# henryhungle/MTN

Measured on AMD Instinct MI355X. Metric: train-step samples/sec (d_model=512, 6L MTN), higher is better.
Workload: dtype bf16; 1 GPU; cfg2: d_model=512 N=6 h=8 d_ff=2048 |V|=3000 Q/H/C/T=20/128/40/20 frames=[32, 32] ft=[2048, 128]; batch_per_gpu=32, global_batch=32, parallelism=dp1, hip_graph=True, rccl_ranks=1

## Files before the change

### include/mtn_hip.h

```cpp
#ifndef MTN_HIP_H
#define MTN_HIP_H

#include <stdint.h>

#ifdef __cplusplus
extern "C" {
#endif

#define MTN_F32 0
#define MTN_BF16 1

#define MTN_OK 0
#define MTN_ERR_ARG 1
#define MTN_ERR_LAUNCH 2

const char* mtn_last_error(void);
int mtn_version(void);

typedef struct {
    float p;
    uint32_t salt;
    const uint64_t* seed;
} mtn_dropout;

// ... 79 lines not shown
} mtn_ln_fwd_desc;
typedef struct {
    int rows, d;
    const long* tokens;
    const float* dx;
    float emb_scale;
    mtn_dropout drop;
    float* dlut;
    int lut_rows;
} mtn_embed_bwd_desc;
int mtn_embed_bwd_group(int count, const mtn_embed_bwd_desc* descs , void* stream);
typedef struct {
    int rows, d;
    float eps;
    const float *x, *a2, *mean, *rstd, *g, *dres;
    float* dx;
    float* partial;
    void* dx_lp;
    int dx_lp_dtype;
    mtn_dropout dx_lp_drop;
} mtn_ln_bwd_desc;
int mtn_layernorm_fwd_group(int dtype, int count, const mtn_ln_fwd_desc* descs , void* stream);
int mtn_layernorm_bwd_group(int count, const mtn_ln_bwd_desc* descs , void* stream);
int mtn_layernorm_fwd(int dtype, int rows, int d, float eps, const float* x, const float* a2, const float* b2,
                      float* y_f32, void* y_lp, float* mean, float* rstd, void* stream);
typedef struct {
    const void* w;
    const float *bias, *a2, *b2;
    float* out;
    int K, block_start;
} mtn_ln_fold_desc;
int mtn_ln_fold(int dtype, const mtn_ln_fold_desc* descs_device, const int* block_desc, int total_blocks, int d, void* stream);
long mtn_layernorm_bwd_partial_floats(int rows, int d);
int mtn_layernorm_bwd_nparts(int rows);
typedef struct {
    const float* partial;
    int nparts, d;
    float *da2, *db2;
} mtn_ln_finalize_desc;
#define MTN_LN_FINALIZE_MAX_GROUP 112
int mtn_layernorm_bwd_finalize(int count, const mtn_ln_finalize_desc* descs , void* stream);
int mtn_layernorm_bwd(int rows, int d, float eps, const float* x, const float* a2, const float* mean,
                      const float* rstd, const float* g, const float* dres, float* dx, float* da2, float* db2,
                      float* partial, void* stream);

typedef struct {
    int B, h, a, m, dk;
    const void *q, *k, *v;
    int ldq, ldkv;
    const uint8_t* mask;
    long mask_sb, mask_sq;
    mtn_dropout drop;
    void* o;
    int ldo;
    float* lse;
    const void* d_o;
    void *dq, *dk_out, *dv_out;
    int q0, qn, kv_accum;
    float* kv_acc;
    int kv_last;
} mtn_attn_args;
#define MTN_ATTN_MAX_GROUP 4
int mtn_attention_fwd_group(int dtype, int count, const mtn_attn_args* args , void* stream);
int mtn_attention_bwd_group(int dtype, int count, const mtn_attn_args* args , void* stream);
int mtn_attention_fwd(int dtype, const mtn_attn_args* args, void* stream);
int mtn_attention_bwd(int dtype, const mtn_attn_args* args, void* stream);

typedef struct {
    int B, a, m, d, h;
    int self_attn;
    float ln_eps;
    mtn_dropout drop_attn;
    mtn_dropout drop_out;
    const float* x;
    const void* mem;
    const uint8_t* mask;
    long mask_sb, mask_sq;
    const float *ln_a, *ln_b;
    const void* w_qkv;
    const float* b_qkv;
    const void* w_o;
    const float* b_o;
    const void* w_qkv_t;
    const void* w_o_t;
    float* y;
    void* xn;
    float* mean;
    float* rstd;
    void* qkv;
    void* kv;
    void* o;
    float* lse;
    const float* dy;
    float* dx;
    float* dmem;
    int dmem_accumulate;
    float *d_ln_a, *d_ln_b;
    float *d_w_qkv, *d_b_qkv, *d_w_o, *d_b_o;
    void* ws_lp;
    float* ws_f32;
    int defer_param_grads;
    const void* dyl_ready;
    void* next_dyl;
    mtn_dropout next_drop;
    int kv_ready;
    void* dmem_lp;
    mtn_dropout dmem_lp_drop;
    const float* ln_fold;
} mtn_mha_args;
int mtn_mha_sublayer_fwd(int dtype, const mtn_mha_args* args, void* stream);
int mtn_mha_sublayer_bwd(int dtype, const mtn_mha_args* args, void* stream);
int mtn_mha_param_grad_work(int dtype, const mtn_mha_args* args, mtn_gemm_problem* out3, mtn_ln_finalize_desc* out_ln);
long mtn_mha_bwd_ws_lp_elems(int B, int a, int m, int d, int self_attn);
long mtn_mha_bwd_ws_f32_floats(int B, int a, int m, int d);

typedef struct {
    int rows, d, d_ff;
    float ln_eps;
    mtn_dropout drop_hidden;
    mtn_dropout drop_out;
    const float* x;
    const float *ln_a, *ln_b;
    const void* w1;
    const float* b1;
    const void* w2;
    const float* b2;
    const void* w1_t;
    const void* w2_t;
    float* y;
    void* xn;
    float* mean;
    float* rstd;
    void* hid;
    const float* dy;
    float* dx;
    float *d_ln_a, *d_ln_b, *d_w1, *d_b1, *d_w2, *d_b2;
    void* ws_lp;
    float* ws_f32;
    int defer_param_grads;
    const void* dyl_ready;
    void* next_dyl;
    mtn_dropout next_drop;
    void* y_lp;
    const float* ln_fold;
} mtn_ffn_args;
int mtn_ffn_sublayer_fwd(int dtype, const mtn_ffn_args* args, void* stream);
int mtn_ffn_sublayer_bwd(int dtype, const mtn_ffn_args* args, void* stream);
long mtn_ffn_bwd_ws_f32_floats(int rows, int d, int d_ff);
int mtn_ffn_param_grad_work(int dtype, const mtn_ffn_args* args, mtn_gemm_problem* out2, mtn_ln_finalize_desc* out_ln);

#define MTN_SUBLAYER_MAX_GROUP 4
int mtn_fused_enable(int on);
int mtn_fused_counters(long* out4);
long mtn_ln_epilogue_groups(void);
int mtn_sublayer_group_fwd(int dtype, int n_mha, const mtn_mha_args* mha, int n_ffn, const mtn_ffn_args* ffn, void* stream);
int mtn_sublayer_group_bwd(int dtype, int n_mha, const mtn_mha_args* mha, int n_ffn, const mtn_ffn_args* ffn, void* stream);

int mtn_cast_f32_to_lp(int dtype, long n, const float* src, void* dst, void* stream);
typedef struct {
    long n;
    const float* src;
    void* dst;
    mtn_dropout drop;
    const float* gate;
} mtn_cast_desc;
#define MTN_CAST_MAX_GROUP 8
int mtn_cast_group(int dtype, int count, const mtn_cast_desc* descs , void* stream);
int mtn_dropout_bwd_to_lp(int dtype, long n, const float* src, mtn_dropout drop, void* dst, void* stream);

#define MTN_LOSSHEAD_MAX_SEG 4
typedef struct {
    int n_seg;
    int rows[MTN_LOSSHEAD_MAX_SEG];
    const long* target[MTN_LOSSHEAD_MAX_SEG];
    const float* norm[MTN_LOSSHEAD_MAX_SEG];
    float coef[MTN_LOSSHEAD_MAX_SEG];
    int V, ldz, pad;
    float smoothing;
    const float* logits;
    float* lse;
    float* rowloss;
    const float* gloss;
    void* dlogits;
    int ldd;
} mtn_losshead_args;
int mtn_losshead_fwd(const mtn_losshead_args* args, void* stream);
int mtn_losshead_bwd(int dtype, const mtn_losshead_args* args, void* stream);

typedef struct {
    long off;
    int rows, cols;
    int tile_start;
    int reserved;
    long dst_off;
} mtn_transpose_desc;
int mtn_transpose_group(int dtype, const void* src, void* dst, const mtn_transpose_desc* descs_device, int count,
                        int total_tiles, void* stream);

int mtn_noam_tick(float* state, float factor, int model_size, int warmup, float beta1, float beta2, void* stream);
int mtn_adam_step(int dtype, long n, float* p, const float* g, float* m, float* v, void* p_lp, const float* state,
                  const float* grad_scale, float beta1, float beta2, float eps, void* stream);
int mtn_adam_step_chunks(int dtype, int n_chunks, const long* off, const int* len, float* p, const float* g, float* m, float* v,
                         void* p_lp, const float* state, const float* grad_scale, float beta1, float beta2, float eps, void* stream);

#define MTN_ASSEMBLE_MAX_GROUP 8
typedef struct {
    const int64_t* flat;
    const int64_t* start;
    const int32_t* len;
    const int32_t* ids;
    int B, L;
    int64_t pad;
    int64_t* out;
    uint8_t* mask;
    uint8_t* std_mask;
    int64_t* n_nonpad;
    const int32_t* row_len;
} mtn_assemble_tokens_desc;
int mtn_assemble_tokens(int count, const mtn_assemble_tokens_desc* descs , void* stream);
typedef struct {
    const float* flat;
    const int64_t* start;
    const int32_t* len;
    const int32_t* ids;
    int B, V, F, skip;
    float* out;
    uint8_t* mask;
} mtn_assemble_features_desc;
int mtn_assemble_features(int count, const mtn_assemble_features_desc* descs , void* stream);

int mtn_topk_rows(const float* x, int rows, int V, long ldx, int k, int extra_col, float* out, void* stream);
typedef struct {
    int dialogues, width, L, k_top, k, beam, unk, eos, pad, min_len;
    double penalty;
    const float* top;
    long* tokens; int* pos; int* anc;
    double* lp; int* n_live; int* step; int* flags;
    int* log_parent; int* log_tok; double* log_score; double* log_done; int* log_n_old; int* log_n_new;
} mtn_beam_args;
int mtn_beam_advance(const mtn_beam_args* args , void* stream);
typedef struct {
    mtn_beam_args beam;
    int groups; float diversity;
} mtn_diverse_args;
int mtn_diverse_advance(const mtn_diverse_args* args , void* stream);
typedef struct {
    int rows, V; long ldx;
    const float* logp;
    float temperature; int top_k; float top_p;
    int n_banned; int banned[4]; int eos, min_len;
    const long* seed;
    const long* key;
    int* step;
    int L;
    int* log_tok; float* log_logp; float* log_u;
    long* tokens; int* pos; int* anc;
} mtn_sample_args;
int mtn_sample_rows(const mtn_sample_args* args , void* stream);
typedef struct {
    int n_seq, L, V, pad; long ldz;
    const float* logits;
    const long* target;
    float* tok_logp;
    int* tok_rank;
    double* seq_logp;
    int* seq_len;
} mtn_score_args;
int mtn_score_rows(const mtn_score_args* args , void* stream);
typedef struct {
    int rows, V; long ldx, ldo;
    const float* logp; float* out;
    int ngram; float theta;
    int L;
    const int* hist; long ldh; const int* hist_len;
    const int* log_tok; const int* log_parent; const int* step;
    int width, rows_per_step;
} mtn_constrain_args;
int mtn_constrain_rows(const mtn_constrain_args* args , void* stream);
typedef struct {
    int rows, V, M, mode;
    const float* x[8]; long ld[8]; float w[8];
    float* out; long ldo;
} mtn_ensemble_args;
int mtn_ensemble_rows(const mtn_ensemble_args* args , void* stream);
int mtn_log_softmax_rows(const float* x, int rows, int V, long ldx, float* out, long ldo, void* stream);

typedef struct {
    int dtype, count, variant, workgroups;
    double flops, bytes;
    int M[4], N[4], K[4];
} mtn_census_launch;
int mtn_census_begin(void);
int mtn_census_end(void);
int mtn_census_info(int i, mtn_census_launch* out);
int mtn_census_replay(int i, int reps, void* stream);
const char* mtn_census_variant_name(int variant);
int mtn_measure_mfma_peak(int iters, float* scratch, void* stream, double* tflops);
int mtn_measure_mfma_peak_shapes(int iters, float* scratch, void* stream, double* tflops_16x16x32, double* tflops_32x32x16);
int mtn_measure_hbm_peak(const void* src, void* dst, long bytes, void* stream, double* gbps);
#define MTN_DEC_EMBED 0
#define MTN_DEC_SELF_QKV 1
#define MTN_DEC_SELF_ATT 2
#define MTN_DEC_OUT 3
#define MTN_DEC_CROSS 4
#define MTN_DEC_FFN1 5
#define MTN_DEC_FFN2 6
// ... 34 lines not shown
```

### mtn_amd/csrc/elementwise.hip

```cpp
#include <stdarg.h>
#include <stdlib.h>

#include "common.h"

static thread_local char g_err[512] = "";
void mtn_set_error(const char* fmt, ...) {
    va_list ap;
    va_start(ap, fmt);
    vsnprintf(g_err, sizeof(g_err), fmt, ap);
    va_end(ap);
}
extern "C" const char* mtn_last_error(void) { return g_err; }
extern "C" int mtn_version(void) { return 119; }

#include <mutex>
static int g_env_gen = 0;
static std::mutex g_env_mutex;
extern "C" int mtn_reload_env(void) { return __atomic_add_fetch(&g_env_gen, 1, __ATOMIC_ACQ_REL); }
const char* mtn_env_lookup(MtnEnvVar* v) {
    const int g = __atomic_load_n(&g_env_gen, __ATOMIC_ACQUIRE);
    if (__atomic_load_n(&v->gen, __ATOMIC_ACQUIRE) != g) {
        std::lock_guard<std::mutex> lock(g_env_mutex);
        if (v->gen != g) {
            const char* e = getenv(v->name);
            v->set = e != nullptr;
            if (e) { strncpy(v->val, e, sizeof(v->val) - 1); v->val[sizeof(v->val) - 1] = 0; }
            __atomic_store_n(&v->gen, g, __ATOMIC_RELEASE);
        }
    }
    return v->set ? v->val : nullptr;
}

static inline int grid_for(long n_vec) {
    long b = (n_vec + 255) / 256;
    if (b > 2048) b = 2048;
    if (b < 1) b = 1;
    return (int)b;
}

struct CastGroup {
    int count;
    mtn_cast_desc d[MTN_CAST_MAX_GROUP];
};

template <typename T>
__global__ __launch_bounds__(256) void cast_kernel(const CastGroup grp) {
    const mtn_cast_desc& D = grp.d[blockIdx.y];
    const long n = D.n;
    const float* __restrict__ src = D.src;
    T* __restrict__ dst = (T*)D.dst;
    const DropState ds = drop_init(D.drop);
    const long n4 = n >> 2;
    for (long i = (long)blockIdx.x * 256 + threadIdx.x; i < n4; i += (long)gridDim.x * 256) {
        float4 v = *(const float4*)(src + i * 4);
        if (ds.on) {
            v.x = drop_keep(ds, (uint64_t)(i * 4 + 0)) ? v.x * ds.scale : 0.f;
            v.y = drop_keep(ds, (uint64_t)(i * 4 + 1)) ? v.y * ds.scale : 0.f;
            v.z = drop_keep(ds, (uint64_t)(i * 4 + 2)) ? v.z * ds.scale : 0.f;
            v.w = drop_keep(ds, (uint64_t)(i * 4 + 3)) ? v.w * ds.scale : 0.f;
        }
        if (D.gate) {
            const float4 gt = *(const float4*)(D.gate + i * 4);
            v.x = gt.x > 0.f ? v.x : 0.f; v.y = gt.y > 0.f ? v.y : 0.f; v.z = gt.z > 0.f ? v.z : 0.f; v.w = gt.w > 0.f ? v.w : 0.f;
        }
        if constexpr (sizeof(T) == 2) {
            uint2 u;
            u.x = (uint32_t)f32_to_bf16(v.x) | ((uint32_t)f32_to_bf16(v.y) << 16);
            u.y = (uint32_t)f32_to_bf16(v.z) | ((uint32_t)f32_to_bf16(v.w) << 16);
            *(uint2*)(dst + i * 4) = u;
        } else {
            *(float4*)(dst + i * 4) = v;
        }
    }
    if (blockIdx.x == 0 && threadIdx.x < (n & 3)) {
        long i = (n4 << 2) + threadIdx.x;
        float v = src[i];
        if (ds.on) v = drop_keep(ds, (uint64_t)i) ? v * ds.scale : 0.f;
        if (D.gate && !(D.gate[i] > 0.f)) v = 0.f;
        dst[i] = LP<T>::from_f32(v);
    }
}

extern "C" int mtn_cast_group(int dtype, int count, const mtn_cast_desc* descs, void* stream) {
    MTN_CHECK_ARG(dtype == MTN_F32 || dtype == MTN_BF16, "bad dtype");
    MTN_CHECK_ARG(count >= 1 && count <= MTN_CAST_MAX_GROUP && descs, "bad group");
    CastGroup grp;
    memset(&grp, 0, sizeof(grp));
    grp.count = count;
    long nmax = 0;
    for (int i = 0; i < count; ++i) {
        MTN_CHECK_ARG(descs[i].n > 0 && descs[i].src && descs[i].dst, "bad cast descriptor");
        grp.d[i] = descs[i];
        if (descs[i].n > nmax) nmax = descs[i].n;
    }
    hipStream_t s = (hipStream_t)stream;
    dim3 grid(grid_for(nmax >> 2), count);
    if (dtype == MTN_BF16) hipLaunchKernelGGL((cast_kernel<bf16_t>), grid, dim3(256), 0, s, grp);
    else hipLaunchKernelGGL((cast_kernel<float>), grid, dim3(256), 0, s, grp);
    MTN_CHECK_LAUNCH();
    return MTN_OK;
}

static int launch_cast(int dtype, long n, const float* src, void* dst, mtn_dropout drop, void* stream) {
    mtn_cast_desc D = {n, src, dst, drop, nullptr};
    return mtn_cast_group(dtype, 1, &D, stream);
}

extern "C" int mtn_cast_f32_to_lp(int dtype, long n, const float* src, void* dst, void* stream) {
    mtn_dropout none = {0.f, 0u, nullptr};
    return launch_cast(dtype, n, src, dst, none, stream);
}
extern "C" int mtn_dropout_bwd_to_lp(int dtype, long n, const float* src, mtn_dropout drop, void* dst, void* stream) {
    return launch_cast(dtype, n, src, dst, drop, stream);
}

template <typename T>
__global__ __launch_bounds__(256) void transpose_group_kernel(const T* __restrict__ src, T* __restrict__ dst,
                                                              const mtn_transpose_desc* __restrict__ descs, int count) {
    constexpr int V = 16 / (int)sizeof(T);
    __shared__ __attribute__((aligned(16))) T tile[64][64 + V];
    int lo = 0, hi = count - 1;
    const int b = blockIdx.x;
    while (lo < hi) {
        int mid = (lo + hi + 1) >> 1;
        if (descs[mid].tile_start <= b) lo = mid; else hi = mid - 1;
    }
    const mtn_transpose_desc D = descs[lo];
    const int tiles_c = (D.cols + 63) >> 6;
    const int t = b - D.tile_start;
    const int r0 = (t / tiles_c) * 64, c0 = (t % tiles_c) * 64;
    const T* s = src + D.off;
    T* d = dst + D.dst_off;
    const bool full = (r0 + 64 <= D.rows) && (c0 + 64 <= D.cols) && (D.rows % V == 0) && (D.cols % V == 0) && (D.off % V == 0) && (D.dst_off % V == 0);
    if (full) {
        constexpr int VPR = 64 / V;
        for (int i = threadIdx.x; i < 64 * VPR; i += 256) {
            const int r = i / VPR, cv = (i % VPR) * V;
            *(uint4*)&tile[r][cv] = *(const uint4*)(s + (size_t)(r0 + r) * D.cols + c0 + cv);
        }
        __syncthreads();
        for (int i = threadIdx.x; i < 64 * VPR; i += 256) {
            const int c = i / VPR, rv = (i % VPR) * V;
            __attribute__((aligned(16))) T tmp[V];
#pragma unroll
            for (int k = 0; k < V; ++k) tmp[k] = tile[rv + k][c];
            *(uint4*)(d + (size_t)(c0 + c) * D.rows + r0 + rv) = *(const uint4*)tmp;
        }
        return;
    }
    const int tx = threadIdx.x & 63, ty = threadIdx.x >> 6;
#pragma unroll 4
    for (int i = 0; i < 16; ++i) {
        const int r = r0 + ty + 4 * i, c = c0 + tx;
        if (r < D.rows && c < D.cols) tile[ty + 4 * i][tx] = s[(size_t)r * D.cols + c];
    }
    __syncthreads();
#pragma unroll 4
    for (int i = 0; i < 16; ++i) {
        const int c = c0 + ty + 4 * i, r = r0 + tx;
        if (r < D.rows && c < D.cols) d[(size_t)c * D.rows + r] = tile[tx][ty + 4 * i];
    }
}

extern "C" int mtn_transpose_group(int dtype, const void* src, void* dst, const mtn_transpose_desc* descs_device, int count,
                                   int total_tiles, void* stream) {
    MTN_CHECK_ARG(dtype == MTN_F32 || dtype == MTN_BF16, "bad dtype");
// ... 183 lines not shown
```

### mtn_amd/csrc/fused.hip

```cpp
#include "fused_common.h"

struct FhMember {
    int kind;
    int rows;
    int rows_per_wg;
    int nslice;
    int a, m, blk;
    int mt;
    int hg, sg;
    int late_v;
    int nks;
    int ncols;
    int ld_out;
    float eps;
    const float* x;
    const float* ln_a;
    const float* ln_b;
    const bf16_t* w;
    const float* bias;
    const bf16_t* mem;
    bf16_t* xn;
    float* mean;
    float* rstd;
    bf16_t* out;
    bf16_t* kv;
    const uint8_t* mask;
    long mask_sb, mask_sq;
    mtn_dropout drop;
    bf16_t* o;
    float* lse;
    int b_off;
};
struct FhGroup {
    int count;
    int stop;
#ifdef FH_TIMELINE
    unsigned long long* dbg;
#endif
    int wg_start[FH_MAX_MEMBERS + 1];
    FhMember m[FH_MAX_MEMBERS];
};

struct FhLds { int gains, xn, xm, qi, ki, vi, mask, total; };
__host__ __device__ inline FhLds fh_lds_map(int mt, bool raw, int key_rows, int pad_rows, int mask_bytes, int ffn_blocks = 0, bool late_v = false) {
    FhLds L;
    L.gains = 0;
    L.xn = 4096 + 1024;
    const int krows = ((key_rows + pad_rows + 7) & ~7);
    if (late_v) {
        L.vi = L.xn;
        const int top = mt * 16 * FH_ROWB > krows * FH_HROWB ? mt * 16 * FH_ROWB : krows * FH_HROWB;
        L.xm = L.xn + top;
        L.qi = L.xm;
        L.ki = L.qi + mt * 16 * FH_HROWB;
        L.mask = L.ki + krows * FH_HROWB;
        L.total = L.mask + ((mask_bytes + 15) & ~15);
        return L;
    }
    L.xm = L.xn + mt * 16 * FH_ROWB;
    L.qi = L.xm + (raw ? mt * 16 * FH_ROWB : 0);
    L.ki = L.qi + mt * 16 * (ffn_blocks ? ffn_blocks * FH_HROWB : FH_HROWB);
    L.vi = L.ki + krows * FH_HROWB;
    L.mask = L.vi + krows * FH_HROWB;
    L.total = L.mask + ((mask_bytes + 15) & ~15);
    return L;
}
static constexpr int FH_PART_FLOATS = 18;
__host__ __device__ inline int fh_pad_rows(int kind, int mk) { return kind == FH_CROSS_READY ? ((mk + 63) & ~63) - mk : 64; }

#ifdef FH_TIMELINE
#define FH_STAMP(k) do { if (threadIdx.x == 0) G.dbg[(size_t)blockIdx.x * 16 + (k)] = wall_clock64(); } while (0)
#define FH_STAMP_CLK(k) do { if (threadIdx.x == 0) G.dbg[(size_t)blockIdx.x * 16 + (k)] = clock64(); } while (0)
#else
#define FH_STAMP(k) do { } while (0)
#define FH_STAMP_CLK(k) do { } while (0)
#endif

template <int NP, int MT>
__device__ __forceinline__ void fh_body(const FhGroup& G, const FhMember& M, const int slice, const int rb, unsigned char* smem) {
    constexpr int NG = (MT * 4 + 7) / 8;
    constexpr int NT = NP * MT;
    const int tid = threadIdx.x;
    const int row0 = rb * M.rows_per_wg;
    const int R = (M.rows - row0) < M.rows_per_wg ? (M.rows - row0) : M.rows_per_wg;
    const int lane = tid & 63, l15 = lane & 15, lg = lane >> 4;
    const int wave = __builtin_amdgcn_readfirstlane(tid >> 6);
    const int wc = wave & 3, kh = wave >> 2;
    const int kind = M.kind;
    const bool raw = kind == FH_CROSS_RAW, ffn = kind == FH_FFN;
    const int a = M.a, m = M.m;
    const int nsamp = ffn ? 0 : R / a, b0 = rb * M.blk;
    const int Rm = raw ? nsamp * m : 0, rm0 = b0 * m;
    const int mk = kind == FH_SELF ? a : m;
    const int key_rows = ffn ? 0 : ((kind == FH_SELF || raw) ? MT * 16 : nsamp * m);
    const int qa = M.mask_sq ? a : 1;
    const int mask_bytes = ffn ? 0 : nsamp * qa * m;
    const bool late_v = kind == FH_CROSS_READY && M.late_v != 0;
    const FhLds L = fh_lds_map(MT, raw, key_rows, fh_pad_rows(kind, mk), mask_bytes, ffn ? NP : 0, late_v);
    unsigned char* xn_s = smem + L.xn;
    unsigned char* xm_s = smem + L.xm;
    unsigned char* qi_s = smem + L.qi;
    unsigned char* ki_s = smem + L.ki;
    unsigned char* vi_s = smem + L.vi;
    unsigned char* mk_s = smem + L.mask;

    float4 gv = make_float4(0.f, 0.f, 0.f, 0.f);
    if (tid < 256) gv = *(const float4*)((tid < 128 ? M.ln_a : M.ln_b - FH_D) + tid * 4);
    int ncol[NP];
    bool act[NP];
#pragma unroll
    for (int p = 0; p < NP; ++p) {
        if (ffn) { ncol[p] = slice * (64 * NP) + p * 64; act[p] = ncol[p] + 16 * wc < M.ncols; }
        else { ncol[p] = p * FH_D + slice * FH_DK; act[p] = (p == 0) || (p < 3 && kind != FH_CROSS_READY); }
    }
    float bias_v = 0.f;
    if (tid < 64 * NP) {
        const int p_ = tid >> 6;
        bool on = false;
        int nc = 0;
#pragma unroll
        for (int p = 0; p < NP; ++p) if (p == p_) { on = act[p] || (ffn && ncol[p] + (tid & 63) < M.ncols); nc = ncol[p]; }
        if (on) bias_v = M.bias[nc + (tid & 63)];
    }
    uint8_t mkb[FH_MASKB];
    const uint8_t* mask_g = M.mask ? M.mask + (size_t)b0 * M.mask_sb : nullptr;
    const bool mask_wide = M.mask == nullptr || (M.mask_sb != 0 && (((size_t)mask_g | (size_t)mask_bytes) & 7) == 0);
    unsigned mkw0 = 0x01010101u, mkw1 = 0x01010101u;
    if (mask_wide) {
        if (M.mask && 8 * tid < mask_bytes) { mkw0 = *(const unsigned*)(mask_g + 8 * tid); mkw1 = *(const unsigned*)(mask_g + 8 * tid + 4); }
    } else {
#pragma unroll
        for (int i = 0; i < FH_MASKB; ++i) {
            const int idx = tid + FH_THREADS * i;
            mkb[i] = 1;
            if (idx < mask_bytes) mkb[i] = mask_g[M.mask_sb ? idx : idx % (qa * m)];
        }
    }
    const float* __restrict__ xg = M.x + (size_t)row0 * FH_D;
    float4 xv[NG][8];
#pragma unroll
    for (int i = 0; i < NG; ++i) {
        const int r = 4 * (wave + 8 * i) + lg;
        const bool ok = r < R;
#pragma unroll
        for (int j = 0; j < 8; ++j)
            xv[i][j] = ok ? *(const float4*)(xg + (size_t)r * FH_D + 64 * j + 4 * l15) : make_float4(0.f, 0.f, 0.f, 0.f);
    }
    FH_STAMP(14);
    if (raw) {
        const fh_rsrc_t rsrc = fh_make_rsrc(M.mem + (size_t)rm0 * FH_D, (unsigned)(Rm * FH_ROWB));
        for (int r = wave; r < MT * 16; r += 8) {
            const unsigned voff = r < Rm ? (unsigned)r * FH_ROWB + (unsigned)((lane ^ (r & 15)) << 4) : 0x80000000u;
            fh_dma16(rsrc, (unsigned)(size_t)(xm_s + r * FH_ROWB), voff);
        }
    }
    auto issue_kv_dma = [&]() {
        const int Kr = nsamp * m;
        const bf16_t* kbase = M.kv + (size_t)rm0 * (2 * FH_D) + slice * FH_DK;
        const fh_rsrc_t rk = fh_make_rsrc(kbase, (unsigned)((Kr - 1) * (4 * FH_D) + FH_HROWB));
        const fh_rsrc_t rv = fh_make_rsrc(kbase + FH_D, (unsigned)((Kr - 1) * (4 * FH_D) + FH_HROWB));
        const int ninst = ((Kr + fh_pad_rows(kind, mk) + 7) & ~7) >> 3;
        for (int i = wave; i < ninst; i += 8) {
            const int row = i * 8 + (lane >> 3), slot = lane & 7;
            const unsigned vk = row < Kr ? (unsigned)row * (4 * FH_D) + (unsigned)((slot ^ (row & 7)) << 4) : 0x80000000u;
            const unsigned vv = row < Kr ? (unsigned)row * (4 * FH_D) + (unsigned)((slot ^ ((row >> 1) & 7)) << 4) : 0x80000000u;
            fh_dma16(rk, (unsigned)(size_t)(ki_s + i * 1024), vk);
            if (!late_v) fh_dma16(rv, (unsigned)(size_t)(vi_s + i * 1024), vv);
        }
    };
    uint4 wf[NP][8];
    auto issue_weights = [&]() {
#pragma unroll
        for (int p = 0; p < NP; ++p) {
            if (act[p]) {
                const bf16_t* wrow = M.w + (size_t)(ncol[p] + 16 * wc + (lane >> 2)) * FH_D + kh * 256 + (lane & 3) * 8;
#pragma unroll
                for (int s = 0; s < 8; ++s) wf[p][s] = *(const uint4*)(wrow + s * 32);
            } else {
#pragma unroll
                for (int s = 0; s < 8; ++s) wf[p][s] = make_uint4(0, 0, 0, 0);
            }
        }
    };
    auto issue_block = [&](const int p_) {
#pragma unroll
        for (int p = 0; p < NP; ++p) {
            if (p != p_) continue;
            const int nc = act[p] ? ncol[p] : ncol[0];
            const bf16_t* wrow = M.w + (size_t)(nc + 16 * wc + (lane >> 2)) * FH_D + kh * 256 + (lane & 3) * 8;
#pragma unroll
            for (int s = 0; s < 8; ++s) wf[p][s] = *(const uint4*)(wrow + s * 32);
        }
    };
    if (mask_wide) {
// ... 218 lines not shown

    FH_STAMP(8);
    if (late_v || kind == FH_CROSS_READY) {
        asm volatile("s_waitcnt vmcnt(0)" ::: "memory");
        __syncthreads();
    }
    const float scale = 0.125f;
    const int nqt = (a + 15) >> 4;
    auto attend = [&](const int si, const int qt, const int cbeg, const int cend, f32x4_t (&ot)[4], float& mrun, float& lrun) {
        const int b = b0 + si;
        const DropBase dbase = drop_base((uint64_t)((b + M.b_off) * (FH_D / FH_DK) + slice) * (uint64_t)a * (uint64_t)mk);
        const int q = qt * 16 + l15, qc = q < a ? q : a - 1;
        const int qrow = si * a + qc, krow0 = si * mk;
        uint4 qf[2];
#pragma unroll
        for (int ks = 0; ks < 2; ++ks) qf[ks] = fh_hfrag(qi_s, qrow, ks * 4 + lg);
#pragma unroll
        for (int nt = 0; nt < 4; ++nt) ot[nt] = f32x4_t{0.f, 0.f, 0.f, 0.f};
        mrun = -INFINITY; lrun = 0.f;
        const unsigned char* mrow = mk_s + (size_t)(si * qa + (M.mask_sq ? qc : 0)) * mk;
        for (int c0 = cbeg; c0 < cend; c0 += 64) {
            const bool wide = mk - c0 > 32;
            f32x4_t st[4];
#pragma unroll
            for (int kt = 0; kt < 4; ++kt) {
                st[kt] = f32x4_t{0.f, 0.f, 0.f, 0.f};
                if (kt >= 2 && !wide) continue;
                int key = c0 + 32 * (kt >> 1) + 8 * (l15 >> 2) + 4 * (kt & 1) + (l15 & 3);
                key = key < mk ? key : mk - 1;
#pragma unroll
                for (int ks = 0; ks < 2; ++ks) mma16<bf16_t>(st[kt], fh_hfrag(ki_s, krow0 + key, ks * 4 + lg), qf[ks]);
            }
            float mx = -INFINITY;
#pragma unroll
            for (int kt = 0; kt < 4; ++kt) {
                if (kt >= 2 && !wide) continue;
#pragma unroll
                for (int r = 0; r < 4; ++r) {
                    const int key = c0 + 32 * (kt >> 1) + 8 * lg + 4 * (kt & 1) + r, kc = key < mk ? key : mk - 1;
                    float sv = mrow[kc] != 0 ? st[kt][r] * scale : -1e9f;
                    sv = key < mk ? sv : -INFINITY;
                    st[kt][r] = sv;
                    mx = fmaxf(mx, sv);
                }
            }
            mx = fh_cross_max(mx);
            const float mn = fmaxf(mrun, mx);
            float psum = 0.f;
#pragma unroll
            for (int kt = 0; kt < 4; ++kt) {
                if (kt >= 2 && !wide) continue;
#pragma unroll
                for (int r = 0; r < 4; ++r) {
                    const int key = c0 + 32 * (kt >> 1) + 8 * lg + 4 * (kt & 1) + r, kc = key < mk ? key : mk - 1;
                    const float pv = __expf(st[kt][r] - mn);
                    psum += pv;
                    st[kt][r] = drop_keep_at(ds, dbase, (uint32_t)(qc * mk + kc)) ? pv * ds.scale : 0.f;
                }
            }
            psum = fh_cross_sum(psum);
            const float alpha = (mrun == -INFINITY) ? 0.f : __expf(mrun - mn);
            lrun = lrun * alpha + psum;
            mrun = mn;
#pragma unroll
            for (int nt = 0; nt < 4; ++nt) { ot[nt][0] *= alpha; ot[nt][1] *= alpha; ot[nt][2] *= alpha; ot[nt][3] *= alpha; }
#pragma unroll
            for (int u = 0; u < 2; ++u) {
                if (u == 1 && !wide) continue;
                const uint4 pf = make_uint4(fh_pack2(st[2 * u][0], st[2 * u][1]), fh_pack2(st[2 * u][2], st[2 * u][3]),
                                            fh_pack2(st[2 * u + 1][0], st[2 * u + 1][1]), fh_pack2(st[2 * u + 1][2], st[2 * u + 1][3]));
                uint4 vf[4];
#pragma unroll
                for (int nt = 0; nt < 4; ++nt) vf[nt] = fh_vfrag(vi_s, krow0 + c0 + 32 * u, nt * 16, l15, lg);
                asm volatile("s_waitcnt lgkmcnt(0)" ::: "memory");
                __builtin_amdgcn_sched_barrier(0);
#pragma unroll
                for (int nt = 0; nt < 4; ++nt) mma16<bf16_t>(ot[nt], vf[nt], pf);
            }
        }
    };
    auto finish = [&](const int si, const int qt, const f32x4_t (&ot)[4], const float mrun, const float lrun) {
        const int b = b0 + si, q = qt * 16 + l15;
        if (q < a) {
            const float inv = 1.0f / lrun;
            bf16_t* og = M.o + (size_t)(b * a + q) * FH_D + slice * FH_DK + 4 * lg;
#pragma unroll
            for (int nt = 0; nt < 4; ++nt)
                *(uint2*)(og + nt * 16) = make_uint2(fh_pack2(ot[nt][0] * inv, ot[nt][1] * inv), fh_pack2(ot[nt][2] * inv, ot[nt][3] * inv));
            if (M.lse && lg == 0) {
                float* stp = M.lse + 2 * ((size_t)(b * (FH_D / FH_DK) + slice) * a + q);
                stp[0] = mrun;
                stp[1] = inv;
            }
        }
    };
    const int nks = M.nks;
    if (nks <= 1) {
        for (int it = wave; it < nsamp * nqt; it += 8) {
            const int si = it / nqt, qt = it - si * nqt;
            f32x4_t ot[4];
            float mrun, lrun;
            attend(si, qt, 0, mk, ot, mrun, lrun);
            finish(si, qt, ot, mrun, lrun);
        }
    } else {
        const int npairs = nsamp * nqt;
        const int pair = wave / nks, kr = wave - pair * nks;
        const bool live = pair < npairs;
        const int si = live ? pair / nqt : 0, qt = live ? pair - si * nqt : 0;
        const int chunks = (mk + 63) >> 6, per = (chunks + nks - 1) / nks;
        int cbeg = kr * per * 64, cend = (kr + 1) * per * 64;
        cend = cend < mk ? cend : mk;
        f32x4_t ot[4];
        float mrun = -INFINITY, lrun = 0.f;
#pragma unroll
        for (int nt = 0; nt < 4; ++nt) ot[nt] = f32x4_t{0.f, 0.f, 0.f, 0.f};
        if (live && cbeg < cend) attend(si, qt, cbeg, cend, ot, mrun, lrun);
        __syncthreads();
        float* part = (float*)ki_s + (size_t)(pair * (nks - 1) + kr - 1) * (FH_PART_FLOATS * 64) + lane;
        if (live && kr != 0) {
#pragma unroll
            for (int nt = 0; nt < 4; ++nt)
#pragma unroll
                for (int r = 0; r < 4; ++r) part[(nt * 4 + r) * 64] = ot[nt][r];
            part[16 * 64] = mrun;
            part[17 * 64] = lrun;
        }
        __syncthreads();
        if (live && kr == 0) {
            for (int k = 1; k < nks; ++k) {
                const float* pk = (const float*)ki_s + (size_t)(pair * (nks - 1) + k - 1) * (FH_PART_FLOATS * 64) + lane;
                const float mo = pk[16 * 64], lo = pk[17 * 64];
                const float mn = fmaxf(mrun, mo);
                const float wa = (mrun == -INFINITY) ? 0.f : __expf(mrun - mn), wb = (mo == -INFINITY) ? 0.f : __expf(mo - mn);
                lrun = lrun * wa + lo * wb;
                mrun = mn;
#pragma unroll
                for (int nt = 0; nt < 4; ++nt)
#pragma unroll
                    for (int r = 0; r < 4; ++r) ot[nt][r] = ot[nt][r] * wa + pk[(nt * 4 + r) * 64] * wb;
            }
            finish(si, qt, ot, mrun, lrun);
        }
    }
    FH_STAMP(9);
    FH_STAMP_CLK(11);
}

template <int NP>
__global__ __launch_bounds__(FH_THREADS) void fused_head_fwd_kernel(const FhGroup G) {
    extern __shared__ __attribute__((aligned(16))) unsigned char smem[];
    FH_STAMP(0);
    FH_STAMP_CLK(10);
    int g = 0;
    while (g + 1 < G.count && (int)blockIdx.x >= G.wg_start[g + 1]) ++g;
    const FhMember& M = G.m[g];
    const int t = (int)blockIdx.x - G.wg_start[g];
    const int xcd = t & 7, j = t >> 3;
    const int hpg = M.nslice / M.hg;
    const int slice = (xcd % M.hg) * hpg + (j % hpg), rb = (j / hpg) * M.sg + (xcd / M.hg);
    FH_STAMP(12);
    if (rb * M.rows_per_wg >= M.rows) return;
    if constexpr (NP == 4) {
        if (M.mt <= 2) fh_body<NP, 2>(G, M, slice, rb, smem);
        else fh_body<NP, 4>(G, M, slice, rb, smem);
    } else {
        if (M.mt <= 2) fh_body<NP, 2>(G, M, slice, rb, smem);
        else if (M.mt == 3) fh_body<NP, 3>(G, M, slice, rb, smem);
        else if (M.mt == 4) fh_body<NP, 4>(G, M, slice, rb, smem);
        else fh_body<NP, 5>(G, M, slice, rb, smem);
    }
}

static int fh_enabled = -1;
extern "C" int mtn_fused_enable(int on) {
    const int prev = fh_enabled;
    fh_enabled = on ? 1 : 0;
    return prev;
}
static bool fh_env_off() {
    if (fh_enabled < 0) fh_enabled = 1;
    return fh_enabled == 0;
}

int fh_is_enabled() { return fh_env_off() ? 0 : 1; }

static constexpr int FH_LDS_MAX = 160 * 1024;
static const int fh_mt_sets[2][4] = {{2, 3, 4, 5}, {2, 4, 4, 4}};

struct FhPlan { int blk, mt, lds, late_v; };
static int fh_member_lds(const mtn_mha_args& A, int blk, int mt, bool late_v = false) {
    const bool self = A.self_attn != 0, raw = !self && !A.kv_ready;
    const int m = self ? A.a : A.m, qa = A.mask_sq ? A.a : 1;
    const int kind = self ? FH_SELF : (raw ? FH_CROSS_RAW : FH_CROSS_READY);
    return fh_lds_map(mt, raw, (self || raw) ? mt * 16 : blk * m, fh_pad_rows(kind, m), blk * qa * m, 0, late_v).total;
}
static FhPlan fh_plan_mha_at(const mtn_mha_args& A, int np, int blk) {
    const int* fh_mt_choices = fh_mt_sets[np == 4];
    const bool self = A.self_attn != 0, raw = !self && !A.kv_ready;
    const int m = self ? A.a : A.m, qa = A.mask_sq ? A.a : 1;
    FhPlan none = {0, 0, 0, 0};
    const int R = blk * A.a, Rm = blk * m;
    int mt = 0;
    for (int c = 0; c < 4; ++c)
        if (fh_mt_choices[c] * 16 >= R && (!raw || fh_mt_choices[c] * 16 >= Rm) && (np == 4 || fh_mt_choices[c] != 4 || A.a > 32)) { mt = fh_mt_choices[c]; break; }
    if (!mt) return none;
    if (A.mask && blk * qa * m > FH_THREADS * FH_MASKB) return none;
    int lds = fh_member_lds(A, blk, mt), late = 0;
    if (lds > FH_LDS_MAX && !self && !raw) {
        lds = fh_member_lds(A, blk, mt, true);
        late = 1;
    }
    if (lds > FH_LDS_MAX) return none;
    return FhPlan{blk, mt, lds, late};
}
static FhPlan fh_plan_mha(const mtn_mha_args& A, int budget, int np) {
    const bool self = A.self_attn != 0;
    const int m = self ? A.a : A.m, qa = A.mask_sq ? A.a : 1;
    FhPlan best = {0, 0, 0, 0};
    if (A.mask && A.mask_sb != 0 && A.mask_sb != (long)qa * m) return best;
    if (A.mask && A.mask_sq != 0 && A.mask_sq != m) return best;
    for (int blk = 1; blk <= A.B; ++blk) {
        const FhPlan pl = fh_plan_mha_at(A, np, blk);
        if (pl.blk == 0) break;
        best = pl;
        if (((A.B + blk - 1) / blk) * (FH_D / FH_DK) <= budget) break;
    }
    return best;
}

static void fh_pick_xcd_map(FhMember& M, int nrb, double x_bytes, double w_bytes) {
    double best = 1e30;
    M.hg = 8; M.sg = 1;
    for (int sg = 1; sg <= 8; sg *= 2) {
        const int hg = 8 / sg;
        if (nrb % sg != 0 || M.nslice % hg != 0) continue;
        const double c = x_bytes / sg + w_bytes / hg;
        if (c < best) { best = c; M.hg = hg; M.sg = sg; }
    }
}

struct FhLaunch { FhGroup G; int wgs, np; size_t lds; };
static bool fh_plan(int n_mha, const mtn_mha_args* mha, int n_ffn, const mtn_ffn_args* ffn, FhLaunch& P) {
    if (n_mha + n_ffn < 1 || n_mha + n_ffn > FH_MAX_MEMBERS) return false;
    FhGroup& G = P.G;
    memset(&G, 0, sizeof(G));
    int np = n_ffn > 0 ? 4 : 1;
    for (int i = 0; i < n_mha; ++i) {
        if (mha[i].d != FH_D || mha[i].h != FH_D / FH_DK) return false;
        if ((mha[i].self_attn || !mha[i].kv_ready) && np < 3) np = 3;
    }
    for (int i = 0; i < n_ffn; ++i)
        if (ffn[i].d != FH_D || ffn[i].d_ff % 256 != 0) return false;
    const int members = n_mha + n_ffn;
    const int budget = 256 / members > 8 ? 256 / members : 8;
    int n = 0, wgs = 0;
    size_t lds = 0;
    auto emit_mha = [&](const mtn_mha_args& a, const FhPlan& pl, const int s0, const int Bp) {
        FhMember& M = G.m[n];
        const int mm = a.self_attn ? a.a : a.m;
        const size_t r0 = (size_t)s0 * a.a, rm0 = (size_t)s0 * mm;
        M.kind = a.self_attn ? FH_SELF : (a.kv_ready ? FH_CROSS_READY : FH_CROSS_RAW);
        M.a = a.a; M.m = mm; M.blk = pl.blk; M.mt = pl.mt; M.late_v = pl.late_v;
        {
            const bool ksplit = true;
            const int npairs = pl.blk * ((a.a + 15) / 16), chunks = (M.m + 63) / 64;
            int nks = 1;
            if (ksplit && npairs <= 4 && chunks >= 4 && !a.self_attn && a.kv_ready) {
                nks = npairs == 1 ? 8 : (npairs == 2 ? 4 : 2);
                while (nks > chunks) nks >>= 1;
                const int kimg = ((pl.blk * M.m + fh_pad_rows(FH_CROSS_READY, M.m) + 7) & ~7) * FH_HROWB;
                if (npairs * (nks - 1) * FH_PART_FLOATS * 64 * 4 > kimg) nks = 1;
            }
            M.nks = nks;
        }
        const int ldo = a.self_attn ? 3 * FH_D : FH_D;
        M.rows = Bp * a.a; M.rows_per_wg = pl.blk * a.a; M.nslice = FH_D / FH_DK; M.b_off = s0;
        M.eps = a.ln_eps; M.x = a.x + r0 * FH_D; M.ln_a = a.ln_a; M.ln_b = a.ln_b;
        M.w = (const bf16_t*)a.w_qkv; M.bias = a.b_qkv; M.mem = a.mem ? (const bf16_t*)a.mem + rm0 * FH_D : nullptr;
        M.xn = (bf16_t*)a.xn + r0 * FH_D; M.mean = a.mean + r0; M.rstd = a.rstd + r0;
        M.out = (bf16_t*)a.qkv + r0 * ldo; M.ld_out = ldo; M.kv = a.kv ? (bf16_t*)a.kv + rm0 * 2 * FH_D : nullptr;
        M.mask = a.mask ? a.mask + (size_t)s0 * a.mask_sb : nullptr; M.mask_sb = a.mask_sb; M.mask_sq = a.mask_sq; M.drop = a.drop_attn;
        M.o = (bf16_t*)a.o + r0 * FH_D; M.lse = a.lse ? a.lse + 2 * (size_t)s0 * (FH_D / FH_DK) * a.a : nullptr;
        G.wg_start[n] = wgs;
        const int nrb = (Bp + pl.blk - 1) / pl.blk;
        fh_pick_xcd_map(M, nrb, (double)M.rows * FH_D * 4, (M.kind == FH_CROSS_READY ? 1.0 : 3.0) * FH_D * FH_D * 2);
        wgs += nrb * M.nslice;
        lds = (size_t)pl.lds > lds ? (size_t)pl.lds : lds;
        ++n;
    };
    FhPlan plan[MTN_SUBLAYER_MAX_GROUP];
    for (int i = 0; i < n_mha; ++i) {
        plan[i] = fh_plan_mha(mha[i], budget, np);
        if (plan[i].blk == 0) return false;
    }
    for (int i = 0; i < n_mha; ++i) emit_mha(mha[i], plan[i], 0, mha[i].B);
    for (int i = 0; i < n_ffn; ++i) {
        const mtn_ffn_args& a = ffn[i];
        FhMember& M = G.m[n];
        M.kind = FH_FFN;
        M.rows = a.rows; M.ncols = a.d_ff; M.nslice = a.d_ff / 256;
        int mt = 4;
        if (((a.rows + 31) / 32) * M.nslice <= budget) mt = 2;
        M.mt = mt; M.rows_per_wg = mt * 16; M.a = 1; M.m = 1; M.blk = mt * 16;
        M.eps = a.ln_eps; M.x = a.x; M.ln_a = a.ln_a; M.ln_b = a.ln_b;
        M.w = (const bf16_t*)a.w1; M.bias = a.b1;
        M.xn = (bf16_t*)a.xn; M.mean = a.mean; M.rstd = a.rstd;
        M.out = (bf16_t*)a.hid; M.ld_out = a.d_ff; M.drop = a.drop_hidden;
        G.wg_start[n] = wgs;
        int nrb = (a.rows + M.rows_per_wg - 1) / M.rows_per_wg;
        while ((nrb * M.nslice) % 8 != 0) ++nrb;
        fh_pick_xcd_map(M, nrb, (double)a.rows * FH_D * 4, (double)a.d_ff * FH_D * 2);
        wgs += nrb * M.nslice;
        const size_t l = (size_t)fh_lds_map(mt, false, 0, 0, 0, 4).total;
        lds = l > lds ? l : lds;
        ++n;
    }
    G.count = n;
    for (int i = n; i <= FH_MAX_MEMBERS; ++i) G.wg_start[i] = wgs;
    { static const int stop = [] { const char* e = getenv("MTN_FH_STOP"); return e ? atoi(e) : 0; }(); G.stop = stop; }
    P.wgs = wgs; P.np = np; P.lds = lds;
    return true;
}

int fh_group_eligible(int dtype, int n_mha, const mtn_mha_args* mha, int n_ffn, const mtn_ffn_args* ffn) {
    if (fh_env_off() || dtype != MTN_BF16) return 0;
    FhLaunch P;
    return fh_plan(n_mha, mha, n_ffn, ffn, P) ? 1 : 0;
}

template <int NP> static int fh_launch(const FhGroup& G, int wgs, size_t lds, hipStream_t s) {
    static bool attr = false;
    if (!attr) {
        if (hipFuncSetAttribute((const void*)fused_head_fwd_kernel<NP>, hipFuncAttributeMaxDynamicSharedMemorySize, FH_LDS_MAX) != hipSuccess) {
            mtn_set_error("fused_head_fwd_kernel: cannot raise the dynamic LDS limit");
            return MTN_ERR_LAUNCH;
        }
        attr = true;
    }
    hipLaunchKernelGGL((fused_head_fwd_kernel<NP>), dim3(wgs), dim3(FH_THREADS), lds, s, G);
    return MTN_OK;
}

int fh_group_fwd_stage1(int n_mha, const mtn_mha_args* mha, int n_ffn, const mtn_ffn_args* ffn, void* stream) {
    FhLaunch P;
    MTN_CHECK_ARG(fh_plan(n_mha, mha, n_ffn, ffn, P), "group outside the fused kernel's tiling");
    hipStream_t s = (hipStream_t)stream;
    const int rc = P.np == 4 ? fh_launch<4>(P.G, P.wgs, P.lds, s) : (P.np == 3 ? fh_launch<3>(P.G, P.wgs, P.lds, s) : fh_launch<1>(P.G, P.wgs, P.lds, s));
    if (rc != MTN_OK) return rc;
    MTN_CHECK_LAUNCH();
    return MTN_OK;
}
```

### mtn_amd/csrc/gemm.hip

```cpp
#include <stdlib.h>
#include <type_traits>

#include "common.h"

struct GemmGroup {
    int count;
    int plain_tile_order;
    int epi_pre;
    unsigned char xcd_rg[MTN_GEMM_MAX_GROUP];
    int tile_start[MTN_GEMM_MAX_GROUP + 1];
    mtn_gemm_problem p[MTN_GEMM_MAX_GROUP];
};

int gemm_k512_try(int count, const mtn_gemm_problem* p, int min_tiles, hipStream_t s, int* tiles_out);

struct AdamSlot { float *p, *m, *v; void* lp; void* lpT; int ldT, write_grad; };
struct AdamGroup {
    const float* state;
    const float* grad_scale;
    float beta1, beta2, eps;
    int any;
    int lds_epilogue;
    AdamSlot a[MTN_GEMM_MAX_GROUP];
};
// ... 1908 lines not shown
    const long need = ((long)sizeof(TTHeader) + (long)count * sizeof(TTProblem) + (tiles + n_front) * 4 + 15) / 16 * 16 + ln_bytes + (long)n_chunks * 12 + 16;
    MTN_CHECK_ARG(need <= MTN_TT_SLOT_BYTES, "problem list too large for one table");
    hipStreamCaptureStatus cap = hipStreamCaptureStatusNone;
    (void)hipStreamIsCapturing(s, &cap);
    TTSlot own, *sl;
    if (cap != hipStreamCaptureStatusNone) {
        if (tt_slot_alloc(own) != MTN_OK) return MTN_ERR_LAUNCH;
        sl = &own;
    } else {
        sl = &g_tt_ring[g_tt_next];
        g_tt_next = (g_tt_next + 1) % 8;
        if (!sl->host) { if (tt_slot_alloc(*sl) != MTN_OK) return MTN_ERR_LAUNCH; }
        else if (!sl->fresh) (void)hipEventSynchronize(sl->ev);
    }
    TTHeader* H = (TTHeader*)sl->host;
    memset(H, 0, sizeof(*H));
    H->n_problems = count; H->n_tiles = (int)tiles;
    H->problems_off = sizeof(TTHeader);
    H->tilemap_off = sizeof(TTHeader) + (long)count * sizeof(TTProblem);
    TTProblem* Q = (TTProblem*)(sl->host + H->problems_off);
    uint32_t* map = (uint32_t*)(sl->host + H->tilemap_off);
    bool lds_ok = true;
    if (aux) {
        H->n_front = n_front; H->n_ln_units = n_ln_units; H->n_chunks = n_chunks;
        H->fp = aux->p; H->fg = aux->g; H->fm = aux->m; H->fv = aux->v; H->flp = (bf16_t*)aux->lp;
        H->ln_off = ((long)sizeof(TTHeader) + (long)count * sizeof(TTProblem) + (tiles + n_front) * 4 + 15) / 16 * 16;
        H->chunk_off_off = H->ln_off + ln_bytes;
        H->chunk_len_off = H->chunk_off_off + (long)n_chunks * 8;
        TTLnUnit* U = (TTLnUnit*)(sl->host + H->ln_off);
        int k = 0;
        for (int i = 0; i < aux->n_ln; ++i)
            for (int c0 = 0; c0 < 2 * aux->ln[i].d; c0 += 256) {
                TTLnUnit& u = U[k++];
                memset(&u, 0, sizeof(u));
                u.partial = aux->ln[i].partial; u.nparts = aux->ln[i].nparts; u.d = aux->ln[i].d; u.col0 = c0; u.a_off = aux->ln[i].a_off; u.b_off = aux->ln[i].b_off;
            }
        if (n_chunks) {
            memcpy(sl->host + H->chunk_off_off, aux->chunk_off, (size_t)n_chunks * 8);
            memcpy(sl->host + H->chunk_len_off, aux->chunk_len, (size_t)n_chunks * 4);
        }
    }
    int first = 0;
    for (int i = 0; i < count; ++i) {
        const mtn_gemm_problem& p = problems[i];
        TTProblem& q = Q[i];
        memset(&q, 0, sizeof(q));
        q.A = p.A; q.B = p.B; q.out = p.out_f32; q.rowsum = p.rowsum_out;
        q.bias_off = -1;
        if (aux && aux->bias_adam && p.rowsum_out && p.rowsum_out >= aux->g && p.rowsum_out + p.M <= aux->g + aux->n_flat) q.bias_off = (long)(p.rowsum_out - aux->g);
        q.lda = p.lda; q.ldb = p.ldb; q.M = p.M; q.N = p.N; q.K = p.K; q.ldc = p.ldc;
        q.tiles_m = (p.M + 127) / 128; q.tiles_n = (p.N + 127) / 128; q.first_tile = first;
        if (p.adam) {
            const mtn_adam_fuse& f = *p.adam;
            MTN_CHECK_ARG(f.p && f.m && f.v && f.state, "optimiser epilogue: p, m, v and state are required");
            MTN_CHECK_ARG(!f.p_lpT || f.ldT >= p.M, "optimiser epilogue: ldT is the row stride of the transposed copy (>= M)");
            if (!H->any) { H->state = f.state; H->grad_scale = f.grad_scale; H->beta1 = f.beta1; H->beta2 = f.beta2; H->eps = f.eps; H->any = 1; }
            MTN_CHECK_ARG(H->state == f.state && H->grad_scale == f.grad_scale && H->beta1 == f.beta1 && H->beta2 == f.beta2 && H->eps == f.eps,
                          "optimiser epilogue: one set of hyper-parameters per launch");
            q.p = f.p; q.m = f.m; q.v = f.v; q.lp = f.p_lp; q.lpT = f.p_lpT; q.ldT = f.ldT; q.write_grad = f.write_grad;
            if ((f.p_lpT && (f.ldT % 8 != 0 || (((uintptr_t)f.p_lpT) & 15) != 0)) || (((uintptr_t)f.p) & 15) != 0 || (f.p_lp && (((uintptr_t)f.p_lp) & 7) != 0))
                lds_ok = false;
        }
        first += q.tiles_m * q.tiles_n;
    }
    if (aux && (n_front > 0 || aux->bias_adam)) {
        MTN_CHECK_ARG(aux->state, "mtn_tt_aux: the optimiser state is required");
        if (!H->any) { H->state = aux->state; H->grad_scale = aux->grad_scale; H->beta1 = aux->beta1; H->beta2 = aux->beta2; H->eps = aux->eps; H->any = 1; }
        MTN_CHECK_ARG(H->state == aux->state && H->grad_scale == aux->grad_scale && H->beta1 == aux->beta1 && H->beta2 == aux->beta2 && H->eps == aux->eps,
                      "mtn_tt_aux: one set of optimiser hyper-parameters per launch");
    }
    H->lds_epilogue = (H->any && lds_ok) ? 1 : 0;
    {
        H->plain_tile_order = 1;
        std::vector<int> order(count);
        std::vector<double> cost(count);
        for (int i = 0; i < count; ++i) {
            order[i] = i;
            cost[i] = (double)Q[i].tiles_m * Q[i].tiles_n * (Q[i].K + (Q[i].p ? 896.0 : 128.0));
        }
        std::stable_sort(order.begin(), order.end(), [&](int a, int b) { return cost[a] > cost[b]; });
        std::vector<int> owner(count);
        double load[8] = {0, 0, 0, 0, 0, 0, 0, 0};
        for (int k = 0; k < count; ++k) {
            int c = 0;
            for (int x = 1; x < 8; ++x) if (load[x] < load[c]) c = x;
            owner[order[k]] = c;
            load[c] += cost[order[k]];
        }
        std::vector<uint32_t> queue[8];
        for (int i = 0; i < count; ++i)
            for (int k = 0; k < Q[i].tiles_m * Q[i].tiles_n; ++k) queue[owner[i]].push_back(((uint32_t)i << 12) | (uint32_t)k);
        size_t head[8] = {0, 0, 0, 0, 0, 0, 0, 0};
        for (long i = 0; i < tiles; ++i) {
            int c = (int)(i & 7);
            if (head[c] >= queue[c].size()) {
                int best = -1;
                size_t left = 0;
                for (int x = 0; x < 8; ++x)
                    if (queue[x].size() - head[x] > left) { left = queue[x].size() - head[x]; best = x; }
                c = best;
            }
            map[i] = queue[c][head[c]++];
        }
    }
    if (n_front > 0) {
        std::vector<uint32_t> dmap(map, map + tiles);
        long pos = 0;
        for (long au = 0; au < n_front; ++au) map[pos++] = 0x80000000u | (uint32_t)au;
        for (long di = 0; di < tiles; ++di) map[pos++] = dmap[di];
    }
    static bool attr_set = false;
    if (!attr_set) {
        (void)hipFuncSetAttribute((const void*)gemm_tt_dma128_table_kernel, hipFuncAttributeMaxDynamicSharedMemorySize, TTB_LDS);
        attr_set = true;
    }
    hipError_t e;
    if (cap != hipStreamCaptureStatusNone) {
        hipStreamCaptureMode mode = hipStreamCaptureModeRelaxed;
        (void)hipThreadExchangeStreamCaptureMode(&mode);
        static hipStream_t copy_stream = nullptr;
        e = copy_stream ? hipSuccess : hipStreamCreateWithFlags(&copy_stream, hipStreamNonBlocking);
        if (e == hipSuccess) e = hipMemcpyAsync(sl->dev, sl->host, (size_t)need, hipMemcpyHostToDevice, copy_stream);
        if (e == hipSuccess) e = hipStreamSynchronize(copy_stream);
        (void)hipThreadExchangeStreamCaptureMode(&mode);
    } else {
        e = hipMemcpyAsync(sl->dev, sl->host, (size_t)need, hipMemcpyHostToDevice, s);
    }
    if (e != hipSuccess) { mtn_set_error("mtn_gemm_tt_table: staging copy failed: %s", hipGetErrorString(e)); return MTN_ERR_LAUNCH; }
    hipLaunchKernelGGL(gemm_tt_dma128_table_kernel, dim3((unsigned)(tiles + n_front)), dim3(256), TTB_LDS, s, (const TTHeader*)sl->dev);
    MTN_CHECK_LAUNCH();
    if (cap == hipStreamCaptureStatusNone) { (void)hipEventRecord(sl->ev, s); sl->fresh = false; }
    if (g_census_on) {
        CensusTable t;
        t.p.assign(problems, problems + count);
        t.adam.resize(count);
        for (int i = 0; i < count; ++i)
            if (problems[i].adam) t.adam[i] = *problems[i].adam;
        t.has_aux = aux != nullptr;
        if (aux) {
            t.aux = *aux;
            t.ln.assign(aux->ln, aux->ln + aux->n_ln);
            t.chunk_off.assign(aux->chunk_off, aux->chunk_off + aux->n_chunks);
            t.chunk_len.assign(aux->chunk_len, aux->chunk_len + aux->n_chunks);
        }
        CensusEntry e;
        memset(&e, 0, sizeof(e));
        e.dtype = dtype; e.count = count; e.variant = V_TT_TABLE; e.tiles = (int)tiles; e.table = (int)g_census_tables.size();
        g_census_tables.push_back(t);
        g_census.push_back(e);
    }
    return MTN_OK;
}

extern "C" int mtn_census_begin(void) { g_census.clear(); g_census_tables.clear(); g_census_on = true; return MTN_OK; }
extern "C" int mtn_census_end(void) { g_census_on = false; return (int)g_census.size(); }
extern "C" const char* mtn_census_variant_name(int variant) { return (variant >= 0 && variant < V_COUNT) ? g_variant_name[variant] : "?"; }

extern "C" int mtn_census_info(int i, mtn_census_launch* out) {
    MTN_CHECK_ARG(i >= 0 && i < (int)g_census.size() && out, "bad census index");
    const CensusEntry& e = g_census[i];
    const double esz = (e.dtype == MTN_BF16) ? 2.0 : 4.0;
    memset(out, 0, sizeof(*out));
    out->dtype = e.dtype; out->count = e.count; out->variant = e.variant; out->workgroups = e.tiles;
    if (e.table >= 0) {
        const CensusTable& t = g_census_tables[e.table];
        for (int k = 0; k < e.count; ++k) {
            const mtn_gemm_problem& p = t.p[k];
            out->flops += 2.0 * p.M * p.N * p.K;
            double per = 4.0;
            if (p.adam) per = 24.0 + (t.adam[k].p_lp ? esz : 0.0) + (t.adam[k].p_lpT ? esz : 0.0) + (t.adam[k].write_grad ? 4.0 : 0.0);
            out->bytes += ((double)p.M + p.N) * p.K * esz + (double)p.M * p.N * per;
            if (k < 4) { out->M[k] = p.M; out->N[k] = p.N; out->K[k] = p.K; }
        }
        if (t.has_aux) {
            for (size_t c = 0; c < t.chunk_len.size(); ++c) out->bytes += (double)t.chunk_len[c] * (28.0 + (t.aux.lp ? esz : 0.0));
            for (size_t u = 0; u < t.ln.size(); ++u) out->bytes += 2.0 * t.ln[u].d * (4.0 * t.ln[u].nparts + 28.0 + (t.aux.lp ? esz : 0.0));
            if (t.aux.bias_adam)
                for (int k = 0; k < e.count; ++k)
                    if (t.p[k].rowsum_out && t.p[k].rowsum_out >= t.aux.g && t.p[k].rowsum_out + t.p[k].M <= t.aux.g + t.aux.n_flat)
                        out->bytes += (double)t.p[k].M * (28.0 + (t.aux.lp ? esz : 0.0));
        }
        return MTN_OK;
    }
    for (int k = 0; k < e.count; ++k) {
        const mtn_gemm_problem& p = e.p[k];
        out->flops += 2.0 * p.M * p.N * p.K;
        if (p.ln && e.ln[k].mode == MTN_LN_CONSUME)
            out->bytes += ((double)p.M + p.N) * p.K * esz + (double)p.M * p.N * (8.0 + (e.ln[k].dres ? 4.0 : 0.0) + (e.ln[k].dx_lp ? esz : 0.0));
        else
        out->bytes += ((double)p.M + p.N) * p.K * esz + (double)p.M * p.N * ((p.out_f32 ? 4.0 : 0.0) + (p.out_lp ? esz : 0.0)) +
                      (p.residual ? (double)p.M * p.N * 4.0 : 0.0);
        if (k < 4) { out->M[k] = p.M; out->N[k] = p.N; out->K[k] = p.K; }
    }
    return MTN_OK;
}

extern "C" int mtn_census_replay(int i, int reps, void* stream) {
    MTN_CHECK_ARG(i >= 0 && i < (int)g_census.size() && reps >= 1, "bad census index");
    const bool was = g_census_on;
    g_census_on = false;
    CensusEntry e = g_census[i];
    if (e.table >= 0) {
        CensusTable t = g_census_tables[e.table];
        for (int k = 0; k < e.count; ++k)
            if (t.p[k].adam) t.p[k].adam = &t.adam[k];
        g_census_on = false;
        int rc = MTN_OK;
        if (t.has_aux) { t.aux.ln = t.ln.data(); t.aux.chunk_off = t.chunk_off.data(); t.aux.chunk_len = t.chunk_len.data(); }
        for (int r = 0; r < reps && rc == MTN_OK; ++r) rc = mtn_gemm_tt_table_aux(e.dtype, e.count, t.p.data(), t.has_aux ? &t.aux : nullptr, stream);
        g_census_on = was;
        return rc;
    }
    for (int k = 0; k < e.count; ++k)
    {
        if (e.p[k].adam) e.p[k].adam = &e.adam[k];
        if (e.p[k].ln) e.p[k].ln = &e.ln[k];
    }
    int rc = MTN_OK;
    for (int r = 0; r < reps && rc == MTN_OK; ++r) rc = mtn_gemm(e.dtype, e.count, e.p, stream);
    g_census_on = was;
    return rc;
}


typedef float f32x16_t __attribute__((ext_vector_type(16)));
template <int SHAPE>
__global__ __launch_bounds__(256) void mfma_spin_kernel(float* out, int iters) {
    bf16x8_t a, b;
#pragma unroll
    for (int i = 0; i < 8; ++i) { a[i] = (__bf16)(0.001f * (float)(threadIdx.x + i)); b[i] = (__bf16)(0.002f * (float)((int)threadIdx.x - i)); }
    if (SHAPE == 16) {
        f32x4_t c[8];
#pragma unroll
        for (int j = 0; j < 8; ++j) c[j] = f32x4_t{0.f, 0.f, 0.f, 0.f};
        for (int i = 0; i < iters; ++i) {
#pragma unroll
            for (int j = 0; j < 8; ++j) c[j] = __builtin_amdgcn_mfma_f32_16x16x32_bf16(a, b, c[j], 0, 0, 0);
        }
        f32x4_t s = c[0] + c[1] + c[2] + c[3] + c[4] + c[5] + c[6] + c[7];
        if (s[0] == 123.456f) out[blockIdx.x * 256 + threadIdx.x] = s[1];
    } else {
        f32x16_t c[4];
#pragma unroll
        for (int j = 0; j < 4; ++j)
#pragma unroll
            for (int k = 0; k < 16; ++k) c[j][k] = 0.f;
        for (int i = 0; i < iters; ++i) {
#pragma unroll
            for (int j = 0; j < 4; ++j) c[j] = __builtin_amdgcn_mfma_f32_32x32x16_bf16(a, b, c[j], 0, 0, 0);
        }
        f32x16_t s = c[0] + c[1] + c[2] + c[3];
        if (s[0] == 123.456f) out[blockIdx.x * 256 + threadIdx.x] = s[1] + s[15];
    }
}

static int measure_mfma(int shape, int iters, float* scratch, hipStream_t s, double* tflops) {
    hipEvent_t e0, e1;
    if (hipEventCreate(&e0) != hipSuccess || hipEventCreate(&e1) != hipSuccess) { mtn_set_error("hipEventCreate failed"); return MTN_ERR_LAUNCH; }
    const int wgs = 256 * 8;
    double best = 0.0;
    for (int rep = 0; rep < 10; ++rep) {
        (void)hipEventRecord(e0, s);
        if (shape == 16) hipLaunchKernelGGL(mfma_spin_kernel<16>, dim3(wgs), dim3(256), 0, s, scratch, iters);
        else hipLaunchKernelGGL(mfma_spin_kernel<32>, dim3(wgs), dim3(256), 0, s, scratch, iters);
        (void)hipEventRecord(e1, s);
        (void)hipEventSynchronize(e1);
        float ms = 0.f;
        (void)hipEventElapsedTime(&ms, e0, e1);
        const double per_iter = shape == 16 ? 8 * (2.0 * 16 * 16 * 32) : 4 * (2.0 * 32 * 32 * 16);
        const double tf = (double)wgs * 4 * iters * per_iter / (ms * 1e-3) / 1e12;
        if (tf > best) best = tf;
    }
    (void)hipEventDestroy(e0); (void)hipEventDestroy(e1);
    MTN_CHECK_LAUNCH();
    *tflops = best;
    return MTN_OK;
}

extern "C" int mtn_measure_mfma_peak(int iters, float* scratch, void* stream, double* tflops) {
    MTN_CHECK_ARG(iters > 0 && scratch && tflops, "bad arguments");
    double a = 0.0, b = 0.0;
    int rc = measure_mfma(16, iters, scratch, (hipStream_t)stream, &a);
    if (rc == MTN_OK) rc = measure_mfma(32, iters, scratch, (hipStream_t)stream, &b);
    *tflops = a > b ? a : b;
    return rc;
}

extern "C" int mtn_measure_mfma_peak_shapes(int iters, float* scratch, void* stream, double* tflops_16x16x32, double* tflops_32x32x16) {
    MTN_CHECK_ARG(iters > 0 && scratch && tflops_16x16x32 && tflops_32x32x16, "bad arguments");
    int rc = measure_mfma(16, iters, scratch, (hipStream_t)stream, tflops_16x16x32);
    if (rc == MTN_OK) rc = measure_mfma(32, iters, scratch, (hipStream_t)stream, tflops_32x32x16);
    return rc;
}
```

### mtn_amd/csrc/gemm_k512.hip

```cpp
#include "fused_common.h"

static constexpr int GK_THREADS = 512;
static constexpr int GK_K = 512;
static constexpr int GK_LDS = 128 * FH_ROWB;
static constexpr int GK_CPITCH = 272;

struct GkProblem { const bf16_t* A; const bf16_t* B; const float* bias; bf16_t* out; int lda, ldb, ldc, M, N, tiles_m; };
struct GkGroup {
    int count;
    int tile_start[MTN_GEMM_MAX_GROUP + 1];
    GkProblem p[MTN_GEMM_MAX_GROUP];
};

__global__ __launch_bounds__(GK_THREADS) void gemm_k512_kernel(const GkGroup G) {
    extern __shared__ __attribute__((aligned(16))) unsigned char smem[];
    const int tid = threadIdx.x, lane = tid & 63, l15 = lane & 15, lg = lane >> 4;
    const int wave = __builtin_amdgcn_readfirstlane(tid >> 6);
    int g = 0;
    while (g + 1 < G.count && (int)blockIdx.x >= G.tile_start[g + 1]) ++g;
    const GkProblem& P = G.p[g];
    const int t = (int)blockIdx.x - G.tile_start[g];
    const int tn = t / P.tiles_m, tm = t - tn * P.tiles_m;
    const int row0 = tm * 128, col0 = tn * 128;
    const int R = (P.M - row0) < 128 ? (P.M - row0) : 128;
    {
        const unsigned ldab = (unsigned)P.lda * 2u;
        const __amdgpu_buffer_rsrc_t rs = __builtin_amdgcn_make_buffer_rsrc((void*)(P.A + (size_t)row0 * P.lda), 0, (R - 1) * ldab + FH_ROWB, 0x00020000);
        for (int r = wave; r < 128; r += 8) {
            const unsigned vo = r < R ? (unsigned)r * ldab + (unsigned)((lane ^ (r & 15)) << 4) : 0x80000000u;
            __builtin_amdgcn_raw_ptr_buffer_load_lds(rs, (fh_lds_void_t*)(smem + r * FH_ROWB), 16, vo, 0, 0, 0);
        }
    }
    uint4 wf[16];
    {
        int n = col0 + 16 * wave + (lane >> 2);
        n = n < P.N ? n : P.N - 1;
        const bf16_t* wrow = P.B + (size_t)n * P.ldb + (lane & 3) * 8;
#pragma unroll
        for (int s = 0; s < 16; ++s) wf[s] = *(const uint4*)(wrow + s * 32);
    }
    const int colq = col0 + 16 * wave + 4 * lg;
    float4 bq = make_float4(0.f, 0.f, 0.f, 0.f);
    if (P.bias && colq < P.N) bq = *(const float4*)(P.bias + colq);
    asm volatile("s_waitcnt vmcnt(0)" ::: "memory");
    __syncthreads();
    {
        const int src = (4 * l15 + lg) * 4;
#pragma unroll
        for (int s = 0; s < 16; ++s) {
            wf[s].x = (unsigned)__builtin_amdgcn_ds_bpermute(src, (int)wf[s].x);
            wf[s].y = (unsigned)__builtin_amdgcn_ds_bpermute(src, (int)wf[s].y);
            wf[s].z = (unsigned)__builtin_amdgcn_ds_bpermute(src, (int)wf[s].z);
            wf[s].w = (unsigned)__builtin_amdgcn_ds_bpermute(src, (int)wf[s].w);
        }
    }
    f32x4_t acc[8];
#pragma unroll
    for (int mt = 0; mt < 8; ++mt) acc[mt] = f32x4_t{0.f, 0.f, 0.f, 0.f};
#pragma unroll
    for (int s = 0; s < 16; ++s)
#pragma unroll
        for (int mt = 0; mt < 8; ++mt) mma16<bf16_t>(acc[mt], wf[s], fh_xfrag(smem, mt * 16 + l15, s * 4 + lg));
    __syncthreads();
#pragma unroll
    for (int mt = 0; mt < 8; ++mt) {
        const int r = mt * 16 + l15;
        *(uint2*)(smem + r * GK_CPITCH + (16 * wave + 4 * lg) * 2) =
            make_uint2(fh_pack2(acc[mt][0] + bq.x, acc[mt][1] + bq.y), fh_pack2(acc[mt][2] + bq.z, acc[mt][3] + bq.w));
    }
    __syncthreads();
#pragma unroll
    for (int ps = 0; ps < 4; ++ps) {
        const int r = ps * 32 + (tid >> 4), c = tid & 15;
        const int col = col0 + c * 8;
        if (r < R && col < P.N)
            *(uint4*)(P.out + (size_t)(row0 + r) * P.ldc + col) = *(const uint4*)(smem + r * GK_CPITCH + c * 16);
    }
}

static constexpr int GW_CPITCH = 528;
__global__ __launch_bounds__(GK_THREADS) void gemm_k512w_kernel(const GkGroup G) {
    extern __shared__ __attribute__((aligned(16))) unsigned char smem[];
    const int tid = threadIdx.x, lane = tid & 63, l15 = lane & 15, lg = lane >> 4;
    const int wave = __builtin_amdgcn_readfirstlane(tid >> 6);
    int g = 0;
    while (g + 1 < G.count && (int)blockIdx.x >= G.tile_start[g + 1]) ++g;
    const GkProblem& P = G.p[g];
    const int t = (int)blockIdx.x - G.tile_start[g];
    const int tn = t / P.tiles_m, tm = t - tn * P.tiles_m;
    const int row0 = tm * 128, col0 = tn * 256;
    const int R = (P.M - row0) < 128 ? (P.M - row0) : 128;
    {
        const unsigned ldab = (unsigned)P.lda * 2u;
        const __amdgpu_buffer_rsrc_t rs = __builtin_amdgcn_make_buffer_rsrc((void*)(P.A + (size_t)row0 * P.lda), 0, (R - 1) * ldab + FH_ROWB, 0x00020000);
        for (int r = wave; r < 128; r += 8) {
            const unsigned vo = r < R ? (unsigned)r * ldab + (unsigned)((lane ^ (r & 15)) << 4) : 0x80000000u;
            __builtin_amdgcn_raw_ptr_buffer_load_lds(rs, (fh_lds_void_t*)(smem + r * FH_ROWB), 16, vo, 0, 0, 0);
        }
    }
    float4 bq[2];
#pragma unroll
    for (int cb = 0; cb < 2; ++cb) {
        const int colq = col0 + 128 * cb + 16 * wave + 4 * lg;
        bq[cb] = make_float4(0.f, 0.f, 0.f, 0.f);
        if (P.bias && colq < P.N) bq[cb] = *(const float4*)(P.bias + colq);
    }
    __builtin_amdgcn_sched_barrier(0);
    uint4 wf[2][16];
    {
        const bf16_t* wrow[2];
#pragma unroll
        for (int cb = 0; cb < 2; ++cb) {
            int n = col0 + 128 * cb + 16 * wave + (lane >> 2);
            n = n < P.N ? n : P.N - 1;
            wrow[cb] = P.B + (size_t)n * P.ldb + (lane & 3) * 8;
        }
#pragma unroll
        for (int s = 0; s < 16; ++s) { wf[0][s] = *(const uint4*)(wrow[0] + s * 32); wf[1][s] = *(const uint4*)(wrow[1] + s * 32); }
    }
    __builtin_amdgcn_sched_barrier(0);
    __builtin_amdgcn_s_waitcnt(0x8F70);
    __builtin_amdgcn_s_barrier();
    f32x4_t acc[2][8];
#pragma unroll
    for (int cb = 0; cb < 2; ++cb)
#pragma unroll
        for (int mt = 0; mt < 8; ++mt) acc[cb][mt] = f32x4_t{0.f, 0.f, 0.f, 0.f};
    const int src = (4 * l15 + lg) * 4;
#pragma unroll
    for (int s = 0; s < 16; ++s) {
#pragma unroll
        for (int cb = 0; cb < 2; ++cb) {
            wf[cb][s].x = (unsigned)__builtin_amdgcn_ds_bpermute(src, (int)wf[cb][s].x);
            wf[cb][s].y = (unsigned)__builtin_amdgcn_ds_bpermute(src, (int)wf[cb][s].y);
            wf[cb][s].z = (unsigned)__builtin_amdgcn_ds_bpermute(src, (int)wf[cb][s].z);
            wf[cb][s].w = (unsigned)__builtin_amdgcn_ds_bpermute(src, (int)wf[cb][s].w);
        }
#pragma unroll
        for (int mt = 0; mt < 8; ++mt) {
            const uint4 xf = fh_xfrag(smem, mt * 16 + l15, s * 4 + lg);
            mma16<bf16_t>(acc[0][mt], wf[0][s], xf);
            mma16<bf16_t>(acc[1][mt], wf[1][s], xf);
        }
    }
    __syncthreads();
#pragma unroll
    for (int cb = 0; cb < 2; ++cb)
#pragma unroll
        for (int mt = 0; mt < 8; ++mt) {
            const int r = mt * 16 + l15;
            *(uint2*)(smem + r * GW_CPITCH + (128 * cb + 16 * wave + 4 * lg) * 2) =
                make_uint2(fh_pack2(acc[cb][mt][0] + bq[cb].x, acc[cb][mt][1] + bq[cb].y), fh_pack2(acc[cb][mt][2] + bq[cb].z, acc[cb][mt][3] + bq[cb].w));
        }
    __syncthreads();
#pragma unroll
    for (int ps = 0; ps < 8; ++ps) {
        const int r = ps * 16 + (tid >> 5), c = tid & 31;
        const int col = col0 + c * 8;
        if (r < R && col < P.N)
            *(uint4*)(P.out + (size_t)(row0 + r) * P.ldc + col) = *(const uint4*)(smem + r * GW_CPITCH + c * 16);
    }
}

static constexpr int GP_ROWS = 64;
static constexpr int GP_IMG = GP_ROWS * FH_ROWB;
static constexpr int GP_STG = 2 * GP_IMG;
static constexpr int GP_LDS = GP_STG + GP_ROWS * GK_CPITCH;
static constexpr int GP_GRID = 256;

struct GpUnit { int p, tn, tm; };

__device__ __forceinline__ GpUnit gp_first_from(const GkGroup& G, int p, int u, int xcd, int j) {
    for (; p < G.count; ++p, u = -1) {
        const GkProblem& P = G.p[p];
        const int ntn = (P.N + 127) >> 7, tm64 = (P.M + GP_ROWS - 1) / GP_ROWS;
        const int nr = tm64 > xcd ? (tm64 - xcd + 7) >> 3 : 0;
        if (u < 0) u = (j + 5 * p) & 31;
        if (u < nr * ntn) return GpUnit{p, u % ntn, xcd + 8 * (u / ntn)};
    }
    return GpUnit{-1, 0, 0};
}

__global__ __launch_bounds__(GK_THREADS, 2) void gemm_k512p_kernel(const GkGroup G) {
    extern __shared__ __attribute__((aligned(16))) unsigned char smem[];
    const int tid = threadIdx.x, lane = tid & 63, l15 = lane & 15, lg = lane >> 4;
    const int wave = __builtin_amdgcn_readfirstlane(tid >> 6);
    const int xcd = (int)blockIdx.x & 7, j = (int)blockIdx.x >> 3;

    auto unit_u = [&](const GpUnit& c) {
        const int ntn = (G.p[c.p].N + 127) >> 7;
        return ((c.tm - xcd) >> 3) * ntn + c.tn;
    };
    auto next_of = [&](const GpUnit& c) { return gp_first_from(G, c.p, unit_u(c) + 32, xcd, j); };
    const bool loader = wave < 4;
    auto issue_x = [&](const GpUnit& c, unsigned char* img) {
        if (!loader || c.p < 0) return;
        const GkProblem& P = G.p[c.p];
        const int row0 = c.tm * GP_ROWS;
        const int R = (P.M - row0) < GP_ROWS ? (P.M - row0) : GP_ROWS;
        const unsigned ldab = (unsigned)P.lda * 2u;
        const __amdgpu_buffer_rsrc_t rs = __builtin_amdgcn_make_buffer_rsrc((void*)(P.A + (size_t)row0 * P.lda), 0, (R - 1) * ldab + FH_ROWB, 0x00020000);
#pragma unroll
        for (int i = 0; i < GP_ROWS / 4; ++i) {
            const int r = wave + 4 * i;
            const unsigned vo = r < R ? (unsigned)r * ldab + (unsigned)((lane ^ (r & 15)) << 4) : 0x80000000u;
            __builtin_amdgcn_raw_ptr_buffer_load_lds(rs, (fh_lds_void_t*)(img + r * FH_ROWB), 16, vo, 0, 0, 0);
        }
    };
    uint4 wf[16];
    float4 bq = make_float4(0.f, 0.f, 0.f, 0.f);
    auto issue_w = [&](const GpUnit& c) {
        const GkProblem& P = G.p[c.p];
        int n = c.tn * 128 + 16 * wave + (lane >> 2);
        n = n < P.N ? n : P.N - 1;
        const bf16_t* wrow = P.B + (size_t)n * P.ldb + (lane & 3) * 8;
#pragma unroll
        for (int s = 0; s < 16; ++s) wf[s] = *(const uint4*)(wrow + s * 32);
        const int colq = c.tn * 128 + 16 * wave + 4 * lg;
        bq = make_float4(0.f, 0.f, 0.f, 0.f);
        if (P.bias && colq < P.N) bq = *(const float4*)(P.bias + colq);
    };

    auto load_w = [&](const GpUnit& c) {
        issue_w(c);
        const int src = (4 * l15 + lg) * 4;
#pragma unroll
        for (int s = 0; s < 16; ++s) {
            wf[s].x = (unsigned)__builtin_amdgcn_ds_bpermute(src, (int)wf[s].x);
            wf[s].y = (unsigned)__builtin_amdgcn_ds_bpermute(src, (int)wf[s].y);
            wf[s].z = (unsigned)__builtin_amdgcn_ds_bpermute(src, (int)wf[s].z);
            wf[s].w = (unsigned)__builtin_amdgcn_ds_bpermute(src, (int)wf[s].w);
        }
        asm volatile("s_waitcnt lgkmcnt(0)" ::: "memory");
    };
#ifdef GP_STAMPS
    long long* dbg_ = (long long*)(G.p[0].out + (size_t)G.p[0].M * G.p[0].ldc) + (wave >= 4 ? 512 : 0);
    int dbg_n_ = 0;
#define GP_STAMP() do { if ((int)blockIdx.x == GP_STAMPS && (tid == 0 || tid == 256) && dbg_n_ < 500) dbg_[dbg_n_++] = (long long)wall_clock64(); } while (0)
#else
#define GP_STAMP() do { } while (0)
#endif
    GpUnit cur = gp_first_from(G, 0, -1, xcd, j);
    if (cur.p < 0) return;
    GpUnit nxt = next_of(cur);
    GP_STAMP();
    issue_x(cur, smem);
    if (nxt.p >= 0) issue_x(nxt, smem + GP_IMG);
    load_w(cur);
    GP_STAMP();
    for (int i = 0;; ++i) {
        if (loader) {
            if (nxt.p >= 0) asm volatile("s_waitcnt vmcnt(16)" ::: "memory");
            else asm volatile("s_waitcnt vmcnt(0)" ::: "memory");
        }
        GP_STAMP();
        __builtin_amdgcn_s_barrier();
        GP_STAMP();
        const unsigned char* img = smem + (i & 1) * GP_IMG;
        f32x4_t acc[4];
#pragma unroll
        for (int mt = 0; mt < 4; ++mt) acc[mt] = f32x4_t{0.f, 0.f, 0.f, 0.f};
        {
            u32x4_t xa[4], xb[4];
            const unsigned ibase = (unsigned)(size_t)img;
            auto xload = [&](u32x4_t* x, int s) {
#pragma unroll
                for (int mt = 0; mt < 4; ++mt) {
                    const int row = mt * 16 + l15;
                    const unsigned addr = ibase + row * FH_ROWB + (((s * 4 + lg) ^ (row & 15)) << 4);
                    asm volatile("ds_read_b128 %0, %1" : "=v"(x[mt]) : "v"(addr));
                }
            };
            auto landed = [&](u32x4_t* x) {
                asm volatile("s_waitcnt lgkmcnt(0)" ::: "memory");
#pragma unroll
                for (int mt = 0; mt < 4; ++mt) MTN_LANDED(x[mt]);
                __builtin_amdgcn_sched_barrier(0);
            };
            xload(xa, 0);
#pragma unroll
            for (int s = 0; s < 16; s += 2) {
                landed(xa);
                xload(xb, s + 1);
                __builtin_amdgcn_sched_barrier(0);
#pragma unroll
                for (int mt = 0; mt < 4; ++mt) mma16<bf16_t>(acc[mt], wf[s], as_uint4(xa[mt]));
                __builtin_amdgcn_sched_barrier(0);
                landed(xb);
                if (s + 2 < 16) xload(xa, s + 2);
                __builtin_amdgcn_sched_barrier(0);
#pragma unroll
                for (int mt = 0; mt < 4; ++mt) mma16<bf16_t>(acc[mt], wf[s + 1], as_uint4(xb[mt]));
                __builtin_amdgcn_sched_barrier(0);
            }
        }
        GP_STAMP();
#pragma unroll
        for (int mt = 0; mt < 4; ++mt) {
            const int r = mt * 16 + l15;
            *(uint2*)(smem + GP_STG + r * GK_CPITCH + (16 * wave + 4 * lg) * 2) =
                make_uint2(fh_pack2(acc[mt][0] + bq.x, acc[mt][1] + bq.y), fh_pack2(acc[mt][2] + bq.z, acc[mt][3] + bq.w));
        }
        asm volatile("s_waitcnt lgkmcnt(0)" ::: "memory");
        GP_STAMP();
        __builtin_amdgcn_s_barrier();
        GP_STAMP();
        const GpUnit nn = nxt.p >= 0 ? next_of(nxt) : GpUnit{-1, 0, 0};
        const bool new_w = nxt.p >= 0 && (nxt.p != cur.p || nxt.tn != cur.tn);
        if (new_w) load_w(nxt);
        if (loader) { __builtin_amdgcn_s_barrier(); issue_x(nn.p >= 0 ? nn : GpUnit{-1, 0, 0}, smem + (i & 1) * GP_IMG); }
        if (!loader) {
            const GkProblem& P = G.p[cur.p];
            const int row0 = cur.tm * GP_ROWS, col0 = cur.tn * 128;
            const int R = (P.M - row0) < GP_ROWS ? (P.M - row0) : GP_ROWS;
            const int t4 = tid - 256;
            u32x4_t o[4];
#pragma unroll
            for (int ps = 0; ps < 4; ++ps) {
                const unsigned addr = (unsigned)(size_t)(smem + GP_STG + (ps * 16 + (t4 >> 4)) * GK_CPITCH + (t4 & 15) * 16);
                asm volatile("ds_read_b128 %0, %1" : "=v"(o[ps]) : "v"(addr));
            }
            asm volatile("s_waitcnt lgkmcnt(0)" ::: "memory");
#pragma unroll
            for (int ps = 0; ps < 4; ++ps) MTN_LANDED(o[ps]);
            __builtin_amdgcn_sched_barrier(0);
#pragma unroll
            for (int ps = 0; ps < 4; ++ps) {
                const int r = ps * 16 + (t4 >> 4), c8 = t4 & 15;
                const int col = col0 + c8 * 8;
                if (r < R && col < P.N)
                    *(uint4*)(P.out + (size_t)(row0 + r) * P.ldc + col) = as_uint4(o[ps]);
            }
            __builtin_amdgcn_s_barrier();
        }
        if (nxt.p < 0) break;
        cur = nxt; nxt = nn;
    }
}

int gemm_k512_try(int count, const mtn_gemm_problem* p, int min_tiles, hipStream_t s, int* tiles_out) {
    if (count < 1 || count > MTN_GEMM_MAX_GROUP) return 0;
    GkGroup G;
    memset(&G, 0, sizeof(G));
    int tiles = 0;
    for (int i = 0; i < count; ++i) {
        const mtn_gemm_problem& q = p[i];
        if (q.a_trans || q.b_trans || q.K != GK_K || q.relu || q.gate || q.residual || q.out_f32 || q.rowsum_out || q.adam || !q.out_lp) return 0;
        if (q.drop.p > 0.f && q.drop.seed) return 0;
        if (q.M < 1 || q.N < 8 || (q.N & 7) || (q.lda & 7) || (q.ldb & 7) || (q.ldc & 7) || q.lda < GK_K || q.ldb < GK_K) return 0;
        if ((long)q.M * q.lda * 2 >= (1L << 31)) return 0;
        if (((size_t)q.A | (size_t)q.B | (size_t)q.out_lp) & 15) return 0;
        if (q.bias && ((size_t)q.bias & 15)) return 0;
        GkProblem& P = G.p[i];
        P.A = (const bf16_t*)q.A; P.B = (const bf16_t*)q.B; P.bias = q.bias; P.out = (bf16_t*)q.out_lp;
        P.lda = q.lda; P.ldb = q.ldb; P.ldc = q.ldc; P.M = q.M; P.N = q.N; P.tiles_m = (q.M + 127) / 128;
        G.tile_start[i] = tiles;
        tiles += P.tiles_m * ((q.N + 127) / 128);
    }
    if (tiles < min_tiles) return 0;
    G.count = count;
    for (int i = count; i <= MTN_GEMM_MAX_GROUP; ++i) G.tile_start[i] = tiles;
    static bool attr = false;
    if (!attr) {
        if (hipFuncSetAttribute((const void*)gemm_k512_kernel, hipFuncAttributeMaxDynamicSharedMemorySize, GK_LDS) != hipSuccess) return 0;
        if (hipFuncSetAttribute((const void*)gemm_k512p_kernel, hipFuncAttributeMaxDynamicSharedMemorySize, GP_LDS) != hipSuccess) return 0;
        attr = true;
    }
    long units = 0;
    for (int i = 0; i < count; ++i) units += (long)((p[i].M + GP_ROWS - 1) / GP_ROWS) * ((p[i].N + 127) / 128);
    const char* pe = MTN_ENV("MTN_K512_PERSIST");
    if (pe ? pe[0] != '0' : units >= 20L * GP_GRID) {
        hipLaunchKernelGGL(gemm_k512p_kernel, dim3(GP_GRID), dim3(GK_THREADS), GP_LDS, s, G);
        if (hipGetLastError() != hipSuccess) return -1;
        if (tiles_out) *tiles_out = GP_GRID;
        return 1;
    }
    bool wide = true;
    for (int i = 0; i < count; ++i) wide = wide && (p[i].N % 256) == 0;
    if (wide) {
        static bool attr_w = false;
        if (!attr_w) {
            if (hipFuncSetAttribute((const void*)gemm_k512w_kernel, hipFuncAttributeMaxDynamicSharedMemorySize, GK_LDS) != hipSuccess) return 0;
            attr_w = true;
        }
        int tw = 0;
        for (int i = 0; i < count; ++i) { G.tile_start[i] = tw; tw += G.p[i].tiles_m * (p[i].N / 256); }
        for (int i = count; i <= MTN_GEMM_MAX_GROUP; ++i) G.tile_start[i] = tw;
        hipLaunchKernelGGL(gemm_k512w_kernel, dim3(tw), dim3(GK_THREADS), GK_LDS, s, G);
        if (hipGetLastError() != hipSuccess) return -1;
        if (tiles_out) *tiles_out = tw;
        return 1;
    }
    hipLaunchKernelGGL(gemm_k512_kernel, dim3(tiles), dim3(GK_THREADS), GK_LDS, s, G);
    if (hipGetLastError() != hipSuccess) return -1;
    if (tiles_out) *tiles_out = tiles;
    return 1;
}
```

### mtn_amd/csrc/sublayer.hip

```cpp
#include "common.h"

int fh_group_eligible(int dtype, int n_mha, const mtn_mha_args* mha, int n_ffn, const mtn_ffn_args* ffn);
int fh_group_fwd_stage1(int n_mha, const mtn_mha_args* mha, int n_ffn, const mtn_ffn_args* ffn, void* stream);
int fh_is_enabled();
struct FbIo { const void* dyl; void *dq, *dk, *dv; int ldq, ldkv; const float* lnf; float* ln_part; };
int fb_group_eligible(int dtype, int n_mha, const mtn_mha_args* mha, const FbIo* io);
int fb_group_bwd_stage(int n_mha, const mtn_mha_args* mha, const FbIo* io, void* stream);

static constexpr int LN_PART_HEADS = 8;

static inline const char* lp_off(const void* p, long elems, int dtype) {
    return (const char*)p + elems * (dtype == MTN_BF16 ? 2 : 4);
}
static inline char* lp_off(void* p, long elems, int dtype) { return (char*)p + elems * (dtype == MTN_BF16 ? 2 : 4); }

static mtn_gemm_problem gemm_init(const void* A, int lda, const void* B, int ldb, int M, int N, int K, int at, int bt) {
    mtn_gemm_problem p;
    memset(&p, 0, sizeof(p));
    p.A = A; p.lda = lda; p.B = B; p.ldb = ldb; p.M = M; p.N = N; p.K = K; p.a_trans = at; p.b_trans = bt;
    p.gate_scale = 1.f;
    return p;
}

static long g_fused_counts[4] = {0, 0, 0, 0};
static long g_ln_epi_groups = 0;
extern "C" long mtn_ln_epilogue_groups(void) { return g_ln_epi_groups; }
extern "C" int mtn_fused_counters(long* out4) {
    MTN_CHECK_ARG(out4, "null output");
    for (int i = 0; i < 4; ++i) out4[i] = g_fused_counts[i];
    return MTN_OK;
}

#define RUN(expr)                        \
    do {                                 \
        int rc__ = (expr);               \
        if (rc__ != MTN_OK) return rc__; \
    } while (0)

static int run_gemms(int dtype, int n, const mtn_gemm_problem* p, void* stream) {
    mtn_gemm_problem buf[MTN_GEMM_MAX_GROUP];
    for (int bt = 0; bt < 2; ++bt) {
        int k = 0;
        for (int i = 0; i < n; ++i)
            if (p[i].b_trans == bt) buf[k++] = p[i];
        if (k) RUN(mtn_gemm(dtype, k, buf, stream));
    }
    return MTN_OK;
}

static int check_mha(const mtn_mha_args* a, bool bwd) {
    MTN_CHECK_ARG(a, "null args");
    MTN_CHECK_ARG(a->B > 0 && a->a > 0 && a->d > 0 && a->h > 0 && a->d % a->h == 0, "bad shape");
    MTN_CHECK_ARG(a->d % 8 == 0 && (a->d / a->h) % 4 == 0, "d_model must be a multiple of 8 and d_k of 4");
    MTN_CHECK_ARG(a->self_attn || (a->m > 0 && a->mem && a->kv), "cross attention needs mem/kv");
    MTN_CHECK_ARG(a->x && a->ln_a && a->ln_b && a->w_qkv && a->b_qkv && a->w_o && a->b_o, "null parameter");
    MTN_CHECK_ARG(a->xn && a->mean && a->rstd && a->qkv && a->o && a->lse, "null saved buffer");
    if (!bwd) MTN_CHECK_ARG(a->y, "null output");
    else {
        MTN_CHECK_ARG(a->dy && a->dx && a->d_ln_a && a->d_ln_b && a->d_w_qkv && a->d_b_qkv && a->d_w_o && a->d_b_o, "null gradient buffer");
        MTN_CHECK_ARG(a->ws_lp && a->ws_f32, "null workspace");
    }
    return MTN_OK;
}

static int check_ffn(const mtn_ffn_args* a, bool bwd) {
    MTN_CHECK_ARG(a, "null args");
    MTN_CHECK_ARG(a->rows > 0 && a->d > 0 && a->d_ff > 0 && a->d % 8 == 0 && a->d_ff % 8 == 0, "bad shape");
    MTN_CHECK_ARG(a->x && a->ln_a && a->ln_b && a->w1 && a->b1 && a->w2 && a->b2, "null parameter");
    MTN_CHECK_ARG(a->xn && a->mean && a->rstd && a->hid, "null saved buffer");
    if (!bwd) MTN_CHECK_ARG(a->y, "null output");
    else {
        MTN_CHECK_ARG(a->dy && a->dx && a->d_ln_a && a->d_ln_b && a->d_w1 && a->d_b1 && a->d_w2 && a->d_b2, "null gradient buffer");
        MTN_CHECK_ARG(a->ws_lp && a->ws_f32, "null workspace");
    }
    return MTN_OK;
}

void attn_args_of(const mtn_mha_args* a, int dtype, mtn_attn_args* t) {
    const int d = a->d, m = a->self_attn ? a->a : a->m;
    memset(t, 0, sizeof(*t));
    t->B = a->B; t->h = a->h; t->a = a->a; t->m = m; t->dk = d / a->h;
    if (a->self_attn) {
        t->q = a->qkv; t->k = lp_off(a->qkv, d, dtype); t->v = lp_off(a->qkv, 2 * d, dtype); t->ldq = t->ldkv = 3 * d;
    } else {
        t->q = a->qkv; t->ldq = d; t->k = a->kv; t->v = lp_off(a->kv, d, dtype); t->ldkv = 2 * d;
    }
    t->mask = a->mask; t->mask_sb = a->mask_sb; t->mask_sq = a->mask_sq; t->drop = a->drop_attn;
    t->o = a->o; t->ldo = d; t->lse = a->lse;
}

extern "C" int mtn_sublayer_group_fwd(int dtype, int n_mha, const mtn_mha_args* mha, int n_ffn, const mtn_ffn_args* ffn, void* stream) {
    MTN_CHECK_ARG(dtype == MTN_F32 || dtype == MTN_BF16, "bad dtype");
    MTN_CHECK_ARG(n_mha >= 0 && n_mha <= MTN_SUBLAYER_MAX_GROUP && n_ffn >= 0 && n_ffn <= MTN_SUBLAYER_MAX_GROUP && n_mha + n_ffn > 0, "bad group size");
    for (int i = 0; i < n_mha; ++i) RUN(check_mha(&mha[i], false));
    for (int i = 0; i < n_ffn; ++i) RUN(check_ffn(&ffn[i], false));
    bool fused = fh_group_eligible(dtype, n_mha, mha, n_ffn, ffn) != 0;
    mtn_mha_args pre[MTN_SUBLAYER_MAX_GROUP];
    if (!fused && n_mha > 0 && dtype == MTN_BF16 && fh_is_enabled()) {
        bool any = false;
        for (int i = 0; i < n_mha; ++i) {
            pre[i] = mha[i];
            if (!mha[i].self_attn && !mha[i].kv_ready) { pre[i].kv_ready = 1; any = true; }
        }
        if (any && fh_group_eligible(dtype, n_mha, pre, n_ffn, ffn) != 0) {
            mtn_gemm_problem p[MTN_SUBLAYER_MAX_GROUP];
            int n = 0;
            for (int i = 0; i < n_mha; ++i) {
                const mtn_mha_args* a = &mha[i];
                if (a->self_attn || a->kv_ready) continue;
                const int d = a->d;
                p[n] = gemm_init(a->mem, d, lp_off(a->w_qkv, (long)d * d, dtype), d, a->B * a->m, 2 * d, d, 0, 0);
                p[n].bias = a->b_qkv + d; p[n].out_lp = a->kv; p[n].ldc = 2 * d; ++n;
            }
            RUN(mtn_gemm(dtype, n, p, stream));
            mha = pre;
            fused = true;
        }
    }
    ++g_fused_counts[fused ? 0 : 1];
    if (fused) RUN(fh_group_fwd_stage1(n_mha, mha, n_ffn, ffn, stream));
    if (!fused) {
        mtn_ln_fwd_desc L[2 * MTN_SUBLAYER_MAX_GROUP];
        int n = 0;
        for (int i = 0; i < n_mha; ++i) {
            const mtn_mha_args* a = &mha[i];
            memset(&L[n], 0, sizeof(L[n]));
            L[n].rows = a->B * a->a; L[n].d = a->d; L[n].eps = a->ln_eps; L[n].x = a->x; L[n].a2 = a->ln_a; L[n].b2 = a->ln_b;
            L[n].y_lp = a->xn; L[n].mean = a->mean; L[n].rstd = a->rstd; ++n;
        }
        for (int i = 0; i < n_ffn; ++i) {
            const mtn_ffn_args* a = &ffn[i];
            memset(&L[n], 0, sizeof(L[n]));
            L[n].rows = a->rows; L[n].d = a->d; L[n].eps = a->ln_eps; L[n].x = a->x; L[n].a2 = a->ln_a; L[n].b2 = a->ln_b;
            L[n].y_lp = a->xn; L[n].mean = a->mean; L[n].rstd = a->rstd; ++n;
        }
        RUN(mtn_layernorm_fwd_group(dtype, n, L, stream));
    }
    if (!fused) {
        mtn_gemm_problem p[3 * MTN_SUBLAYER_MAX_GROUP];
        int n = 0;
        for (int i = 0; i < n_mha; ++i) {
            const mtn_mha_args* a = &mha[i];
            const int d = a->d, rows = a->B * a->a;
            if (a->self_attn) {
                p[n] = gemm_init(a->xn, d, a->w_qkv, d, rows, 3 * d, d, 0, 0);
                p[n].bias = a->b_qkv; p[n].out_lp = a->qkv; p[n].ldc = 3 * d; ++n;
            } else {
                p[n] = gemm_init(a->xn, d, a->w_qkv, d, rows, d, d, 0, 0);
                p[n].bias = a->b_qkv; p[n].out_lp = a->qkv; p[n].ldc = d; ++n;
                if (!a->kv_ready) {
                    p[n] = gemm_init(a->mem, d, lp_off(a->w_qkv, (long)d * d, dtype), d, a->B * a->m, 2 * d, d, 0, 0);
                    p[n].bias = a->b_qkv + d; p[n].out_lp = a->kv; p[n].ldc = 2 * d; ++n;
                }
            }
        }
        for (int i = 0; i < n_ffn; ++i) {
            const mtn_ffn_args* a = &ffn[i];
            p[n] = gemm_init(a->xn, a->d, a->w1, a->d, a->rows, a->d_ff, a->d, 0, 0);
            p[n].bias = a->b1; p[n].relu = 1; p[n].drop = a->drop_hidden; p[n].out_lp = a->hid; p[n].ldc = a->d_ff; ++n;
        }
        RUN(mtn_gemm(dtype, n, p, stream));
    }
    if (n_mha && !fused) {
        mtn_attn_args t[MTN_SUBLAYER_MAX_GROUP];
        for (int i = 0; i < n_mha; ++i) attn_args_of(&mha[i], dtype, &t[i]);
        RUN(mtn_attention_fwd_group(dtype, n_mha, t, stream));
    }
    {
        mtn_gemm_problem p[2 * MTN_SUBLAYER_MAX_GROUP];
        int n = 0;
        for (int i = 0; i < n_mha; ++i) {
            const mtn_mha_args* a = &mha[i];
            const int d = a->d, rows = a->B * a->a;
            p[n] = gemm_init(a->o, d, a->w_o, d, rows, d, d, 0, 0);
            p[n].bias = a->b_o; p[n].drop = a->drop_out; p[n].residual = a->x; p[n].ldr = d; p[n].out_f32 = a->y; p[n].ldc = d;
            ++n;
        }
        for (int i = 0; i < n_ffn; ++i) {
            const mtn_ffn_args* a = &ffn[i];
            p[n] = gemm_init(a->hid, a->d_ff, a->w2, a->d_ff, a->rows, a->d, a->d_ff, 0, 0);
            p[n].bias = a->b2; p[n].drop = a->drop_out; p[n].residual = a->x; p[n].ldr = a->d; p[n].out_f32 = a->y; p[n].out_lp = a->y_lp; p[n].ldc = a->d;
            ++n;
        }
        RUN(mtn_gemm(dtype, n, p, stream));
    }
    return MTN_OK;
}

extern "C" int mtn_mha_sublayer_fwd(int dtype, const mtn_mha_args* a, void* stream) { return mtn_sublayer_group_fwd(dtype, 1, a, 0, nullptr, stream); }
extern "C" int mtn_ffn_sublayer_fwd(int dtype, const mtn_ffn_args* a, void* stream) { return mtn_sublayer_group_fwd(dtype, 0, nullptr, 1, a, stream); }

extern "C" long mtn_mha_bwd_ws_lp_elems(int B, int a, int m, int d, int self_attn) {
    long rows = (long)B * a, rows_m = (long)B * (self_attn ? a : m);
    return 2 * rows * d + (self_attn ? 3 * rows * d : rows * d + 2 * rows_m * d);
}
extern "C" long mtn_mha_bwd_ws_f32_floats(int B, int a, int m, int d) {
    long rows = (long)B * a;
    const long kvacc = a > 32 ? 2L * B * (m > a ? m : a) * d : 0;
    return rows * d + mtn_layernorm_bwd_partial_floats((int)rows, d) + kvacc + rows * 2 * LN_PART_HEADS;
}
extern "C" long mtn_ffn_bwd_ws_f32_floats(int rows, int d, int d_ff) {
    return (long)rows * d + mtn_layernorm_bwd_partial_floats(rows, d) + (long)rows * 2 * ((d_ff + 63) / 64);
}

struct MhaWs { void *dyl, *dO, *dqkv, *dkv; float *dxn, *ln_partial, *kv_acc, *ln_part; };
static MhaWs mha_ws(const mtn_mha_args* a, int dtype) {
    const long rows = (long)a->B * a->a, d = a->d;
    MhaWs w;
    w.dyl = a->dyl_ready ? (void*)a->dyl_ready : a->ws_lp;
    w.dO = lp_off(a->ws_lp, rows * d, dtype);
    w.dqkv = lp_off(a->ws_lp, 2 * rows * d, dtype);
    w.dkv = lp_off(w.dqkv, rows * d, dtype);
    w.dxn = a->ws_f32;
    w.ln_partial = a->ws_f32 + rows * d;
    w.kv_acc = a->a > 32 ? w.ln_partial + mtn_layernorm_bwd_partial_floats((int)rows, (int)d) : nullptr;
    const long rows_kv = (long)a->B * (a->m > a->a ? a->m : a->a);
    w.ln_part = w.ln_partial + mtn_layernorm_bwd_partial_floats((int)rows, (int)d) + (a->a > 32 ? 2L * rows_kv * d : 0);
    return w;
}
struct FfnWs { void *dyl, *dh; float *dxn, *ln_partial, *ln_part; };
static FfnWs ffn_ws(const mtn_ffn_args* a, int dtype) {
    FfnWs w;
    w.dyl = a->dyl_ready ? (void*)a->dyl_ready : a->ws_lp;
    w.dh = lp_off(a->ws_lp, (long)a->rows * a->d, dtype);
    w.dxn = a->ws_f32;
    w.ln_partial = a->ws_f32 + (long)a->rows * a->d;
    w.ln_part = w.ln_partial + mtn_layernorm_bwd_partial_floats(a->rows, a->d);
    return w;
}

extern "C" int mtn_sublayer_group_bwd(int dtype, int n_mha, const mtn_mha_args* mha, int n_ffn, const mtn_ffn_args* ffn, void* stream) {
    MTN_CHECK_ARG(dtype == MTN_F32 || dtype == MTN_BF16, "bad dtype");
    MTN_CHECK_ARG(n_mha >= 0 && n_mha <= MTN_SUBLAYER_MAX_GROUP && n_ffn >= 0 && n_ffn <= MTN_SUBLAYER_MAX_GROUP && n_mha + n_ffn > 0, "bad group size");
    for (int i = 0; i < n_mha; ++i) RUN(check_mha(&mha[i], true));
    for (int i = 0; i < n_ffn; ++i) RUN(check_ffn(&ffn[i], true));
    {
        mtn_cast_desc c[2 * MTN_SUBLAYER_MAX_GROUP];
        int n = 0;
        for (int i = 0; i < n_mha; ++i)
            if (!mha[i].dyl_ready) c[n++] = mtn_cast_desc{(long)mha[i].B * mha[i].a * mha[i].d, mha[i].dy, mha_ws(&mha[i], dtype).dyl, mha[i].drop_out};
        for (int i = 0; i < n_ffn; ++i)
            if (!ffn[i].dyl_ready) c[n++] = mtn_cast_desc{(long)ffn[i].rows * ffn[i].d, ffn[i].dy, ffn_ws(&ffn[i], dtype).dyl, ffn[i].drop_out};
        if (n) RUN(mtn_cast_group(dtype, n, c, stream));
    }
    const bool epi_on = dtype == MTN_BF16 && !(MTN_ENV("MTN_LN_EPI") && MTN_ENV("MTN_LN_EPI")[0] == '0');
    bool epi_m[MTN_SUBLAYER_MAX_GROUP], epi_f[MTN_SUBLAYER_MAX_GROUP];
    for (int i = 0; i < n_mha; ++i) epi_m[i] = epi_on && mha[i].ln_fold && mha[i].d == 512 && mha[i].h == LN_PART_HEADS;
    for (int i = 0; i < n_ffn; ++i) epi_f[i] = epi_on && ffn[i].ln_fold && ffn[i].d_ff % 64 == 0 && ffn[i].d % 16 == 0 && ffn[i].d <= 512;
// ... 181 lines not shown
```

### mtn_amd/lib.py

```python
from __future__ import annotations

import ctypes as C
import os

import torch

_HERE = os.path.dirname(os.path.abspath(__file__))
LIB_PATH = os.path.join(_HERE, "libmtn_hip.so")

MTN_F32, MTN_BF16 = 0, 1


class Dropout(C.Structure):
    _fields_ = [("p", C.c_float), ("salt", C.c_uint32), ("seed", C.c_void_p)]


class AdamFuse(C.Structure):
    _fields_ = [("p", C.c_void_p), ("m", C.c_void_p), ("v", C.c_void_p), ("p_lp", C.c_void_p), ("p_lpT", C.c_void_p),
                ("ldT", C.c_int), ("write_grad", C.c_int), ("state", C.c_void_p), ("grad_scale", C.c_void_p),
                ("beta1", C.c_float), ("beta2", C.c_float), ("eps", C.c_float)]


class LnEpilogue(C.Structure):
    _fields_ = [("mode", C.c_int), ("fold", C.c_void_p), ("gate_inv_scale", C.c_float), ("part", C.c_void_p), ("np", C.c_int),
# ... 62 lines not shown
                ("V", C.c_int), ("ldz", C.c_int), ("pad", C.c_int), ("smoothing", C.c_float),
                ("logits", C.c_void_p), ("lse", C.c_void_p), ("rowloss", C.c_void_p),
                ("gloss", C.c_void_p), ("dlogits", C.c_void_p), ("ldd", C.c_int)]


class TransposeDesc(C.Structure):
    _fields_ = [("off", C.c_long), ("rows", C.c_int), ("cols", C.c_int), ("tile_start", C.c_int), ("reserved", C.c_int), ("dst_off", C.c_long)]


class LnFwdDesc(C.Structure):
    _fields_ = [("rows", C.c_int), ("d", C.c_int), ("eps", C.c_float), ("x", C.c_void_p), ("a2", C.c_void_p), ("b2", C.c_void_p),
                ("y_f32", C.c_void_p), ("y_lp", C.c_void_p), ("mean", C.c_void_p), ("rstd", C.c_void_p),
                ("tokens", C.c_void_p), ("lut", C.c_void_p), ("emb_scale", C.c_float), ("pe", C.c_void_p), ("seq_len", C.c_int),
                ("drop", Dropout), ("x_out", C.c_void_p), ("no_ln", C.c_int)]


class EmbedBwdDesc(C.Structure):
    _fields_ = [("rows", C.c_int), ("d", C.c_int), ("tokens", C.c_void_p), ("dx", C.c_void_p), ("emb_scale", C.c_float),
                ("drop", Dropout), ("dlut", C.c_void_p), ("lut_rows", C.c_int)]


class LnBwdDesc(C.Structure):
    _fields_ = [("rows", C.c_int), ("d", C.c_int), ("eps", C.c_float), ("x", C.c_void_p), ("a2", C.c_void_p), ("mean", C.c_void_p),
                ("rstd", C.c_void_p), ("g", C.c_void_p), ("dres", C.c_void_p), ("dx", C.c_void_p), ("partial", C.c_void_p),
                ("dx_lp", C.c_void_p), ("dx_lp_dtype", C.c_int), ("dx_lp_drop", Dropout)]


class CastDesc(C.Structure):
    _fields_ = [("n", C.c_long), ("src", C.c_void_p), ("dst", C.c_void_p), ("drop", Dropout), ("gate", C.c_void_p)]


class TtLnUnit(C.Structure):
    _fields_ = [("partial", C.c_void_p), ("nparts", C.c_int), ("d", C.c_int), ("a_off", C.c_long), ("b_off", C.c_long)]


class TtAux(C.Structure):
    _fields_ = [("p", C.c_void_p), ("g", C.c_void_p), ("m", C.c_void_p), ("v", C.c_void_p), ("lp", C.c_void_p), ("n_flat", C.c_long),
                ("n_ln", C.c_int), ("ln", C.POINTER(TtLnUnit)), ("n_chunks", C.c_int), ("chunk_off", C.POINTER(C.c_long)),
                ("chunk_len", C.POINTER(C.c_int)), ("bias_adam", C.c_int), ("state", C.c_void_p), ("grad_scale", C.c_void_p),
                ("beta1", C.c_float), ("beta2", C.c_float), ("eps", C.c_float)]


class DecodeStage(C.Structure):
    _fields_ = [("kind", C.c_int), ("N", C.c_int), ("K", C.c_int), ("w", C.c_void_p), ("bias", C.c_void_p), ("ln_a", C.c_void_p),
                ("ln_b", C.c_void_p), ("ln_eps", C.c_float), ("kv", C.c_void_p), ("m", C.c_int), ("mask", C.c_void_p),
                ("mask_stride", C.c_long), ("cache", C.c_void_p)]


class DecodeArgs(C.Structure):
    _fields_ = [("W", C.c_int), ("d", C.c_int), ("h", C.c_int), ("L", C.c_int), ("n_stages", C.c_int), ("d_ff", C.c_int), ("xg", C.c_void_p), ("qg", C.c_void_p),
                ("og", C.c_void_p), ("hg", C.c_void_p), ("out_lp", C.c_void_p), ("tokens", C.c_void_p), ("lut", C.c_void_p),
                ("emb_scale", C.c_float), ("pe", C.c_void_p), ("pos", C.c_void_p), ("anc", C.c_void_p), ("sync", C.c_void_p), ("dbg", C.c_void_p), ("max_m", C.c_int)]


DEC_EMBED, DEC_SELF_QKV, DEC_SELF_ATT, DEC_OUT, DEC_CROSS, DEC_FFN1, DEC_FFN2, DEC_FINAL = range(8)


class BeamArgs(C.Structure):
    _fields_ = [("dialogues", C.c_int), ("width", C.c_int), ("L", C.c_int), ("k_top", C.c_int), ("k", C.c_int), ("beam", C.c_int), ("unk", C.c_int),
                ("eos", C.c_int), ("pad", C.c_int), ("min_len", C.c_int), ("penalty", C.c_double), ("top", C.c_void_p), ("tokens", C.c_void_p),
                ("pos", C.c_void_p), ("anc", C.c_void_p), ("lp", C.c_void_p), ("n_live", C.c_void_p), ("step", C.c_void_p), ("flags", C.c_void_p),
                ("log_parent", C.c_void_p), ("log_tok", C.c_void_p), ("log_score", C.c_void_p), ("log_done", C.c_void_p), ("log_n_old", C.c_void_p),
                ("log_n_new", C.c_void_p)]


class DiverseArgs(C.Structure):
    _fields_ = [("beam", BeamArgs), ("groups", C.c_int), ("diversity", C.c_float)]


class SampleArgs(C.Structure):
    _fields_ = [("rows", C.c_int), ("V", C.c_int), ("ldx", C.c_long), ("logp", C.c_void_p), ("temperature", C.c_float), ("top_k", C.c_int),
                ("top_p", C.c_float), ("n_banned", C.c_int), ("banned", C.c_int * 4), ("eos", C.c_int), ("min_len", C.c_int),
                ("seed", C.c_void_p), ("key", C.c_void_p), ("step", C.c_void_p), ("L", C.c_int), ("log_tok", C.c_void_p),
                ("log_logp", C.c_void_p), ("log_u", C.c_void_p), ("tokens", C.c_void_p), ("pos", C.c_void_p), ("anc", C.c_void_p)]


class ScoreArgs(C.Structure):
    _fields_ = [("n_seq", C.c_int), ("L", C.c_int), ("V", C.c_int), ("pad", C.c_int), ("ldz", C.c_long), ("logits", C.c_void_p),
                ("target", C.c_void_p), ("tok_logp", C.c_void_p), ("tok_rank", C.c_void_p), ("seq_logp", C.c_void_p), ("seq_len", C.c_void_p)]


class ConstrainArgs(C.Structure):
    _fields_ = [("rows", C.c_int), ("V", C.c_int), ("ldx", C.c_long), ("ldo", C.c_long), ("logp", C.c_void_p), ("out", C.c_void_p),
                ("ngram", C.c_int), ("theta", C.c_float), ("L", C.c_int), ("hist", C.c_void_p), ("ldh", C.c_long), ("hist_len", C.c_void_p),
                ("log_tok", C.c_void_p), ("log_parent", C.c_void_p), ("step", C.c_void_p), ("width", C.c_int), ("rows_per_step", C.c_int)]


class EnsembleArgs(C.Structure):
    _fields_ = [("rows", C.c_int), ("V", C.c_int), ("M", C.c_int), ("mode", C.c_int), ("x", C.c_void_p * 8), ("ld", C.c_long * 8),
                ("w", C.c_float * 8), ("out", C.c_void_p), ("ldo", C.c_long)]


class LnFinalizeDesc(C.Structure):
    _fields_ = [("partial", C.c_void_p), ("nparts", C.c_int), ("d", C.c_int), ("da2", C.c_void_p), ("db2", C.c_void_p)]


GEMM_MAX_GROUP = 16


_P = C.c_void_p
class AssembleTokensDesc(C.Structure):
    _fields_ = [("flat", C.c_void_p), ("start", C.c_void_p), ("len", C.c_void_p), ("ids", C.c_void_p), ("B", C.c_int), ("L", C.c_int),
                ("pad", C.c_int64), ("out", C.c_void_p), ("mask", C.c_void_p), ("std_mask", C.c_void_p), ("n_nonpad", C.c_void_p),
                ("row_len", C.c_void_p)]


class AssembleFeaturesDesc(C.Structure):
    _fields_ = [("flat", C.c_void_p), ("start", C.c_void_p), ("len", C.c_void_p), ("ids", C.c_void_p), ("B", C.c_int), ("V", C.c_int),
                ("F", C.c_int), ("skip", C.c_int), ("out", C.c_void_p), ("mask", C.c_void_p)]


class CensusLaunch(C.Structure):
    _fields_ = [("dtype", C.c_int), ("count", C.c_int), ("variant", C.c_int), ("workgroups", C.c_int),
                ("flops", C.c_double), ("bytes", C.c_double), ("M", C.c_int * 4), ("N", C.c_int * 4), ("K", C.c_int * 4)]


SYMBOLS = {
    "mtn_assemble_tokens": (C.c_int, [C.c_int, C.POINTER(AssembleTokensDesc), _P]),
    "mtn_assemble_features": (C.c_int, [C.c_int, C.POINTER(AssembleFeaturesDesc), _P]),
    "mtn_topk_rows": (C.c_int, [_P, C.c_int, C.c_int, C.c_long, C.c_int, C.c_int, _P, _P]),
    "mtn_log_softmax_rows": (C.c_int, [_P, C.c_int, C.c_int, C.c_long, _P, C.c_long, _P]),
    "mtn_census_begin": (C.c_int, []),
    "mtn_census_end": (C.c_int, []),
    "mtn_census_info": (C.c_int, [C.c_int, C.POINTER(CensusLaunch)]),
    "mtn_census_replay": (C.c_int, [C.c_int, C.c_int, _P]),
    "mtn_census_variant_name": (C.c_char_p, [C.c_int]),
    "mtn_measure_mfma_peak": (C.c_int, [C.c_int, _P, _P, C.POINTER(C.c_double)]),
    "mtn_measure_mfma_peak_shapes": (C.c_int, [C.c_int, _P, _P, C.POINTER(C.c_double), C.POINTER(C.c_double)]),
    "mtn_measure_hbm_peak": (C.c_int, [_P, _P, C.c_long, _P, C.POINTER(C.c_double)]),
    "mtn_reload_env": (C.c_int, []),
    "mtn_stream_create_cu_masked": (C.c_int, [C.c_int, C.c_int, C.POINTER(C.c_void_p)]),
    "mtn_stream_destroy": (C.c_int, [_P]),
    "mtn_last_error": (C.c_char_p, []),
    "mtn_version": (C.c_int, []),
    "mtn_gemm": (C.c_int, [C.c_int, C.c_int, C.POINTER(GemmProblem), _P]),
    "mtn_gemm_tt_table": (C.c_int, [C.c_int, C.c_int, C.POINTER(GemmProblem), _P]),
    "mtn_decode_step": (C.c_int, [C.POINTER(DecodeArgs), _P, C.c_int, _P]),
    "mtn_beam_advance": (C.c_int, [C.POINTER(BeamArgs), _P]),
    "mtn_diverse_advance": (C.c_int, [C.POINTER(DiverseArgs), _P]),
    "mtn_sample_rows": (C.c_int, [C.POINTER(SampleArgs), _P]),
    "mtn_score_rows": (C.c_int, [C.POINTER(ScoreArgs), _P]),
    "mtn_constrain_rows": (C.c_int, [C.POINTER(ConstrainArgs), _P]),
    "mtn_ensemble_rows": (C.c_int, [C.POINTER(EnsembleArgs), _P]),
    "mtn_debug_hold_cus": (C.c_int, [C.c_int, C.c_int, C.c_int, _P]),
    "mtn_gemm_tt_table_aux": (C.c_int, [C.c_int, C.c_int, C.POINTER(GemmProblem), C.POINTER(TtAux), _P]),
    "mtn_layernorm_fwd": (C.c_int, [C.c_int, C.c_int, C.c_int, C.c_float, _P, _P, _P, _P, _P, _P, _P, _P]),
    "mtn_layernorm_fwd_group": (C.c_int, [C.c_int, C.c_int, C.POINTER(LnFwdDesc), _P]),
    "mtn_embed_bwd_group": (C.c_int, [C.c_int, C.POINTER(EmbedBwdDesc), _P]),
    "mtn_layernorm_bwd_group": (C.c_int, [C.c_int, C.POINTER(LnBwdDesc), _P]),
    "mtn_attention_fwd_group": (C.c_int, [C.c_int, C.c_int, C.POINTER(AttnArgs), _P]),
    "mtn_attention_bwd_group": (C.c_int, [C.c_int, C.c_int, C.POINTER(AttnArgs), _P]),
    "mtn_cast_group": (C.c_int, [C.c_int, C.c_int, C.POINTER(CastDesc), _P]),
    "mtn_fused_enable": (C.c_int, [C.c_int]),
    "mtn_fused_counters": (C.c_int, [C.POINTER(C.c_long)]),
    "mtn_ln_epilogue_groups": (C.c_long, []),
    "mtn_ln_fold": (C.c_int, [C.c_int, _P, _P, C.c_int, C.c_int, _P]),
    "mtn_sublayer_group_fwd": (C.c_int, [C.c_int, C.c_int, C.POINTER(MhaArgs), C.c_int, C.POINTER(FfnArgs), _P]),
    "mtn_sublayer_group_bwd": (C.c_int, [C.c_int, C.c_int, C.POINTER(MhaArgs), C.c_int, C.POINTER(FfnArgs), _P]),
    "mtn_layernorm_bwd_partial_floats": (C.c_long, [C.c_int, C.c_int]),
    "mtn_layernorm_bwd_nparts": (C.c_int, [C.c_int]),
    "mtn_layernorm_bwd_finalize": (C.c_int, [C.c_int, C.POINTER(LnFinalizeDesc), _P]),
    "mtn_mha_param_grad_work": (C.c_int, [C.c_int, C.POINTER(MhaArgs), C.POINTER(GemmProblem), C.POINTER(LnFinalizeDesc)]),
    "mtn_ffn_param_grad_work": (C.c_int, [C.c_int, C.POINTER(FfnArgs), C.POINTER(GemmProblem), C.POINTER(LnFinalizeDesc)]),
    "mtn_layernorm_bwd": (C.c_int, [C.c_int, C.c_int, C.c_float, _P, _P, _P, _P, _P, _P, _P, _P, _P, _P, _P]),
    "mtn_attention_fwd": (C.c_int, [C.c_int, C.POINTER(AttnArgs), _P]),
    "mtn_attention_bwd": (C.c_int, [C.c_int, C.POINTER(AttnArgs), _P]),
    "mtn_mha_sublayer_fwd": (C.c_int, [C.c_int, C.POINTER(MhaArgs), _P]),
    "mtn_mha_sublayer_bwd": (C.c_int, [C.c_int, C.POINTER(MhaArgs), _P]),
    "mtn_mha_bwd_ws_lp_elems": (C.c_long, [C.c_int, C.c_int, C.c_int, C.c_int, C.c_int]),
    "mtn_mha_bwd_ws_f32_floats": (C.c_long, [C.c_int, C.c_int, C.c_int, C.c_int]),
    "mtn_ffn_sublayer_fwd": (C.c_int, [C.c_int, C.POINTER(FfnArgs), _P]),
    "mtn_ffn_sublayer_bwd": (C.c_int, [C.c_int, C.POINTER(FfnArgs), _P]),
    "mtn_ffn_bwd_ws_f32_floats": (C.c_long, [C.c_int, C.c_int, C.c_int]),
    "mtn_cast_f32_to_lp": (C.c_int, [C.c_int, C.c_long, _P, _P, _P]),
    "mtn_dropout_bwd_to_lp": (C.c_int, [C.c_int, C.c_long, _P, Dropout, _P, _P]),
    "mtn_losshead_fwd": (C.c_int, [C.POINTER(LossHeadArgs), _P]),
    "mtn_losshead_bwd": (C.c_int, [C.c_int, C.POINTER(LossHeadArgs), _P]),
    "mtn_transpose_group": (C.c_int, [C.c_int, _P, _P, _P, C.c_int, C.c_int, _P]),
    "mtn_noam_tick": (C.c_int, [_P, C.c_float, C.c_int, C.c_int, C.c_float, C.c_float, _P]),
    "mtn_adam_step": (C.c_int, [C.c_int, C.c_long, _P, _P, _P, _P, _P, _P, _P, C.c_float, C.c_float, C.c_float, _P]),
    "mtn_adam_step_chunks": (C.c_int, [C.c_int, C.c_int, _P, _P, _P, _P, _P, _P, _P, _P, _P, C.c_float, C.c_float, C.c_float, _P]),
}

_lib = None


class MtnHipError(RuntimeError):
    pass


def load():
    global _lib
    if _lib is not None:
        return _lib
    path = os.environ.get("MTN_HIP_LIB", LIB_PATH)
    if not os.path.exists(path):
        raise MtnHipError(f"{path} is missing: build it with `python -m mtn_amd.build` "
                          "(hipcc --offload-arch=gfx950).  mtn_amd has no CPU/PyTorch fallback.")
    lib = C.CDLL(path)
    for name, (res, args) in SYMBOLS.items():
        fn = getattr(lib, name)
        fn.restype, fn.argtypes = res, args
    _lib = lib
    return lib


def fused_counters():
    out = (C.c_long * 4)()
    check(load().mtn_fused_counters(out))
    return tuple(int(v) for v in out)


def reload_env():
    if _lib is not None:
        _lib.mtn_reload_env()


def check(rc: int):
    if rc != 0:
        raise MtnHipError(f"libmtn_hip error {rc}: {load().mtn_last_error().decode()}")


def stream_ptr() -> int:
    return torch.cuda.current_stream().cuda_stream


def ptr(t) -> int:
    return 0 if t is None else t.data_ptr()


def dtype_code(dt: torch.dtype) -> int:
    if dt == torch.float32:
        return MTN_F32
    if dt == torch.bfloat16:
        return MTN_BF16
    raise ValueError(f"unsupported compute dtype {dt}")
```

### mtn_amd/mtn.py

```python
from __future__ import annotations

import math
import os
from typing import List, Optional, Sequence

import torch
import torch.nn as nn
import torch.nn.functional as F

from . import lib as L
from . import ops

ATTN_DROPOUT_DEFAULT = 0.1


_HANDOFF = True


class LayerNorm(nn.Module):

    def __init__(self, features: int, eps: float = 1e-6):
        super().__init__()
        self.a_2 = nn.Parameter(torch.ones(features))
        self.b_2 = nn.Parameter(torch.zeros(features))
# ... 624 lines not shown
        self._tdescs_all = list(tdescs)
        self._rest_cache = {}
        for n, layer in enumerate(self.decoder.layers):
            object.__setattr__(layer, "_owner", self)
            object.__setattr__(layer, "_next_layer", self.decoder.layers[n + 1] if n + 1 < len(self.decoder.layers) else None)
            layer._layer_index = n
            for k, s in enumerate(layer.sublayer):
                object.__setattr__(s, "_owner", self)
                s.salt = n * 64 + k + 1
        self._build_ln_fold()

    def _build_ln_fold(self):
        self._ln_fold_buf = self._ln_fold_table = None
        self._ln_fold_stale = True
        for layer in self.decoder.layers:
            for sc in layer.sublayer:
                sc._ln_fold = None
        dev = self._flat.device
        if dev.type != "cuda" or self.compute_dtype != torch.bfloat16 or self.auto_encoder_ft not in ("caption", "summary", "query"):
            return
        pairs = []
        for layer in self.decoder.layers:
            sl, nF = layer.sublayer, len(layer.auto_encoder_vid_attn)
            if len(sl) != 5 + 4 * nF:
                continue
            text = [layer.self_attn, layer.his_attn] + ([layer.src_attn, layer.cap_attn] if self.auto_encoder_ft in ("caption", "summary")
                                                        else [layer.cap_attn, layer.src_attn])
            sched = [(sl[j], m, j == 0) for j, m in enumerate(text)]
            for i in range(nF):
                sched += [(sl[4 + 4 * i], layer.auto_encoder_self_attn[i], True), (sl[5 + 4 * i], layer.auto_encoder_vid_attn[i], False),
                          (sl[6 + 4 * i], layer.auto_encoder_feed_forward[i], None), (sl[7 + 4 * i], layer.auto_encoder_attn[i], False)]
            sched.append((sl[4 + 4 * nF], layer.feed_forward, None))
            for sc, mod, self_attn in sched:
                f = mod._fused
                if f is None or sc.norm._grads is None:
                    continue
                if isinstance(mod, MultiHeadedAttention):
                    d = f["w_o"].size(0)
                    K = 3 * d if self_attn else d
                    pairs.append((sc, mod, f["w_qkv_lp"][:K], f["b_qkv"][:K]))
                else:
                    pairs.append((sc, mod, f["w1_lp"], f["b1"]))
        if not pairs:
            return
        d = pairs[0][2].size(1)
        if any(w.size(1) != d for _, _, w, _ in pairs) or d % 8 != 0 or d > 2048:
            return
        total = sum(2 * w.size(0) for _, _, w, _ in pairs)
        buf = torch.zeros(total, device=dev, dtype=torch.float32)
        descs = (L.LnFoldDesc * len(pairs))()
        block_desc, off, blocks = [], 0, 0
        for i, (sc, mod, w, b) in enumerate(pairs):
            K = w.size(0)
            view = buf[off:off + 2 * K]
            descs[i].w, descs[i].bias, descs[i].a2, descs[i].b2 = w.data_ptr(), b.data_ptr(), sc.norm.a_2.data_ptr(), sc.norm.b_2.data_ptr()
            descs[i].out, descs[i].K, descs[i].block_start = view.data_ptr(), K, blocks
            nb = (K + 63) // 64
            block_desc += [i] * nb
            blocks += nb
            off += 2 * K
            sc._ln_fold = (id(mod), view)
        table = torch.frombuffer(bytearray(bytes(descs)), dtype=torch.uint8).to(dev)
        self._ln_fold_buf = buf
        self._ln_fold_table = (table, torch.tensor(block_desc, dtype=torch.int32).to(dev), blocks, d)

    def fold_layer_norms(self):
        t = self._ln_fold_table
        if t is not None:
            L.check(L.load().mtn_ln_fold(L.MTN_BF16, t[0].data_ptr(), t[1].data_ptr(), t[2], t[3], L.stream_ptr()))
        self._ln_fold_stale = False

    def state_dict(self, *a, **kw):
        if self._master_sync is not None:
            self._master_sync()
        return super().state_dict(*a, **kw)

    def _apply(self, fn, *a, **kw):
        super()._apply(fn, *a, **kw)
        self._flat = None
        return self

    def set_compute_dtype(self, dtype):
        self.compute_dtype = {"bf16": torch.bfloat16, "fp32": torch.float32}.get(dtype, dtype)
        self._flat = None
        return self

    def prepare(self):
        if self._flat is None:
            self._flatten()
        ver = sum(p._version for p in self._flat_params)
        if self._flat_lp is not self._flat and ver != self._flat_version and self._flat_version != -1 and self._master_sync is not None:
            self._master_sync()
        if self._flat_lp is not self._flat and ver != self._flat_version:
            L.check(L.load().mtn_cast_f32_to_lp(L.dtype_code(self.compute_dtype), self._flat.numel(), self._flat.data_ptr(),
                                                self._flat_lp.data_ptr(), L.stream_ptr()))
            self._flat_version = ver
            self._ln_fold_stale = True
            self.refresh_transposed()
        elif self._flat_lp is self._flat and ver != self._flat_version:
            self._flat_version = ver
            self.refresh_transposed()
        return self

    def _tdesc_table(self, descs):
        if not descs:
            return None
        arr = (L.TransposeDesc * len(descs))()
        tiles = 0
        for i, (o, r, c) in enumerate(descs):
            arr[i].off, arr[i].dst_off, arr[i].rows, arr[i].cols, arr[i].tile_start = o, self._t_off[o], r, c, tiles
            tiles += ((r + 63) // 64) * ((c + 63) // 64)
        raw = torch.frombuffer(bytearray(bytes(arr)), dtype=torch.uint8).to(self._flat.device)
        return (raw, len(descs), tiles)

    def rest_tables(self, covered: frozenset):
        hit = self._rest_cache.get(covered)
        if hit is None:
            dev = self._flat.device
            total = self._flat.numel()
            done = [t for t in self._fusable if t[0] in covered]
            offs_c, lens_c, cur = [], [], 0
            for o, r, c in done + [(total, 0, 0)]:
                assert o % 4 == 0 and (r * c) % 4 == 0
                while cur < o:
                    n = min(4096, o - cur)
                    offs_c.append(cur); lens_c.append(n); cur += n
                cur = o + r * c
            chunks = (torch.tensor(offs_c, dtype=torch.int64).to(dev), torch.tensor(lens_c, dtype=torch.int32).to(dev), len(offs_c))
            dset = set(done)
            hit = (chunks, self._tdesc_table([t for t in self._tdescs_all if t not in dset]))
            self._rest_cache[covered] = hit
        return hit

    def refresh_transposed(self, table=None):
        table = self._tdesc if table is None else table
        if table is None:
            return
        raw, n, tiles = table
        L.check(L.load().mtn_transpose_group(L.dtype_code(self.compute_dtype), self._flat_lp.data_ptr(), self._flat_lpT.data_ptr(),
                                             raw.data_ptr(), n, tiles, L.stream_ptr()))

    def flat_buffers(self):
        self.prepare()
        return self._flat, self._flat_lp, self._flat_grad

    def zero_glue_grads(self):
        self._flat_grad[: self._glue_numel].zero_()

    def advance_dropout_seed(self):
        if self._seed is not None:
            self._seed.add_(0x9E3779B97F4A7C15 & 0x7FFFFFFFFFFFFFFF)

    def forward(self, b):
        q, v, cp, hs, ae = self.encode(b.query, b.query_mask, b.his, b.his_mask, b.cap, b.cap_mask, b.fts, b.fts_mask)
        return self.decode(v, hs, cp, q, b.fts_mask, b.his_mask, b.cap_mask, b.query_mask, b.trg, b.trg_mask, ae)

    def vid_encode(self, video_features, video_features_mask=None, encoded_query=None):
        return [self.vid_encoder[i](ft) for i, ft in enumerate(video_features)]

    def _embed_fused(self, items):
        luts, streams = [], []
        for k, (tok, emb, ln) in enumerate(items):
            lut = emb[0].lut.weight
            idx = next((j for j, t in enumerate(luts) if t is lut), None)
            if idx is None:
                luts.append(lut); idx = len(luts) - 1
            lninfo = None
            if ln is not None:
                ga, gb = ln._grads if ln._grads is not None else (None, None)
                lninfo = (ln.a_2, ln.b_2, ln.eps, ga, gb)
            streams.append(dict(tokens=tok, lut=idx, pe=emb[1].pe[0], scale=math.sqrt(emb[0].d_model),
                                p=emb[1].dropout.p if self.training else 0.0, salt=900000 + self._embed_calls * 16 + k, ln=lninfo))
        self._embed_calls += 1
        spec = dict(streams=streams, lp_dtype=self.compute_dtype, seed=self._seed if self.training else None, queue=self._queue)
        outs = ops.EmbedNormFn.apply(spec, *luts)
        for y, y_lp, (_, _, ln) in zip(outs, spec["_lp_out"], items):
            if ln is not None:
                y._mtn_lp = y_lp if y_lp is not None else y.detach()
        return list(outs)

    def _features_fused(self, vid):
        streams, weights = [], []
        off = {id(p): o for p, o in zip(self._flat_params, self._flat_offsets)}
        for i, x in enumerate(vid):
            lin, pos = self.vid_encoder[i][0], self.vid_encoder[i][2]
            ln = self.query_encoder.norm[1 + i]
            o = off[id(lin.weight)]
            w_lp = self._flat_lp[o:o + lin.weight.numel()].view(lin.weight.shape)
            streams.append(dict(x=x, w_lp=w_lp, bias=lin.bias, grad_w=lin.weight.grad, grad_b=lin.bias.grad, pe=pos.pe[0],
                                p=pos.dropout.p if self.training else 0.0, salt=910000 + i,
                                ln=(ln.a_2, ln.b_2, ln.eps, ln._grads[0], ln._grads[1])))
            weights.append(lin.weight)
        spec = dict(streams=streams, lp_dtype=self.compute_dtype, seed=self._seed if self.training else None, queue=self._queue)
        outs = ops.FeatureEncodeFn.apply(spec, *weights)
        for y, y_lp in zip(outs, spec["_lp_out"]):
            y._mtn_lp = y_lp if y_lp is not None else y.detach()
        return list(outs)

    def _fused_embed_ok(self, tokens):
        return self.fused_embed and tokens.is_cuda and self._flat is not None and all(n._grads is not None for n in self.query_encoder.norm)

    def encode(self, query, query_mask, his=None, his_mask=None, cap=None, cap_mask=None, vid=None, vid_mask=None):
        self.prepare()
        self.fold_layer_norms()
        if self.training:
            self.advance_dropout_seed()
        self._embed_calls = 0
        if self._fused_embed_ok(query):
            nF = len(vid)
            norm = self.query_encoder.norm
            items = [(query, self.query_embed, norm[0]), (cap, self.query_embed, norm[nF + 1]), (his, self.query_embed, norm[nF + 2])]
            if self.diff_encoder:
                ft = cap if self.auto_encoder_ft in ("caption", "summary") else query
                for i in range(nF):
                    emb = self.auto_encoder_embed[i] if self.auto_encoder_embed is not None else self.query_embed
                    items.append((ft, emb, norm[nF + 3 + i]))
            outs = self._embed_fused(items)
            if all(v.size(-1) % 8 == 0 for v in vid):
                vids = self._features_fused(vid)
            else:
                vids = [self.query_encoder._apply_norm(1 + i, v) for i, v in enumerate(self.vid_encode(vid, vid_mask))]
            return [outs[0], vids, outs[1], outs[2], outs[3:] if self.diff_encoder else None]
        streams = [self.query_embed(query), self.vid_encode(vid, vid_mask), self.query_embed(cap), self.query_embed(his)]
        if not self.diff_encoder:
            out = self.query_encoder(*streams)
            out.append(None)
            return out
        ft = cap if self.auto_encoder_ft in ("caption", "summary") else query
        if self.auto_encoder_embed is not None:
            ae = [self.auto_encoder_embed[i](ft) for i in range(len(vid))]
        else:
            ae = [self.query_embed(ft) for _ in range(len(vid))]
        return self.query_encoder(*streams, ae)

    def hoist_memory_kv(self, cap_memory, his_memory, q_memory, vid_fts, outs=None):
        if not (self.hoist_kv and self.lockstep and self._flat is not None and q_memory.is_cuda):
            return None
        nF = len(vid_fts)
        items, targets = [], []
        for layer in self.decoder.layers:
            if layer._forward_hooks_on_sublayers() or nF + 1 > 4:
                continue
            text, chains, _, _ = layer._plan(cap_memory, None, his_memory, None, q_memory, None, None, vid_fts, [None] * nF,
                                             self.auto_encoder_ft)
            for sc, mod, mem, _ in list(text[1:]) + [chains[i][1] for i in range(nF)]:
                mem_lp = getattr(mem, "_mtn_lp", None)
                f = mod.fused()
                if mem_lp is None or mem_lp.dtype != self.compute_dtype or f.get("w_qkv_lp") is None:
                    continue
                items.append((mem_lp, f["w_qkv_lp"], f["b_qkv"]))
                targets.append(sc)
        kvs = ops.project_memories(items, self.compute_dtype, outs)
        self._kv_targets = list(zip(targets, kvs))
        self.attach_memory_kv(self._kv_targets)
        return kvs

    @staticmethod
    def attach_memory_kv(pairs):
        for sc, kv in pairs:
            object.__setattr__(sc, "_kv_ready", kv)

    def clear_memory_kv(self):
        for layer in self.decoder.layers:
            for sc in layer.sublayer:
                if getattr(sc, "_kv_ready", None) is not None:
                    object.__setattr__(sc, "_kv_ready", None)

    def embed_target(self, tgt):
        if self._fused_embed_ok(tgt):
            return self._embed_fused([(tgt, self.tgt_embed, None)])[0]
        return self.tgt_embed(tgt)

    def forward_segmented(self, b):
        q, v, cp, hs, ae = self.encode(b.query, b.query_mask, b.his, b.his_mask, b.cap, b.cap_mask, b.fts, b.fts_mask)
        x = self.embed_target(b.trg)
        enc_out = [q, cp, hs, x] + list(v) + (list(ae) if ae is not None else [])

        def cut(t):
            u = t.detach().requires_grad_()
            for attr in ("_mtn_lp", "_mtn_next"):
                if hasattr(t, attr):
                    setattr(u, attr, getattr(t, attr))
            return u

        enc_leaf = [cut(t) for t in enc_out]
        nF = len(v)
        q_l, cp_l, hs_l, x_l = enc_leaf[:4]
        v_l = enc_leaf[4:4 + nF]
        ae_l = enc_leaf[4 + nF:] if ae is not None else None
        ops.prepare_masks(b.trg_mask, b.his_mask, b.cap_mask, b.query_mask, b.fts_mask)
        self.hoist_memory_kv(cp_l, hs_l, q_l, v_l)
        layers = []
        x_in, ae_in = x_l, ae_l
        for layer in self.decoder.layers:
            x_out, ae_out = layer(x_in, cp_l, b.cap_mask, hs_l, b.his_mask, q_l, b.query_mask, b.trg_mask, v_l, b.fts_mask,
                                  ae_in, self.auto_encoder_ft)
            ins = [x_in] + (list(ae_in) if isinstance(ae_in, (list, tuple)) else [])
            layers.append((ins, [x_out] + list(ae_out)))
            x_in, ae_in = cut(x_out), [cut(a) for a in ae_out]
        self.clear_memory_kv()
        top_in = [x_in] + ae_in
        if x_in.is_cuda and len(ae_in) == len(self.decoder.ae_norm):
            ys = ops.layer_norm_group([x_in] + list(ae_in), [self.decoder.norm] + list(self.decoder.ae_norm))
            out, ae_fin = ys[0], ys[1:]
        else:
            out = self.decoder.norm(x_in)
            ae_fin = [self.decoder.ae_norm[i](a) for i, a in enumerate(ae_in)]
        return dict(enc_out=enc_out, enc_leaf=enc_leaf, layers=layers, top_in=top_in, out=out, ae_out=ae_fin)

    def decode(self, encoded_vid_features, his_memory, cap_memory, query_memory, vid_features_mask, his_mask, cap_mask,
               query_mask, tgt, tgt_mask, auto_encoded_ft):
        self.prepare()
        x0 = self.embed_target(tgt)
        self.hoist_memory_kv(cap_memory, his_memory, query_memory, encoded_vid_features)
        try:
            return self._decode_layers(encoded_vid_features, vid_features_mask, x0, his_memory, his_mask, cap_memory, cap_mask,
                                       query_memory, query_mask, tgt_mask, auto_encoded_ft)
        finally:
            self.clear_memory_kv()

    def _decode_layers(self, encoded_vid_features, vid_features_mask, x0, his_memory, his_mask, cap_memory, cap_mask, query_memory,
                       query_mask, tgt_mask, auto_encoded_ft):
        return self.decoder(encoded_vid_features, vid_features_mask, x0, his_memory, his_mask, cap_memory,
                            cap_mask, query_memory, query_mask, tgt_mask, auto_encoded_ft, self.auto_encoder_ft)


def make_model(src_vocab, tgt_vocab, N=6, d_model=512, d_ff=2048, h=8, dropout=0.1, separate_his_embed=False,
               separate_cap_embed=False, ft_sizes=None, diff_encoder=False, diff_embed=False, diff_gen=False,
               auto_encoder_ft=None, auto_encoder_attn=False, compute_dtype="bf16", attn_dropout=ATTN_DROPOUT_DEFAULT):
    ft_sizes = list(ft_sizes or [])
    F_ = len(ft_sizes)
    attn = lambda: MultiHeadedAttention(h, d_model, attn_dropout)
    ff = lambda: PositionwiseFeedForward(d_model, d_ff, dropout)
    pos = lambda: PositionalEncoding(d_model, dropout)
    embed = lambda vocab: nn.Sequential(Embeddings(d_model, vocab), pos())
    query_embed, tgt_embed = embed(src_vocab), embed(tgt_vocab)
    his_embed = embed(src_vocab) if separate_his_embed else None
    cap_embed = embed(src_vocab) if separate_cap_embed else None
    auto_encoder_embed = nn.ModuleList([embed(src_vocab) for _ in ft_sizes]) if diff_embed else None
    query_encoder = Encoder(d_model, nb_layers=3 + (2 * F_ if diff_encoder else F_))
    vid_encoder = nn.ModuleList([nn.Sequential(nn.Linear(fs, d_model), nn.ReLU(), pos()) for fs in ft_sizes])
    generator = Generator(d_model, tgt_vocab)
    auto_encoder_generator = nn.ModuleList([Generator(d_model, tgt_vocab) for _ in ft_sizes]) if diff_gen else None

    def make_layer():
        return DecoderLayer(d_model, attn(), attn(), attn(), attn(),
                            nn.ModuleList([attn() for _ in ft_sizes]), nn.ModuleList([attn() for _ in ft_sizes]),
                            nn.ModuleList([attn() for _ in ft_sizes]), ff(), nn.ModuleList([ff() for _ in ft_sizes]), dropout)

    decoder = Decoder(make_layer, N, ft_sizes)
    cd = {"bf16": torch.bfloat16, "fp32": torch.float32}.get(compute_dtype, compute_dtype)
    model = EncoderDecoder(query_encoder=query_encoder, his_encoder=None, cap_encoder=None, vid_encoder=vid_encoder,
                           decoder=decoder, query_embed=query_embed, his_embed=his_embed, cap_embed=cap_embed,
                           tgt_embed=tgt_embed, generator=generator, auto_encoder_generator=auto_encoder_generator,
                           auto_encoder_embed=auto_encoder_embed, diff_encoder=diff_encoder, auto_encoder_ft=auto_encoder_ft,
                           compute_dtype=cd)
    for p in model.parameters():
        if p.dim() > 1:
            nn.init.xavier_uniform_(p)
    return model
```

### mtn_amd/ops.py

```python
from __future__ import annotations

import ctypes as C
import os
from dataclasses import dataclass
from typing import Optional

import torch

from . import lib as L


_XACC = True
_HANDOFF_MEM = True


def _drop(p: float, salt: int, seed: Optional[torch.Tensor]) -> L.Dropout:
    if p > 0.0 and seed is not None:
        return L.Dropout(float(p), int(salt) & 0xFFFFFFFF, seed.data_ptr())
    return L.Dropout(0.0, 0, None)


def _require_cuda(*ts):
    for t in ts:
        if t is not None and not t.is_cuda:
# ... 849 lines not shown
    x = x.contiguous()
    out = torch.empty(x.size(0), 2 * k + 1, device=x.device, dtype=torch.float32)
    L.check(L.load().mtn_topk_rows(x.data_ptr(), x.size(0), x.size(1), x.stride(0), k, extra_col, out.data_ptr(), L.stream_ptr()))
    return out


def sample_args(logp, seed, keys, step, log, *, temperature=1.0, top_k=0, top_p=1.0, banned=(), eos=-1, min_len=0, rows=None,
                tokens=None, pos=None, anc=None):
    _require_cuda(logp, seed, keys, step, *log)
    if logp.dtype != torch.float32 or logp.stride(-1) != 1 or seed.dtype != torch.int64 or keys.dtype != torch.int64 or step.dtype != torch.int32:
        raise ValueError("sample_rows: logp fp32 with unit column stride, seed / keys int64, step int32")
    n, V = logp.shape
    rows = n if rows is None else int(rows)
    if rows != n and n != 1:
        raise ValueError("sample_rows: rows differs from logp's only when one distribution serves every row")
    banned = [int(b) for b in banned]
    lt, ll, lu = log
    if len(banned) > 4 or keys.numel() != rows or step.numel() != rows or seed.numel() != 1:
        raise ValueError("sample_rows: at most 4 banned tokens; one key and one step per row, one seed")
    if not (lt.dtype == torch.int32 and ll.dtype == lu.dtype == torch.float32 and lt.shape == ll.shape == lu.shape and lt.dim() == 2
            and lt.size(1) == rows and all(t.is_contiguous() for t in (lt, ll, lu, keys, step))):
        raise ValueError("sample_rows: the log is (int32, fp32, fp32), each contiguous (L, rows)")
    a = L.SampleArgs()
    a.rows, a.V, a.ldx, a.logp = rows, V, (0 if rows != n else (V if n == 1 else logp.stride(0))), logp.data_ptr()
    a.temperature, a.top_k, a.top_p = float(temperature), int(top_k), float(top_p)
    a.n_banned, a.eos, a.min_len = len(banned), int(eos), int(min_len)
    for i, b in enumerate(banned):
        a.banned[i] = b
    a.seed, a.key, a.step, a.L = seed.data_ptr(), keys.data_ptr(), step.data_ptr(), lt.size(0)
    a.log_tok, a.log_logp, a.log_u = lt.data_ptr(), ll.data_ptr(), lu.data_ptr()
    as_ptr = lambda t: None if t is None else (t if isinstance(t, int) else t.data_ptr())
    a.tokens, a.pos, a.anc = as_ptr(tokens), as_ptr(pos), as_ptr(anc)
    return a


def sample_rows(logp, seed, keys, step, log=None, max_len=1, **kw):
    rows = kw.get("rows") or logp.size(0)
    if log is None:
        log = (torch.zeros(max_len, rows, device=logp.device, dtype=torch.int32), torch.zeros(max_len, rows, device=logp.device),
               torch.zeros(max_len, rows, device=logp.device))
    a = sample_args(logp, seed, keys, step, log, **kw)
    L.check(L.load().mtn_sample_rows(C.byref(a), L.stream_ptr()))
    return log


def constrain_rows(logp, ngram=0, theta=1.0, *, hist=None, hist_len=None, log_tok=None, log_parent=None, step=None, width=1,
                   rows_per_step=1, log_len=None, out=None):
    _require_cuda(logp)
    if logp.dim() != 2 or logp.dtype != torch.float32 or (logp.size(1) > 1 and logp.stride(1) != 1) or logp.stride(0) < logp.size(1):
        raise ValueError("constrain_rows: logp fp32 (rows, V) with unit column stride")
    rows, V = logp.shape
    ngram, theta = int(ngram), float(theta)
    if not 0 <= ngram <= 8 or not theta >= 1.0:
        raise ValueError("constrain_rows: 0 <= ngram <= 8, theta >= 1")
    if out is None:
        out = logp
    else:
        _require_cuda(out)
        if out.shape != logp.shape or out.dtype != torch.float32 or (V > 1 and out.stride(1) != 1) or out.stride(0) < V:
            raise ValueError("constrain_rows: out is fp32 of logp's shape with unit column stride")
        span = lambda t: (t.data_ptr(), t.data_ptr() + ((rows - 1) * t.stride(0) + V) * 4)
        (lo, hi), (olo, ohi) = span(logp), span(out)
        ld, off = logp.stride(0), abs(olo - lo) // 4
        apart = out.stride(0) == ld and (off == 0 or (off % ld >= V and ld - off % ld >= V))
        if lo < ohi and olo < hi and not apart:
            raise ValueError("constrain_rows: out overlaps logp without being logp (in place: leave out None or pass logp itself)")
    a = L.ConstrainArgs()
    a.rows, a.V, a.ldx, a.ldo, a.logp, a.out = rows, V, logp.stride(0), out.stride(0), logp.data_ptr(), out.data_ptr()
    a.ngram, a.theta = ngram, theta
    if hist is not None:
        if hist_len is None:
            raise ValueError("constrain_rows: hist needs hist_len, int32 (rows,)")
        _require_cuda(hist, hist_len)
        if (hist.dim() != 2 or hist.dtype != torch.int32 or hist.size(0) != rows or hist.size(1) < 1 or hist.stride(1) != 1 or hist_len.dtype != torch.int32
                or hist_len.numel() != rows or not hist_len.is_contiguous() or log_tok is not None):
            raise ValueError("constrain_rows: hist int32 (rows, L) with unit column stride and hist_len int32 (rows,); one history source")
        a.L = hist.size(1) if log_len is None else int(log_len)
        if a.L > hist.size(1):
            raise ValueError("constrain_rows: log_len exceeds the history table's width")
        a.hist, a.ldh, a.hist_len = hist.data_ptr(), max(hist.stride(0), hist.size(1)), hist_len.data_ptr()
    else:
        if log_tok is None or step is None:
            raise ValueError("constrain_rows: a history source is required (hist + hist_len, or log_tok + step)")
        width, rows_per_step = int(width), int(rows_per_step)
        if not 1 <= width <= 16 or rows % width or rows_per_step < 1:
            raise ValueError("constrain_rows: 1 <= width <= 16, rows a multiple of width, rows_per_step >= 1")
        for t in (log_tok, log_parent):
            if t is not None and not isinstance(t, int):
                _require_cuda(t)
                if t.dtype != torch.int32 or t.dim() != 2 or t.size(1) != rows or not t.is_contiguous() or (log_len is not None and t.size(0) < int(log_len)):
                    raise ValueError("constrain_rows: the step log is int32, contiguous (L, rows)")
        if not isinstance(step, int):
            _require_cuda(step)
            if step.dtype != torch.int32 or not step.is_contiguous() or step.numel() * rows_per_step < rows:
                raise ValueError("constrain_rows: step int32, one counter per rows_per_step rows")
        if log_len is None:
            if isinstance(log_tok, int):
                raise ValueError("constrain_rows: log_len is required with a raw log pointer")
            log_len = log_tok.size(0)
        as_ptr = lambda t: None if t is None else (t if isinstance(t, int) else t.data_ptr())
        a.L, a.log_tok, a.log_parent, a.step, a.width, a.rows_per_step = int(log_len), as_ptr(log_tok), as_ptr(log_parent), as_ptr(step), width, rows_per_step
    L.check(L.load().mtn_constrain_rows(C.byref(a), L.stream_ptr()))
    return out


ENSEMBLE_MODES = {"prob": 0, "logprob": 1}
ENSEMBLE_MAX = 8


def ensemble_weights(n, weights=None):
    import numpy as np
    w = np.full(n, 1.0, dtype=np.float64) if weights is None else np.asarray([float(v) for v in weights], dtype=np.float64)
    if w.shape != (n,) or not np.isfinite(w).all() or (w < 0).any() or not w.sum() > 0:
        raise ValueError("ensemble: one finite weight >= 0 per member, not all of them 0")
    return w / w.sum()


def ensemble_rows(xs, weights=None, mode="prob", out=None):
    xs = list(xs)
    if not 1 <= len(xs) <= ENSEMBLE_MAX:
        raise ValueError("ensemble_rows: 1 to 8 members")
    if mode not in ENSEMBLE_MODES:
        raise ValueError("ensemble_rows: mode is 'prob' or 'logprob'")
    w = ensemble_weights(len(xs), weights)
    _require_cuda(*xs)
    x0 = xs[0]
    for x in xs:
        if (x.dim() != 2 or x.dtype != torch.float32 or x.shape != x0.shape or x.device != x0.device or x.numel() == 0
                or (x.size(1) > 1 and x.stride(1) != 1) or (x.size(0) > 1 and x.stride(0) < x.size(1))):
            raise ValueError("ensemble_rows: every member is fp32 (rows, V), non-empty, of one shape and device, with unit column stride")
    rows, V = x0.shape
    if V >= 1 << 24:
        raise ValueError("ensemble_rows: V < 2^24")
    if out is None:
        out = torch.empty(rows, V, device=x0.device, dtype=torch.float32)
    else:
        _require_cuda(out)
        if out.shape != x0.shape or out.dtype != torch.float32 or out.device != x0.device or (V > 1 and out.stride(1) != 1) or (rows > 1 and out.stride(0) < V):
            raise ValueError("ensemble_rows: out is fp32 of the members' shape with unit column stride")
        span = lambda t: (t.data_ptr(), t.data_ptr() + ((rows - 1) * t.stride(0) + V) * 4)
        olo, ohi = span(out)
        for x in xs:
            lo, hi = span(x)
            if lo < ohi and olo < hi:
                raise ValueError("ensemble_rows: out overlaps a member")
    a = L.EnsembleArgs()
    a.rows, a.V, a.M, a.mode, a.out, a.ldo = rows, V, len(xs), ENSEMBLE_MODES[mode], out.data_ptr(), max(out.stride(0), V)
    for m, x in enumerate(xs):
        a.x[m], a.ld[m], a.w[m] = x.data_ptr(), max(x.stride(0), V), float(w[m])
    L.check(L.load().mtn_ensemble_rows(C.byref(a), L.stream_ptr()))
    return out


def project_memories(items, lp_dtype, outs=None):
    if not items:
        return []
    code = L.dtype_code(lp_dtype)
    reuse, outs, probs = outs, [], []
    for k, (mem_lp, w, b) in enumerate(items):
        Bm = mem_lp.size(0) * mem_lp.size(1)
        d = mem_lp.size(-1)
        kv = reuse[k] if reuse is not None else torch.empty(Bm, 2 * d, device=mem_lp.device, dtype=lp_dtype)
        p = L.GemmProblem()
        p.A, p.B, p.lda, p.ldb, p.M, p.N, p.K = mem_lp.data_ptr(), w.data_ptr() + d * d * w.element_size(), d, d, Bm, 2 * d, d
        p.bias, p.gate_scale, p.out_lp, p.ldc = b.data_ptr() + d * b.element_size(), 1.0, kv.data_ptr(), 2 * d
        outs.append(kv)
        probs.append(p)
    for i in range(0, len(probs), L.GEMM_MAX_GROUP):
        gemm(code, probs[i:i + L.GEMM_MAX_GROUP])
    return outs


class EmbedNormFn(torch.autograd.Function):

    @staticmethod
    def forward(ctx, spec, *luts):
        lib = L.load()
        streams = spec["streams"]
        lp = spec["lp_dtype"]
        code = L.dtype_code(lp) if lp is not None else L.MTN_F32
        dev = luts[0].device
        descs = (L.LnFwdDesc * len(streams))()
        outs, saved = [], []
        for i, st in enumerate(streams):
            tok = st["tokens"].contiguous()
            B, Ls = tok.shape
            d = luts[st["lut"]].size(1)
            rows = B * Ls
            y = torch.empty(B, Ls, d, device=dev, dtype=torch.float32)
            D = descs[i]
            D.rows, D.d, D.tokens, D.lut, D.emb_scale = rows, d, tok.data_ptr(), luts[st["lut"]].data_ptr(), float(st["scale"])
            D.pe, D.seq_len = st["pe"].data_ptr(), Ls
            D.drop = _drop(st["p"], st["salt"], spec["seed"])
            sv = dict(tok=tok, rows=rows, d=d)
            if st["ln"] is not None:
                a2, b2, eps = st["ln"][0], st["ln"][1], st["ln"][2]
                x_save = torch.empty(rows, d, device=dev, dtype=torch.float32)
                mean = torch.empty(rows, device=dev, dtype=torch.float32)
                rstd = torch.empty_like(mean)
                y_lp = torch.empty(B, Ls, d, device=dev, dtype=lp) if (lp is not None and lp != torch.float32) else None
                D.eps, D.a2, D.b2, D.x_out, D.mean, D.rstd = eps, a2.data_ptr(), b2.data_ptr(), x_save.data_ptr(), mean.data_ptr(), rstd.data_ptr()
                D.y_f32, D.y_lp, D.no_ln = y.data_ptr(), L.ptr(y_lp), 0
                sv.update(x=x_save, mean=mean, rstd=rstd, a2=a2, y_lp=y_lp)
            else:
                D.y_f32, D.no_ln = y.data_ptr(), 1
            outs.append(y)
            saved.append(sv)
        L.check(lib.mtn_layernorm_fwd_group(code, len(streams), descs, L.stream_ptr()))
        ctx.spec, ctx.saved_streams, ctx.luts = spec, saved, luts
        ctx.lp_copies = [sv.get("y_lp") for sv in saved]
        spec["_lp_out"] = ctx.lp_copies
        return tuple(outs)

    @staticmethod
    def backward(ctx, *dys):
        lib = L.load()
        spec, saved, luts = ctx.spec, ctx.saved_streams, ctx.luts
        streams = spec["streams"]
        dev = luts[0].device
        queue = spec.get("queue")
        ln_descs, ln_final, emb = [], [], (L.EmbedBwdDesc * len(streams))()
        keep = []
        ret = [None] * len(luts)
        dluts = []
        for j, lut in enumerate(luts):
            if lut.grad is not None:
                dluts.append(lut.grad)
            else:
                g = torch.zeros_like(lut)
                dluts.append(g)
                ret[j] = g
        for i, (st, sv, dy) in enumerate(zip(streams, saved, dys)):
            dy = dy.contiguous() if dy is not None else torch.zeros(sv["rows"], sv["d"], device=dev)
            dx = dy
            if st["ln"] is not None:
                dx = torch.empty(sv["rows"], sv["d"], device=dev, dtype=torch.float32)
                partial = torch.empty(lib.mtn_layernorm_bwd_partial_floats(sv["rows"], sv["d"]), device=dev, dtype=torch.float32)
                ln_descs.append(L.LnBwdDesc(sv["rows"], sv["d"], st["ln"][2], sv["x"].data_ptr(), sv["a2"].data_ptr(), sv["mean"].data_ptr(),
                                            sv["rstd"].data_ptr(), dy.data_ptr(), None, dx.data_ptr(), partial.data_ptr()))
                ga, gb = st["ln"][3], st["ln"][4]
                ln_final.append((L.LnFinalizeDesc(partial.data_ptr(), lib.mtn_layernorm_bwd_nparts(sv["rows"]), sv["d"], ga.data_ptr(), gb.data_ptr()), partial))
            keep += [dy, dx]
            E = emb[i]
            E.rows, E.d, E.tokens, E.dx, E.emb_scale = sv["rows"], sv["d"], sv["tok"].data_ptr(), dx.data_ptr(), float(st["scale"])
            E.drop = _drop(st["p"], st["salt"], spec["seed"])
            E.dlut = dluts[st["lut"]].data_ptr()
            E.lut_rows = luts[st["lut"]].size(0)
        if ln_descs:
            arr = (L.LnBwdDesc * len(ln_descs))(*ln_descs)
            L.check(lib.mtn_layernorm_bwd_group(len(ln_descs), arr, L.stream_ptr()))
            if queue is not None:
                for desc, partial in ln_final:
                    queue.add(queue.dtype, [], desc, [partial])
            else:
                farr = (L.LnFinalizeDesc * len(ln_final))(*[f[0] for f in ln_final])
                L.check(lib.mtn_layernorm_bwd_finalize(len(ln_final), farr, L.stream_ptr()))
        if queue is not None and all(r is None for r in ret):
            queue.add_embed([emb[i] for i in range(len(streams))], keep)
        else:
            L.check(lib.mtn_embed_bwd_group(len(streams), emb, L.stream_ptr()))
        return (None, *ret)


class FeatureEncodeFn(torch.autograd.Function):

    @staticmethod
    def forward(ctx, spec, *weights):
        lib = L.load()
        streams, lp = spec["streams"], spec["lp_dtype"]
        code = L.dtype_code(lp)
        dev = weights[0].device
        n = len(streams)
        casts = (L.CastDesc * n)()
        probs, lns, saved, outs = [], (L.LnFwdDesc * n)(), [], []
        for i, st in enumerate(streams):
            x = st["x"].contiguous()
            B, V, F = x.shape
            d = st["w_lp"].size(0)
            rows = B * V
            x_lp = torch.empty(rows, F, device=dev, dtype=lp)
            casts[i].n, casts[i].src, casts[i].dst = rows * F, x.data_ptr(), x_lp.data_ptr()
            h = torch.empty(rows, d, device=dev, dtype=torch.float32)
            p = L.GemmProblem()
            p.A, p.B, p.lda, p.ldb, p.M, p.N, p.K = x_lp.data_ptr(), st["w_lp"].data_ptr(), F, F, rows, d, F
            p.bias, p.relu, p.gate_scale, p.out_f32, p.ldc = st["bias"].data_ptr(), 1, 1.0, h.data_ptr(), d
            probs.append(p)
            a2, b2, eps = st["ln"][0], st["ln"][1], st["ln"][2]
            y = torch.empty(B, V, d, device=dev, dtype=torch.float32)
            y_lp = torch.empty(B, V, d, device=dev, dtype=lp) if lp != torch.float32 else None
            xs = torch.empty(rows, d, device=dev, dtype=torch.float32)
            mean = torch.empty(rows, device=dev, dtype=torch.float32)
            rstd = torch.empty_like(mean)
            D = lns[i]
            D.rows, D.d, D.eps, D.x, D.a2, D.b2 = rows, d, eps, h.data_ptr(), a2.data_ptr(), b2.data_ptr()
            D.pe, D.seq_len, D.drop = st["pe"].data_ptr(), V, _drop(st["p"], st["salt"], spec["seed"])
            D.x_out, D.mean, D.rstd, D.y_f32, D.y_lp = xs.data_ptr(), mean.data_ptr(), rstd.data_ptr(), y.data_ptr(), L.ptr(y_lp)
            outs.append(y)
            saved.append(dict(x_lp=x_lp, h=h, xs=xs, mean=mean, rstd=rstd, rows=rows, d=d, F=F, y_lp=y_lp, a2=a2))
        if lp != torch.float32:
            L.check(lib.mtn_cast_group(code, n, casts, L.stream_ptr()))
        else:
            for sv, st in zip(saved, streams):
                sv["x_lp"].copy_(st["x"].reshape(sv["rows"], sv["F"]))
        gemm(code, probs)
        L.check(lib.mtn_layernorm_fwd_group(code, n, lns, L.stream_ptr()))
        ctx.spec, ctx.saved_streams, ctx.n_w = spec, saved, len(weights)
        spec["_lp_out"] = [sv["y_lp"] for sv in saved]
        return tuple(outs)

    @staticmethod
    def backward(ctx, *dys):
        lib = L.load()
        spec, saved = ctx.spec, ctx.saved_streams
        streams, lp = spec["streams"], spec["lp_dtype"]
        code = L.dtype_code(lp)
        queue = spec.get("queue")
        n = len(streams)
        dev = saved[0]["h"].device
        lnb = (L.LnBwdDesc * n)()
        casts = (L.CastDesc * n)()
        probs, finals, keep = [], [], []
        for i, (st, sv, dy) in enumerate(zip(streams, saved, dys)):
            rows, d, F = sv["rows"], sv["d"], sv["F"]
# ... 237 lines not shown
```

Baseline: 8969 samples/s.

## Defer memory K/V projection tiles as riders on idle CUs of fused-head kernels

The cross-attention K/V projections for decoder layers after the first are no longer launched up front. They are queued on the host, and their 128x256 GEMM tiles are appended as extra workgroups to later fused-head forward launches, filling CUs those launches leave idle. Any leftover tiles are flushed in a separate launch just before a sublayer reads that K/V, and at the end of forward. This aims to overlap the projection GEMMs with the attention kernels and save standalone launches, but it adds host-side bookkeeping with a mutex and larger kernel arguments, and under HIP graph capture it depends on the capture order being stable.

```diff
diff --git a/include/mtn_hip.h b/include/mtn_hip.h
--- a/include/mtn_hip.h
+++ b/include/mtn_hip.h
@@ -255,6 +255,10 @@
 #define MTN_SUBLAYER_MAX_GROUP 4
 int mtn_fused_enable(int on);
 int mtn_fused_counters(long* out4);
+int mtn_kv_project(int dtype, int count, const mtn_gemm_problem* problems , int n_now, void* stream);
+int mtn_riders_flush(void* stream);
+int mtn_riders_enabled(void);
+int mtn_rider_counters(long* out4);
 long mtn_ln_epilogue_groups(void);
 int mtn_sublayer_group_fwd(int dtype, int n_mha, const mtn_mha_args* mha, int n_ffn, const mtn_ffn_args* ffn, void* stream);
 int mtn_sublayer_group_bwd(int dtype, int n_mha, const mtn_mha_args* mha, int n_ffn, const mtn_ffn_args* ffn, void* stream);
diff --git a/mtn_amd/csrc/elementwise.hip b/mtn_amd/csrc/elementwise.hip
--- a/mtn_amd/csrc/elementwise.hip
+++ b/mtn_amd/csrc/elementwise.hip
@@ -11,7 +11,7 @@
     va_end(ap);
 }
 extern "C" const char* mtn_last_error(void) { return g_err; }
-extern "C" int mtn_version(void) { return 119; }
+extern "C" int mtn_version(void) { return 120; }
 
 #include <mutex>
 static int g_env_gen = 0;
diff --git a/mtn_amd/csrc/fused.hip b/mtn_amd/csrc/fused.hip
--- a/mtn_amd/csrc/fused.hip
+++ b/mtn_amd/csrc/fused.hip
@@ -1,4 +1,5 @@
 #include "fused_common.h"
+#include "gemm_k512_tile.h"
 
 struct FhMember {
     int kind;
@@ -39,7 +40,10 @@
 #endif
     int wg_start[FH_MAX_MEMBERS + 1];
     FhMember m[FH_MAX_MEMBERS];
+    int rider_base;
+    GkRider kv;
 };
+static_assert(sizeof(FhGroup) <= 4096, "FhGroup travels by value in the kernel arguments");
 
 struct FhLds { int gains, xn, xm, qi, ki, vi, mask, total; };
 __host__ __device__ inline FhLds fh_lds_map(int mt, bool raw, int key_rows, int pad_rows, int mask_bytes, int ffn_blocks = 0, bool late_v = false) {
@@ -564,6 +568,11 @@
     extern __shared__ __attribute__((aligned(16))) unsigned char smem[];
     FH_STAMP(0);
     FH_STAMP_CLK(10);
+    if ((int)blockIdx.x >= G.wg_start[FH_MAX_MEMBERS]) {
+        const int r = (int)blockIdx.x - G.rider_base;
+        if (r >= 0 && r < G.kv.units) gk_rider_unit(G.kv, r, smem);
+        return;
+    }
     int g = 0;
     while (g + 1 < G.count && (int)blockIdx.x >= G.wg_start[g + 1]) ++g;
     const FhMember& M = G.m[g];
@@ -754,10 +763,45 @@
     return MTN_OK;
 }
 
+static int fh_cu_count() {
+    static int cus[64];
+    int dev = 0;
+    if (hipGetDevice(&dev) != hipSuccess || dev < 0 || dev >= 64) return 0;
+    int n = __atomic_load_n(&cus[dev], __ATOMIC_RELAXED);
+    if (n == 0) {
+        if (hipDeviceGetAttribute(&n, hipDeviceAttributeMultiprocessorCount, dev) != hipSuccess || n < 1) n = -1;
+        __atomic_store_n(&cus[dev], n, __ATOMIC_RELAXED);
+    }
+    return n > 0 ? n : 0;
+}
+static bool fh_rider_ffn_hosts() {
+    const char* e = MTN_ENV("MTN_RIDER_FFN_HOSTS");
+    return e ? e[0] != '0' : true;
+}
+static int fh_rider_slots(const FhLaunch& P) {
+    if (!mtn_riders_enabled()) return 0;
+    if (P.np == 4 && !fh_rider_ffn_hosts()) return 0;
+    const int base = (P.wgs + 7) & ~7;
+    int slots = fh_cu_count() - base;
+    const char* cap = MTN_ENV("MTN_RIDER_MAX_SLOTS");
+    if (cap && atoi(cap) < slots) slots = atoi(cap);
+    return slots > 0 ? slots : 0;
+}
+
 int fh_group_fwd_stage1(int n_mha, const mtn_mha_args* mha, int n_ffn, const mtn_ffn_args* ffn, void* stream) {
     FhLaunch P;
     MTN_CHECK_ARG(fh_plan(n_mha, mha, n_ffn, ffn, P), "group outside the fused kernel's tiling");
     hipStream_t s = (hipStream_t)stream;
+    const int slots = fh_rider_slots(P);
+    if (slots > 0) {
+        gk_rider_take(slots, &P.G.kv);
+        if (P.G.kv.units > 0) {
+            P.G.rider_base = (P.wgs + 7) & ~7;
+            P.wgs = P.G.rider_base + P.G.kv.units;
+            if (P.lds < (size_t)GK_LDS) P.lds = GK_LDS;
+        }
+    }
+    static_assert(GK_LDS <= FH_LDS_MAX, "a rider tile's x image fits the launch's dynamic LDS limit");
     const int rc = P.np == 4 ? fh_launch<4>(P.G, P.wgs, P.lds, s) : (P.np == 3 ? fh_launch<3>(P.G, P.wgs, P.lds, s) : fh_launch<1>(P.G, P.wgs, P.lds, s));
     if (rc != MTN_OK) return rc;
     MTN_CHECK_LAUNCH();
diff --git a/mtn_amd/csrc/gemm.hip b/mtn_amd/csrc/gemm.hip
--- a/mtn_amd/csrc/gemm.hip
+++ b/mtn_amd/csrc/gemm.hip
@@ -2084,6 +2084,15 @@
     return MTN_OK;
 }
 
+void gemm_census_note_k512(int count, const mtn_gemm_problem* p, int tiles) {
+    if (!g_census_on) return;
+    CensusEntry e;
+    memset(&e, 0, sizeof(e));
+    e.dtype = MTN_BF16; e.count = count; e.variant = V_K512; e.tiles = tiles; e.table = -1;
+    for (int i = 0; i < count; ++i) e.p[i] = p[i];
+    g_census.push_back(e);
+}
+
 extern "C" int mtn_census_begin(void) { g_census.clear(); g_census_tables.clear(); g_census_on = true; return MTN_OK; }
 extern "C" int mtn_census_end(void) { g_census_on = false; return (int)g_census.size(); }
 extern "C" const char* mtn_census_variant_name(int variant) { return (variant >= 0 && variant < V_COUNT) ? g_variant_name[variant] : "?"; }
diff --git a/mtn_amd/csrc/gemm_k512.hip b/mtn_amd/csrc/gemm_k512.hip
--- a/mtn_amd/csrc/gemm_k512.hip
+++ b/mtn_amd/csrc/gemm_k512.hip
@@ -1,11 +1,5 @@
-#include "fused_common.h"
-
-static constexpr int GK_THREADS = 512;
-static constexpr int GK_K = 512;
-static constexpr int GK_LDS = 128 * FH_ROWB;
-static constexpr int GK_CPITCH = 272;
-
-struct GkProblem { const bf16_t* A; const bf16_t* B; const float* bias; bf16_t* out; int lda, ldb, ldc, M, N, tiles_m; };
+#include "gemm_k512_tile.h"
+
 struct GkGroup {
     int count;
     int tile_start[MTN_GEMM_MAX_GROUP + 1];
@@ -78,88 +72,11 @@
     }
 }
 
-static constexpr int GW_CPITCH = 528;
 __global__ __launch_bounds__(GK_THREADS) void gemm_k512w_kernel(const GkGroup G) {
     extern __shared__ __attribute__((aligned(16))) unsigned char smem[];
-    const int tid = threadIdx.x, lane = tid & 63, l15 = lane & 15, lg = lane >> 4;
-    const int wave = __builtin_amdgcn_readfirstlane(tid >> 6);
     int g = 0;
     while (g + 1 < G.count && (int)blockIdx.x >= G.tile_start[g + 1]) ++g;
-    const GkProblem& P = G.p[g];
-    const int t = (int)blockIdx.x - G.tile_start[g];
-    const int tn = t / P.tiles_m, tm = t - tn * P.tiles_m;
-    const int row0 = tm * 128, col0 = tn * 256;
-    const int R = (P.M - row0) < 128 ? (P.M - row0) : 128;
-    {
-        const unsigned ldab = (unsigned)P.lda * 2u;
-        const __amdgpu_buffer_rsrc_t rs = __builtin_amdgcn_make_buffer_rsrc((void*)(P.A + (size_t)row0 * P.lda), 0, (R - 1) * ldab + FH_ROWB, 0x00020000);
-        for (int r = wave; r < 128; r += 8) {
-            const unsigned vo = r < R ? (unsigned)r * ldab + (unsigned)((lane ^ (r & 15)) << 4) : 0x80000000u;
-            __builtin_amdgcn_raw_ptr_buffer_load_lds(rs, (fh_lds_void_t*)(smem + r * FH_ROWB), 16, vo, 0, 0, 0);
-        }
-    }
-    float4 bq[2];
-#pragma unroll
-    for (int cb = 0; cb < 2; ++cb) {
-        const int colq = col0 + 128 * cb + 16 * wave + 4 * lg;
-        bq[cb] = make_float4(0.f, 0.f, 0.f, 0.f);
-        if (P.bias && colq < P.N) bq[cb] = *(const float4*)(P.bias + colq);
-    }
-    __builtin_amdgcn_sched_barrier(0);
-    uint4 wf[2][16];
-    {
-        const bf16_t* wrow[2];
-#pragma unroll
-        for (int cb = 0; cb < 2; ++cb) {
-            int n = col0 + 128 * cb + 16 * wave + (lane >> 2);
-            n = n < P.N ? n : P.N - 1;
-            wrow[cb] = P.B + (size_t)n * P.ldb + (lane & 3) * 8;
-        }
-#pragma unroll
-        for (int s = 0; s < 16; ++s) { wf[0][s] = *(const uint4*)(wrow[0] + s * 32); wf[1][s] = *(const uint4*)(wrow[1] + s * 32); }
-    }
-    __builtin_amdgcn_sched_barrier(0);
-    __builtin_amdgcn_s_waitcnt(0x8F70);
-    __builtin_amdgcn_s_barrier();
-    f32x4_t acc[2][8];
-#pragma unroll
-    for (int cb = 0; cb < 2; ++cb)
-#pragma unroll
-        for (int mt = 0; mt < 8; ++mt) acc[cb][mt] = f32x4_t{0.f, 0.f, 0.f, 0.f};
-    const int src = (4 * l15 + lg) * 4;
-#pragma unroll
-    for (int s = 0; s < 16; ++s) {
-#pragma unroll
-        for (int cb = 0; cb < 2; ++cb) {
-            wf[cb][s].x = (unsigned)__builtin_amdgcn_ds_bpermute(src, (int)wf[cb][s].x);
-            wf[cb][s].y = (unsigned)__builtin_amdgcn_ds_bpermute(src, (int)wf[cb][s].y);
-            wf[cb][s].z = (unsigned)__builtin_amdgcn_ds_bpermute(src, (int)wf[cb][s].z);
-            wf[cb][s].w = (unsigned)__builtin_amdgcn_ds_bpermute(src, (int)wf[cb][s].w);
-        }
-#pragma unroll
-        for (int mt = 0; mt < 8; ++mt) {
-            const uint4 xf = fh_xfrag(smem, mt * 16 + l15, s * 4 + lg);
-            mma16<bf16_t>(acc[0][mt], wf[0][s], xf);
-            mma16<bf16_t>(acc[1][mt], wf[1][s], xf);
-        }
-    }
-    __syncthreads();
-#pragma unroll
-    for (int cb = 0; cb < 2; ++cb)
-#pragma unroll
-        for (int mt = 0; mt < 8; ++mt) {
-            const int r = mt * 16 + l15;
-            *(uint2*)(smem + r * GW_CPITCH + (128 * cb + 16 * wave + 4 * lg) * 2) =
-                make_uint2(fh_pack2(acc[cb][mt][0] + bq[cb].x, acc[cb][mt][1] + bq[cb].y), fh_pack2(acc[cb][mt][2] + bq[cb].z, acc[cb][mt][3] + bq[cb].w));
-        }
-    __syncthreads();
-#pragma unroll
-    for (int ps = 0; ps < 8; ++ps) {
-        const int r = ps * 16 + (tid >> 5), c = tid & 31;
-        const int col = col0 + c * 8;
-        if (r < R && col < P.N)
-            *(uint4*)(P.out + (size_t)(row0 + r) * P.ldc + col) = *(const uint4*)(smem + r * GW_CPITCH + c * 16);
-    }
+    gk_wide_tile(G.p[g], (int)blockIdx.x - G.tile_start[g], smem);
 }
 
 static constexpr int GP_ROWS = 64;
@@ -338,24 +255,40 @@
     }
 }
 
+static bool gk_fill(const mtn_gemm_problem& q, GkProblem& P) {
+    if (q.a_trans || q.b_trans || q.K != GK_K || q.relu || q.gate || q.residual || q.out_f32 || q.rowsum_out || q.adam || !q.out_lp) return false;
+    if (q.drop.p > 0.f && q.drop.seed) return false;
+    if (q.M < 1 || q.N < 8 || (q.N & 7) || (q.lda & 7) || (q.ldb & 7) || (q.ldc & 7) || q.lda < GK_K || q.ldb < GK_K) return false;
+    if ((long)q.M * q.lda * 2 >= (1L << 31)) return false;
+    if (((size_t)q.A | (size_t)q.B | (size_t)q.out_lp) & 15) return false;
+    if (q.bias && ((size_t)q.bias & 15)) return false;
+    P.A = (const bf16_t*)q.A; P.B = (const bf16_t*)q.B; P.bias = q.bias; P.out = (bf16_t*)q.out_lp;
+    P.lda = q.lda; P.ldb = q.ldb; P.ldc = q.ldc; P.M = q.M; P.N = q.N; P.tiles_m = (q.M + 127) / 128;
+    return true;
+}
+static long gk_persist_units(int count, const mtn_gemm_problem* p) {
+    long units = 0;
+    for (int i = 0; i < count; ++i) units += (long)((p[i].M + GP_ROWS - 1) / GP_ROWS) * ((p[i].N + 127) / 128);
+    return units;
+}
+static bool gk_wide_attr() {
+    static bool attr_w = false;
+    if (!attr_w) {
+        if (hipFuncSetAttribute((const void*)gemm_k512w_kernel, hipFuncAttributeMaxDynamicSharedMemorySize, GK_LDS) != hipSuccess) return false;
+        attr_w = true;
+    }
+    return true;
+}
+
 int gemm_k512_try(int count, const mtn_gemm_problem* p, int min_tiles, hipStream_t s, int* tiles_out) {
     if (count < 1 || count > MTN_GEMM_MAX_GROUP) return 0;
     GkGroup G;
     memset(&G, 0, sizeof(G));
     int tiles = 0;
     for (int i = 0; i < count; ++i) {
-        const mtn_gemm_problem& q = p[i];
-        if (q.a_trans || q.b_trans || q.K != GK_K || q.relu || q.gate || q.residual || q.out_f32 || q.rowsum_out || q.adam || !q.out_lp) return 0;
-        if (q.drop.p > 0.f && q.drop.seed) return 0;
-        if (q.M < 1 || q.N < 8 || (q.N & 7) || (q.lda & 7) || (q.ldb & 7) || (q.ldc & 7) || q.lda < GK_K || q.ldb < GK_K) return 0;
-        if ((long)q.M * q.lda * 2 >= (1L << 31)) return 0;
-        if (((size_t)q.A | (size_t)q.B | (size_t)q.out_lp) & 15) return 0;
-        if (q.bias && ((size_t)q.bias & 15)) return 0;
-        GkProblem& P = G.p[i];
-        P.A = (const bf16_t*)q.A; P.B = (const bf16_t*)q.B; P.bias = q.bias; P.out = (bf16_t*)q.out_lp;
-        P.lda = q.lda; P.ldb = q.ldb; P.ldc = q.ldc; P.M = q.M; P.N = q.N; P.tiles_m = (q.M + 127) / 128;
+        if (!gk_fill(p[i], G.p[i])) return 0;
         G.tile_start[i] = tiles;
-        tiles += P.tiles_m * ((q.N + 127) / 128);
+        tiles += G.p[i].tiles_m * ((p[i].N + 127) / 128);
     }
     if (tiles < min_tiles) return 0;
     G.count = count;
@@ -366,8 +299,7 @@
         if (hipFuncSetAttribute((const void*)gemm_k512p_kernel, hipFuncAttributeMaxDynamicSharedMemorySize, GP_LDS) != hipSuccess) return 0;
         attr = true;
     }
-    long units = 0;
-    for (int i = 0; i < count; ++i) units += (long)((p[i].M + GP_ROWS - 1) / GP_ROWS) * ((p[i].N + 127) / 128);
+    const long units = gk_persist_units(count, p);
     const char* pe = MTN_ENV("MTN_K512_PERSIST");
     if (pe ? pe[0] != '0' : units >= 20L * GP_GRID) {
         hipLaunchKernelGGL(gemm_k512p_kernel, dim3(GP_GRID), dim3(GK_THREADS), GP_LDS, s, G);
@@ -378,11 +310,7 @@
     bool wide = true;
     for (int i = 0; i < count; ++i) wide = wide && (p[i].N % 256) == 0;
     if (wide) {
-        static bool attr_w = false;
-        if (!attr_w) {
-            if (hipFuncSetAttribute((const void*)gemm_k512w_kernel, hipFuncAttributeMaxDynamicSharedMemorySize, GK_LDS) != hipSuccess) return 0;
-            attr_w = true;
-        }
+        if (!gk_wide_attr()) return 0;
         int tw = 0;
         for (int i = 0; i < count; ++i) { G.tile_start[i] = tw; tw += G.p[i].tiles_m * (p[i].N / 256); }
         for (int i = count; i <= MTN_GEMM_MAX_GROUP; ++i) G.tile_start[i] = tw;
@@ -396,3 +324,112 @@
     if (tiles_out) *tiles_out = tiles;
     return 1;
 }
+
+#include <deque>
+#include <mutex>
+void gemm_census_note_k512(int count, const mtn_gemm_problem* p, int tiles);
+
+struct GkPending { mtn_gemm_problem q; GkProblem P; int total, done; };
+static std::deque<GkPending> g_pending;
+static std::mutex g_pending_mutex;
+static long g_rider_stats[3] = {0, 0, 0};
+
+extern "C" int mtn_riders_enabled(void) {
+    const char* e = MTN_ENV("MTN_RIDERS");
+    if (e && e[0] == '0') return 0;
+    const char* cap = MTN_ENV("MTN_RIDER_MAX_SLOTS");
+    return (cap && atoi(cap) <= 0) ? 0 : 1;
+}
+
+static int gk_flush_head(int n, hipStream_t s) {
+    if (n > 0 && !gk_wide_attr()) { mtn_set_error("gemm_k512w_kernel: cannot raise the dynamic LDS limit"); return MTN_ERR_LAUNCH; }
+    while (n > 0) {
+        const int k = n < MTN_GEMM_MAX_GROUP ? n : MTN_GEMM_MAX_GROUP;
+        GkGroup G;
+        memset(&G, 0, sizeof(G));
+        mtn_gemm_problem q[MTN_GEMM_MAX_GROUP];
+        int tw = -g_pending[0].done;
+        for (int i = 0; i < k; ++i) {
+            G.p[i] = g_pending[i].P; q[i] = g_pending[i].q;
+            G.tile_start[i] = tw;
+            tw += g_pending[i].total;
+        }
+        for (int i = k; i <= MTN_GEMM_MAX_GROUP; ++i) G.tile_start[i] = tw;
+        G.count = k;
+        if (tw > 0) {
+            hipLaunchKernelGGL(gemm_k512w_kernel, dim3(tw), dim3(GK_THREADS), GK_LDS, s, G);
+            if (hipGetLastError() != hipSuccess) { mtn_set_error("gemm_k512w_kernel: launch failed"); return MTN_ERR_LAUNCH; }
+            gemm_census_note_k512(k, q, tw);
+            g_rider_stats[1] += tw; ++g_rider_stats[2];
+        }
+        g_pending.erase(g_pending.begin(), g_pending.begin() + k);
+        n -= k;
+    }
+    return MTN_OK;
+}
+
+int gk_pending_flush_reads(int n, const void* const* outs, void* stream) {
+    std::lock_guard<std::mutex> lock(g_pending_mutex);
+    int last = -1;
+    for (int i = 0; i < (int)g_pending.size(); ++i)
+        for (int j = 0; j < n; ++j)
+            if (outs[j] && (const void*)g_pending[i].P.out == outs[j]) last = i;
+    return last < 0 ? MTN_OK : gk_flush_head(last + 1, (hipStream_t)stream);
+}
+
+void gk_rider_take(int slots, GkRider* K) {
+    std::lock_guard<std::mutex> lock(g_pending_mutex);
+    memset(K, 0, sizeof(*K));
+    int j = 0;
+    while (j < GK_RIDER_PROBLEMS && slots > 0 && !g_pending.empty()) {
+        GkPending& e = g_pending.front();
+        const int n = e.total - e.done < slots ? e.total - e.done : slots;
+        K->start[j] = K->units; K->tile0[j] = e.done; K->p[j] = e.P;
+        K->units += n; slots -= n; e.done += n;
+        ++j;
+        if (e.done == e.total) g_pending.pop_front();
+    }
+    for (int i = j; i <= GK_RIDER_PROBLEMS; ++i) K->start[i] = K->units;
+    g_rider_stats[0] += K->units;
+}
+
+int gk_pending_flush_all(void* stream) {
+    std::lock_guard<std::mutex> lock(g_pending_mutex);
+    return gk_flush_head((int)g_pending.size(), (hipStream_t)stream);
+}
+
+extern "C" int mtn_rider_counters(long* out4) {
+    MTN_CHECK_ARG(out4, "null output");
+    std::lock_guard<std::mutex> lock(g_pending_mutex);
+    long left = 0;
+    for (const GkPending& e : g_pending) left += e.total - e.done;
+    out4[0] = g_rider_stats[0]; out4[1] = g_rider_stats[1]; out4[2] = g_rider_stats[2]; out4[3] = left;
+    return MTN_OK;
+}
+
+extern "C" int mtn_kv_project(int dtype, int count, const mtn_gemm_problem* problems, int n_now, void* stream) {
+    MTN_CHECK_ARG(count >= 1 && problems && n_now >= 0, "bad problem list");
+    bool defer = mtn_riders_enabled() && dtype == MTN_BF16 && n_now < count && !MTN_ENV("MTN_K512_PERSIST") && !MTN_ENV("MTN_K512_WIDE");
+    GkProblem tmp;
+    for (int i = 0; i < count && defer; ++i) defer = gk_fill(problems[i], tmp) && problems[i].N % 256 == 0;
+    for (int i = 0; i < count && defer; i += MTN_GEMM_MAX_GROUP)
+        defer = gk_persist_units(count - i < MTN_GEMM_MAX_GROUP ? count - i : MTN_GEMM_MAX_GROUP, problems + i) < 20L * GP_GRID;
+    if (!defer) {
+        for (int i = 0; i < count; i += MTN_GEMM_MAX_GROUP) {
+            const int rc = mtn_gemm(dtype, count - i < MTN_GEMM_MAX_GROUP ? count - i : MTN_GEMM_MAX_GROUP, problems + i, stream);
+            if (rc != MTN_OK) return rc;
+        }
+        return MTN_OK;
+    }
+    std::lock_guard<std::mutex> lock(g_pending_mutex);
+    int rc = gk_flush_head((int)g_pending.size(), (hipStream_t)stream);
+    if (rc != MTN_OK) return rc;
+    for (int i = 0; i < count; ++i) {
+        GkPending e;
+        e.q = problems[i];
+        gk_fill(problems[i], e.P);
+        e.total = e.P.tiles_m * (e.P.N / 256); e.done = 0;
+        g_pending.push_back(e);
+    }
+    return gk_flush_head(n_now, (hipStream_t)stream);
+}
diff --git a/mtn_amd/csrc/gemm_k512_tile.h b/mtn_amd/csrc/gemm_k512_tile.h
--- /dev/null
+++ b/mtn_amd/csrc/gemm_k512_tile.h
@@ -0,0 +1,104 @@
+#pragma once
+#include "fused_common.h"
+
+static constexpr int GK_THREADS = 512;
+static constexpr int GK_K = 512;
+static constexpr int GK_LDS = 128 * FH_ROWB;
+static constexpr int GK_CPITCH = 272;
+static constexpr int GW_CPITCH = 528;
+
+struct GkProblem { const bf16_t* A; const bf16_t* B; const float* bias; bf16_t* out; int lda, ldb, ldc, M, N, tiles_m; };
+
+__device__ __forceinline__ void gk_wide_tile(const GkProblem& P, const int t, unsigned char* smem) {
+    const int tid = threadIdx.x, lane = tid & 63, l15 = lane & 15, lg = lane >> 4;
+    const int wave = __builtin_amdgcn_readfirstlane(tid >> 6);
+    const int tn = t / P.tiles_m, tm = t - tn * P.tiles_m;
+    const int row0 = tm * 128, col0 = tn * 256;
+    const int R = (P.M - row0) < 128 ? (P.M - row0) : 128;
+    {
+        const unsigned ldab = (unsigned)P.lda * 2u;
+        const __amdgpu_buffer_rsrc_t rs = __builtin_amdgcn_make_buffer_rsrc((void*)(P.A + (size_t)row0 * P.lda), 0, (R - 1) * ldab + FH_ROWB, 0x00020000);
+        for (int r = wave; r < 128; r += 8) {
+            const unsigned vo = r < R ? (unsigned)r * ldab + (unsigned)((lane ^ (r & 15)) << 4) : 0x80000000u;
+            __builtin_amdgcn_raw_ptr_buffer_load_lds(rs, (fh_lds_void_t*)(smem + r * FH_ROWB), 16, vo, 0, 0, 0);
+        }
+    }
+    float4 bq[2];
+#pragma unroll
+    for (int cb = 0; cb < 2; ++cb) {
+        const int colq = col0 + 128 * cb + 16 * wave + 4 * lg;
+        bq[cb] = make_float4(0.f, 0.f, 0.f, 0.f);
+        if (P.bias && colq < P.N) bq[cb] = *(const float4*)(P.bias + colq);
+    }
+    __builtin_amdgcn_sched_barrier(0);
+    uint4 wf[2][16];
+    {
+        const bf16_t* wrow[2];
+#pragma unroll
+        for (int cb = 0; cb < 2; ++cb) {
+            int n = col0 + 128 * cb + 16 * wave + (lane >> 2);
+            n = n < P.N ? n : P.N - 1;
+            wrow[cb] = P.B + (size_t)n * P.ldb + (lane & 3) * 8;
+        }
+#pragma unroll
+        for (int s = 0; s < 16; ++s) { wf[0][s] = *(const uint4*)(wrow[0] + s * 32); wf[1][s] = *(const uint4*)(wrow[1] + s * 32); }
+    }
+    __builtin_amdgcn_sched_barrier(0);
+    __builtin_amdgcn_s_waitcnt(0x8F70);
+    __builtin_amdgcn_s_barrier();
+    f32x4_t acc[2][8];
+#pragma unroll
+    for (int cb = 0; cb < 2; ++cb)
+#pragma unroll
+        for (int mt = 0; mt < 8; ++mt) acc[cb][mt] = f32x4_t{0.f, 0.f, 0.f, 0.f};
+    const int src = (4 * l15 + lg) * 4;
+#pragma unroll
+    for (int s = 0; s < 16; ++s) {
+#pragma unroll
+        for (int cb = 0; cb < 2; ++cb) {
+            wf[cb][s].x = (unsigned)__builtin_amdgcn_ds_bpermute(src, (int)wf[cb][s].x);
+            wf[cb][s].y = (unsigned)__builtin_amdgcn_ds_bpermute(src, (int)wf[cb][s].y);
+            wf[cb][s].z = (unsigned)__builtin_amdgcn_ds_bpermute(src, (int)wf[cb][s].z);
+            wf[cb][s].w = (unsigned)__builtin_amdgcn_ds_bpermute(src, (int)wf[cb][s].w);
+        }
+#pragma unroll
+        for (int mt = 0; mt < 8; ++mt) {
+            const uint4 xf = fh_xfrag(smem, mt * 16 + l15, s * 4 + lg);
+            mma16<bf16_t>(acc[0][mt], wf[0][s], xf);
+            mma16<bf16_t>(acc[1][mt], wf[1][s], xf);
+        }
+    }
+    __syncthreads();
+#pragma unroll
+    for (int cb = 0; cb < 2; ++cb)
+#pragma unroll
+        for (int mt = 0; mt < 8; ++mt) {
+            const int r = mt * 16 + l15;
+            *(uint2*)(smem + r * GW_CPITCH + (128 * cb + 16 * wave + 4 * lg) * 2) =
+                make_uint2(fh_pack2(acc[cb][mt][0] + bq[cb].x, acc[cb][mt][1] + bq[cb].y), fh_pack2(acc[cb][mt][2] + bq[cb].z, acc[cb][mt][3] + bq[cb].w));
+        }
+    __syncthreads();
+#pragma unroll
+    for (int ps = 0; ps < 8; ++ps) {
+        const int r = ps * 16 + (tid >> 5), c = tid & 31;
+        const int col = col0 + c * 8;
+        if (r < R && col < P.N)
+            *(uint4*)(P.out + (size_t)(row0 + r) * P.ldc + col) = *(const uint4*)(smem + r * GW_CPITCH + c * 16);
+    }
+}
+
+#define GK_RIDER_PROBLEMS 4
+struct GkRider {
+    int units;
+    int start[GK_RIDER_PROBLEMS + 1];
+    int tile0[GK_RIDER_PROBLEMS];
+    GkProblem p[GK_RIDER_PROBLEMS];
+};
+__device__ __forceinline__ void gk_rider_unit(const GkRider& K, const int r, unsigned char* smem) {
+    int j = 0;
+    while (j + 1 < GK_RIDER_PROBLEMS && r >= K.start[j + 1]) ++j;
+    gk_wide_tile(K.p[j], K.tile0[j] + r - K.start[j], smem);
+}
+
+void gk_rider_take(int slots, GkRider* K);
+int gk_pending_flush_reads(int n, const void* const* outs, void* stream);
diff --git a/mtn_amd/csrc/sublayer.hip b/mtn_amd/csrc/sublayer.hip
--- a/mtn_amd/csrc/sublayer.hip
+++ b/mtn_amd/csrc/sublayer.hip
@@ -3,6 +3,8 @@
 int fh_group_eligible(int dtype, int n_mha, const mtn_mha_args* mha, int n_ffn, const mtn_ffn_args* ffn);
 int fh_group_fwd_stage1(int n_mha, const mtn_mha_args* mha, int n_ffn, const mtn_ffn_args* ffn, void* stream);
 int fh_is_enabled();
+int gk_pending_flush_reads(int n, const void* const* outs, void* stream);
+int gk_pending_flush_all(void* stream);
 struct FbIo { const void* dyl; void *dq, *dk, *dv; int ldq, ldkv; const float* lnf; float* ln_part; };
 int fb_group_eligible(int dtype, int n_mha, const mtn_mha_args* mha, const FbIo* io);
 int fb_group_bwd_stage(int n_mha, const mtn_mha_args* mha, const FbIo* io, void* stream);
@@ -89,11 +91,20 @@
     t->o = a->o; t->ldo = d; t->lse = a->lse;
 }
 
+extern "C" int mtn_riders_flush(void* stream) { return gk_pending_flush_all(stream); }
+
 extern "C" int mtn_sublayer_group_fwd(int dtype, int n_mha, const mtn_mha_args* mha, int n_ffn, const mtn_ffn_args* ffn, void* stream) {
     MTN_CHECK_ARG(dtype == MTN_F32 || dtype == MTN_BF16, "bad dtype");
     MTN_CHECK_ARG(n_mha >= 0 && n_mha <= MTN_SUBLAYER_MAX_GROUP && n_ffn >= 0 && n_ffn <= MTN_SUBLAYER_MAX_GROUP && n_mha + n_ffn > 0, "bad group size");
     for (int i = 0; i < n_mha; ++i) RUN(check_mha(&mha[i], false));
     for (int i = 0; i < n_ffn; ++i) RUN(check_ffn(&ffn[i], false));
+    {
+        const void* reads[MTN_SUBLAYER_MAX_GROUP];
+        int n = 0;
+        for (int i = 0; i < n_mha; ++i)
+            if (!mha[i].self_attn && mha[i].kv_ready) reads[n++] = mha[i].kv;
+        if (n) RUN(gk_pending_flush_reads(n, reads, stream));
+    }
     bool fused = fh_group_eligible(dtype, n_mha, mha, n_ffn, ffn) != 0;
     mtn_mha_args pre[MTN_SUBLAYER_MAX_GROUP];
     if (!fused && n_mha > 0 && dtype == MTN_BF16 && fh_is_enabled()) {
diff --git a/mtn_amd/lib.py b/mtn_amd/lib.py
--- a/mtn_amd/lib.py
+++ b/mtn_amd/lib.py
@@ -238,6 +238,10 @@
     "mtn_attention_bwd_group": (C.c_int, [C.c_int, C.c_int, C.POINTER(AttnArgs), _P]),
     "mtn_cast_group": (C.c_int, [C.c_int, C.c_int, C.POINTER(CastDesc), _P]),
     "mtn_fused_enable": (C.c_int, [C.c_int]),
+    "mtn_kv_project": (C.c_int, [C.c_int, C.c_int, C.POINTER(GemmProblem), C.c_int, _P]),
+    "mtn_riders_flush": (C.c_int, [_P]),
+    "mtn_riders_enabled": (C.c_int, []),
+    "mtn_rider_counters": (C.c_int, [C.POINTER(C.c_long)]),
     "mtn_fused_counters": (C.c_int, [C.POINTER(C.c_long)]),
     "mtn_ln_epilogue_groups": (C.c_long, []),
     "mtn_ln_fold": (C.c_int, [C.c_int, _P, _P, C.c_int, C.c_int, _P]),
diff --git a/mtn_amd/mtn.py b/mtn_amd/mtn.py
--- a/mtn_amd/mtn.py
+++ b/mtn_amd/mtn.py
@@ -800,8 +800,12 @@
             self._seed.add_(0x9E3779B97F4A7C15 & 0x7FFFFFFFFFFFFFFF)
 
     def forward(self, b):
-        q, v, cp, hs, ae = self.encode(b.query, b.query_mask, b.his, b.his_mask, b.cap, b.cap_mask, b.fts, b.fts_mask)
-        return self.decode(v, hs, cp, q, b.fts_mask, b.his_mask, b.cap_mask, b.query_mask, b.trg, b.trg_mask, ae)
+        try:
+            q, v, cp, hs, ae = self.encode(b.query, b.query_mask, b.his, b.his_mask, b.cap, b.cap_mask, b.fts, b.fts_mask)
+            return self.decode(v, hs, cp, q, b.fts_mask, b.his_mask, b.cap_mask, b.query_mask, b.trg, b.trg_mask, ae)
+        finally:
+            if self._flat is not None and self._flat.is_cuda:
+                ops.flush_riders()
 
     def vid_encode(self, video_features, video_features_mask=None, encoded_query=None):
         return [self.vid_encoder[i](ft) for i, ft in enumerate(video_features)]
@@ -881,14 +885,17 @@
             ae = [self.query_embed(ft) for _ in range(len(vid))]
         return self.query_encoder(*streams, ae)
 
-    def hoist_memory_kv(self, cap_memory, his_memory, q_memory, vid_fts, outs=None):
+    def hoist_memory_kv(self, cap_memory, his_memory, q_memory, vid_fts, outs=None, defer=False):
         if not (self.hoist_kv and self.lockstep and self._flat is not None and q_memory.is_cuda):
             return None
         nF = len(vid_fts)
-        items, targets = [], []
-        for layer in self.decoder.layers:
+        items, targets, n_head, use_order = [], [], None, []
+        for li, layer in enumerate(self.decoder.layers):
+            if li == 1:
+                n_head = len(items)
             if layer._forward_hooks_on_sublayers() or nF + 1 > 4:
                 continue
+            first = len(items)
             text, chains, _, _ = layer._plan(cap_memory, None, his_memory, None, q_memory, None, None, vid_fts, [None] * nF,
                                              self.auto_encoder_ft)
             for sc, mod, mem, _ in list(text[1:]) + [chains[i][1] for i in range(nF)]:
@@ -898,7 +905,11 @@
                     continue
                 items.append((mem_lp, f["w_qkv_lp"], f["b_qkv"]))
                 targets.append(sc)
-        kvs = ops.project_memories(items, self.compute_dtype, outs)
+            idx = list(range(first, len(items)))
+            text_n = sum(1 for sc in targets[first:] if any(sc is t[0] for t in text[1:]))
+            use_order += idx[:1] + idx[text_n:] + idx[1:text_n] if text_n else idx
+        n_now = (n_head if n_head is not None else len(items)) if defer and L.load().mtn_riders_enabled() else None
+        kvs = ops.project_memories(items, self.compute_dtype, outs, n_now=n_now, order=use_order)
         self._kv_targets = list(zip(targets, kvs))
         self.attach_memory_kv(self._kv_targets)
         return kvs
@@ -909,6 +920,8 @@
             object.__setattr__(sc, "_kv_ready", kv)
 
     def clear_memory_kv(self):
+        if self._flat is not None and self._flat.is_cuda:
+            ops.flush_riders()
         for layer in self.decoder.layers:
             for sc in layer.sublayer:
                 if getattr(sc, "_kv_ready", None) is not None:
@@ -937,7 +950,7 @@
         v_l = enc_leaf[4:4 + nF]
         ae_l = enc_leaf[4 + nF:] if ae is not None else None
         ops.prepare_masks(b.trg_mask, b.his_mask, b.cap_mask, b.query_mask, b.fts_mask)
-        self.hoist_memory_kv(cp_l, hs_l, q_l, v_l)
+        self.hoist_memory_kv(cp_l, hs_l, q_l, v_l, defer=True)
         layers = []
         x_in, ae_in = x_l, ae_l
         for layer in self.decoder.layers:
@@ -960,7 +973,7 @@
                query_mask, tgt, tgt_mask, auto_encoded_ft):
         self.prepare()
         x0 = self.embed_target(tgt)
-        self.hoist_memory_kv(cap_memory, his_memory, query_memory, encoded_vid_features)
+        self.hoist_memory_kv(cap_memory, his_memory, query_memory, encoded_vid_features, defer=True)
         try:
             return self._decode_layers(encoded_vid_features, vid_features_mask, x0, his_memory, his_mask, cap_memory, cap_mask,
                                        query_memory, query_mask, tgt_mask, auto_encoded_ft)
diff --git a/mtn_amd/ops.py b/mtn_amd/ops.py
--- a/mtn_amd/ops.py
+++ b/mtn_amd/ops.py
@@ -1025,7 +1025,7 @@
     return out
 
 
-def project_memories(items, lp_dtype, outs=None):
+def project_memories(items, lp_dtype, outs=None, n_now=None, order=None):
     if not items:
         return []
     code = L.dtype_code(lp_dtype)
@@ -1039,9 +1039,17 @@
         p.bias, p.gate_scale, p.out_lp, p.ldc = b.data_ptr() + d * b.element_size(), 1.0, kv.data_ptr(), 2 * d
         outs.append(kv)
         probs.append(p)
+    if n_now is not None:
+        arr = (L.GemmProblem * len(probs))(*(probs[k] for k in (order if order is not None else range(len(probs)))))
+        L.check(L.load().mtn_kv_project(code, len(probs), arr, min(n_now, len(probs)), L.stream_ptr()))
+        return outs
     for i in range(0, len(probs), L.GEMM_MAX_GROUP):
         gemm(code, probs[i:i + L.GEMM_MAX_GROUP])
     return outs
+
+
+def flush_riders():
+    L.check(L.load().mtn_riders_flush(L.stream_ptr()))
 
 
 class EmbedNormFn(torch.autograd.Function):
```

After: 9154 samples/s (median of 6 runs). +2.1%, better.
